# leakless21/VietVoice-TTS

Hardware: AMD Instinct MI355X
Metric: audio-seconds/sec (24 kHz) at batch 32, 256-token utterances; RTF (higher is better)
Workload: dtype bf16

## Files before the change

vietvoice-tts_amd/csrc/vv_api.hip:

```cpp
#include <hip/hip_runtime.h>
#include <algorithm>
#include <cmath>
#include <cstdarg>
#include <cstdio>
#include <cstring>
#include <map>
#include <string>
#include <utility>
#include <vector>
#include "vv_kernels.h"

#define VV_VERSION_STR "vvtts-hip 0.14 (gfx950)"

namespace {
std::string g_create_error;

struct Bound { const void* p; uint64_t bytes; };

struct ProfRec { hipEvent_t a, b; int cls, sub; };

inline size_t align_up(size_t v, size_t a) { return (v + a - 1) / a * a; }
inline int pad_to(int v, int a) { return (v + a - 1) / a * a; }
}

struct vv_ctx {
    int device = 0;
    vv_model_cfg cfg{};
    int dt = VV_DTYPE_BF16;
    std::string err;
    std::map<std::string, Bound> w;
    bool finalized = false;
    bool ever_finalized = false;
    bool vocos = false;
    vv_vocos_cfg vcfg{};
    float post_bias = 0.f;
    int n_steps = 0;
    std::vector<float> dt_host;
    float* modtab = nullptr;
    float* fintab = nullptr;
    int ode_s = 1;
    double ode_a[16] = {}, ode_b[4] = {1.0, 0, 0, 0};
    int ode_kslot[4] = {-1, -1, -1, -1};
    int ode_nk = 0;
    int ms_q = 0;
    std::vector<double> ms_beta;
    double* ode_report = nullptr;
    int report_steps = 0, report_B = 0;
    char* ws = nullptr;
    size_t ws_cap = 0;
    uint64_t ws_generation = 0;
    int* d_mult = nullptr;
    int rope_rows = 0;
    int split_k_tail = 0;
    int chip_share = 1;
    int ring_tiles_max = 256;
    int ring_tiles = 1;
    int pp_min_tiles = -1;
    int lanes = 0;
    hipStream_t side_stream[1] = {};
    hipEvent_t ev_fork = nullptr, ev_join[1] = {};
    float rope_theta = 0.f;
    int rope_q_attn = 1;
    int voc_x3 = -1;
    int voc_x3_rows = 0;
    char* x3_buf = nullptr;
    std::map<std::string, const void*> x3_w;
    int fuse_mrf = 2;
    bool prof = false;
    std::vector<ProfRec> recs;
    std::vector<hipEvent_t> pool;
    int64_t p_launch[VV_PROF_NCLASS]{};
    double p_flops[VV_PROF_NCLASS]{}, p_bytes[VV_PROF_NCLASS]{}, p_ms[VV_PROF_NCLASS]{};

    int fail(int code, const char* fmt, ...) {
        char buf[1024];
        va_list ap;
        va_start(ap, fmt);
        vsnprintf(buf, sizeof buf, fmt, ap);
        va_end(ap);
        err = buf;
        return code;
    }
    const void* W(const std::string& n) const {
        auto it = w.find(n);
        return it == w.end() ? nullptr : it->second.p;
    }
    const float* Wf(const std::string& n) const { return (const float*)W(n); }
    int esz() const { return dt == VV_DTYPE_BF16 ? 2 : 4; }
    int bk() const { return dt == VV_DTYPE_BF16 ? 64 : 32; }
};

namespace {

#define HIPCHK(ctx, call)                                                                   \
    do {                                                                                    \
        hipError_t e__ = (call);                                                            \
        if (e__ != hipSuccess) return (ctx)->fail(-5, "%s: %s", #call, hipGetErrorString(e__)); \
    } while (0)

#define KCHK(ctx, call)                                              \
    do {                                                             \
        const char* m__ = "";                                        \
        int r__ = (call);                                            \
        if (r__ != 0) return (ctx)->fail(r__, "%s", m__);            \
    } while (0)

struct Prof {
    vv_ctx* c; int idx = -1; hipStream_t st;
    Prof(vv_ctx* c_, int cls, double flops, double bytes, hipStream_t st_, int sub = -1) : c(c_), st(st_) {
        if (!c->prof) return;
        ProfRec r; r.cls = cls; r.sub = sub;
        if (sub >= 0) { c->p_launch[sub]++; c->p_flops[sub] += flops; c->p_bytes[sub] += bytes; }
        auto get = [&]() { hipEvent_t e; if (!c->pool.empty()) { e = c->pool.back(); c->pool.pop_back(); } else hipEventCreate(&e); return e; };
        r.a = get(); r.b = get();
        hipEventRecord(r.a, st);
        c->recs.push_back(r); idx = (int)c->recs.size() - 1;
        c->p_launch[cls]++; c->p_flops[cls] += flops; c->p_bytes[cls] += bytes;
    }
    ~Prof() { if (idx >= 0) hipEventRecord(c->recs[idx].b, st); }
};

struct Arena {
    char* base = nullptr; size_t cap = 0, off = 0;
    template <typename T> T* take(size_t n) { off = align_up(off, 256); T* p = base ? (T*)(base + off) : nullptr; off += n * sizeof(T); return p; }
};
template <typename F> size_t plan_bytes(F&& plan) { Arena dry; plan(dry); return dry.off; }
int ensure_ws(vv_ctx* c, size_t bytes, Arena* a) {
    if (bytes > c->ws_cap) {
        if (c->ws) { hipDeviceSynchronize(); hipFree(c->ws); c->ws = nullptr; c->ws_cap = 0; }
        const size_t want = align_up(bytes + bytes / 16, 1 << 20);
        hipError_t e = hipMalloc((void**)&c->ws, want);
        if (e != hipSuccess) return c->fail(-12, "workspace hipMalloc(%zu MiB): %s", want >> 20, hipGetErrorString(e));
        c->ws_cap = want; ++c->ws_generation;
    }
    *a = Arena{c->ws, c->ws_cap, 0};
    return 0;
}
int use_ws(vv_ctx* c, void* block, size_t have, size_t need, Arena* a) {
    if ((uintptr_t)block % 256) return c->fail(-22, "workspace block must be 256-byte aligned");
    if (have < need) return c->fail(-22, "workspace block too small: %zu < %zu bytes", have, need);
    *a = Arena{(char*)block, have, 0};
    return 0;
}
template <typename F> int plan_ws(vv_ctx* c, void* block, size_t have, F&& plan) {
    const size_t need = plan_bytes(plan);
    Arena a;
    if (int r = block ? use_ws(c, block, have, need, &a) : ensure_ws(c, need, &a)) return r;
    plan(a);
    if (a.off > a.cap) return c->fail(-14, "workspace plan took %zu bytes of a %zu-byte block", a.off, a.cap);
    return 0;
}

struct Gemm : vv_gemm_args { const char* wname; };
Gemm gemm_args(const vv_ctx* c, int dtype, int out_dtype, int mode, int act, const void* A, int lda, const char* wname, int ldw,
               const char* bname, void* C, int ldc, int M, int N, int K) {
    Gemm g{};
    g.dtype = dtype; g.out_dtype = out_dtype; g.mode = mode; g.act = act;
    g.A = A; g.lda = lda; g.W = c->W(wname); g.ldw = ldw; g.C = C; g.ldc = ldc; g.M = M; g.N = N; g.K = K;
    g.bias = bname ? c->Wf(bname) : nullptr; g.wname = wname;
    if (bname && !g.bias) g.W = nullptr;
    return g;
}
int launch_gemm(vv_ctx* c, Gemm g, int cls, hipStream_t st, double alg_flops = -1) {
    if (!g.W) return c->fail(-2, "weight '%s' is not bound", g.wname);
    const int M = g.M, N = g.N, K = g.K, bf16 = g.dtype == VV_DTYPE_BF16;
    if (!g.chip_share) g.chip_share = c->chip_share;
    if (g.tile == 0 && c->pp_min_tiles >= 0 && bf16 && N % 256 == 0)
        g.tile = (M >= 4096 && (long long)((M + 255) / 256) * (N / 256) >= c->pp_min_tiles) ? 256 : 128;
    if (c->ring_tiles && g.tile == 0 && bf16 && N <= 1024 && N % 64 == 0 && (long long)((M + 63) / 64) * (N / 128) <= c->ring_tiles_max)
        g.tile = 6464;
    const int esz = bf16 ? 2 : 4, osz = g.out_dtype == VV_DTYPE_BF16 ? 2 : 4;
    const double fl = alg_flops >= 0 ? alg_flops : 2.0 * M * (double)N * K;
    Prof p(c, cls, fl, (double)M * K * esz + (double)N * K * esz + (double)M * N * osz * (g.mode == VV_EPI_GATE_RES ? 2 : 1), st);
    const char* m = "";
    if (int r = vvk_gemm(&g, st, &m)) return c->fail(r, "%s (weight %s, M=%d N=%d K=%d)", m, g.wname, M, N, K);
    return 0;
}

std::string blk(int i, const char* s) { return "blocks." + std::to_string(i) + s; }

inline hipStream_t enter(vv_ctx* c, void* stream) {
    hipSetDevice(c->device);
    return (hipStream_t)stream;
}

inline bool fits(int64_t off, int64_t n, int64_t total) { return off >= 0 && n >= 0 && n <= total && off <= total - n; }

inline bool spans_overlap(const void* a, uint64_t na, const void* b, uint64_t nb) {
    return (uintptr_t)a < (uintptr_t)b + nb && (uintptr_t)b < (uintptr_t)a + na;
}

struct PtrArg { const char* name; const void* p; unsigned align = 1; bool may_be_null = false; };

int check_ptrs(vv_ctx* c, const char* entry, std::initializer_list<PtrArg> args) {
    for (const PtrArg& a : args) {
        if (!a.p && !a.may_be_null) return c->fail(-22, "%s: null pointer (%s)", entry, a.name);
        if ((uintptr_t)a.p % a.align) return c->fail(-22, "%s: misaligned pointer (%s: %u bytes)", entry, a.name, a.align);
    }
    return 0;
}

int check_ws(vv_ctx* c, const char* entry, uint64_t have, uint64_t need, const char* what = "ws") {
    return have < need ? c->fail(-22, "%s: %s of %llu bytes, %llu are needed", entry, what, (unsigned long long)have, (unsigned long long)need) : 0;
}

int flac_rows(vv_ctx* c, const char* name, const int64_t* rows, const int64_t* rows_host, int R, int64_t n_bytes, int* max_channels) {
    if (R < 1 || R > 65535 || n_bytes < 8 || n_bytes > ((int64_t)1 << 31) - 64)
        return c->fail(-22, "%s: bad sizes (1 <= R <= 65535, 8 <= n_bytes <= 2^31 - 64)", name);
    if (int e = check_ptrs(c, name, {{"rows", rows, 8}, {"rows_host", rows_host, 8}})) return e;
    int64_t at = 0;
    *max_channels = 1;
    for (int r = 0; r < R; ++r) {
        const int64_t* q = rows_host + 8 * (size_t)r;
        if (q[0] < at || q[0] % 4 || !fits(q[0], q[1], n_bytes - 8))
            return c->fail(-22, "%s: row %d: the clips lie in ascending order, 4-byte aligned, inside data less 8 bytes of padding", name, r);
        if (q[2] < 1 || q[2] > 8 || (q[3] != 8 && q[3] != 16 && q[3] != 24) || q[5] < 16 || q[5] > 65535 || q[4] < 0 || q[4] > q[5] || q[6] < 1 ||
            q[6] > 1048575 || q[7] < 0 || q[7] > VV_FLAC_MAX_CLIP)
            return c->fail(-22, "%s: row %d: channels 1 ... 8, bits 8 / 16 / 24, 16 <= max block <= 65535, min <= max, rate 1 ... 1048575, total <= 2^26", name, r);
        at = q[0] + q[1];
        if (q[2] > *max_channels) *max_channels = (int)q[2];
    }
    return 0;
}

}

extern "C" {

const char* vv_version(void) { return VV_VERSION_STR; }

const char* vv_last_error(const vv_ctx* ctx) { return ctx ? ctx->err.c_str() : g_create_error.c_str(); }

int vv_create(vv_ctx** out, int device, const vv_model_cfg* cfg, int acoustic_dtype) {
    if (!out || !cfg) { g_create_error = "vv_create: null argument"; return -22; }
    *out = nullptr;
    int n = 0;
    hipError_t e = hipGetDeviceCount(&n);
    if (e != hipSuccess || n <= 0) { g_create_error = "vv_create: no HIP device visible (the HIP path has no CPU fallback)"; return -19; }
    if (device < 0 || device >= n) { g_create_error = "vv_create: device index out of range"; return -22; }
    if (acoustic_dtype != VV_DTYPE_F32 && acoustic_dtype != VV_DTYPE_BF16) { g_create_error = "vv_create: dtype must be f32 or bf16"; return -22; }
    if (cfg->head_dim != 64 || cfg->heads * 64 != cfg->dim) { g_create_error = "vv_create: head_dim must be 64"; return -22; }
    if (cfg->dim % 128 || cfg->text_dim % 128 || cfg->dim / cfg->pos_conv_groups != 64 || cfg->n_mel % 4 || cfg->dim > 1024 ||
        cfg->text_dim > 1024) {
        g_create_error = "vv_create: dim/text_dim must be multiples of 128 (<=1024), 64 channels per pos-conv group"; return -22;
    }
    if (cfg->voc_n_up < 1 || cfg->voc_n_up > VV_MAX_UP || cfg->voc_n_res > VV_MAX_RES || cfg->voc_n_dil > VV_MAX_RES) {
        g_create_error = "vv_create: vocoder topology out of range"; return -22;
    }
    e = hipSetDevice(device);
    if (e != hipSuccess) { g_create_error = hipGetErrorString(e); return -5; }
    vv_ctx* c = new vv_ctx();
    c->device = device; c->cfg = *cfg; c->dt = acoustic_dtype;
    *out = c;
    return 0;
}

void vv_destroy(vv_ctx* c) {
    if (!c) return;
    hipSetDevice(c->device);
    hipDeviceSynchronize();
    if (c->ws) hipFree(c->ws);
    if (c->modtab) hipFree(c->modtab);
    if (c->fintab) hipFree(c->fintab);
    if (c->d_mult) hipFree(c->d_mult);
    if (c->x3_buf) hipFree(c->x3_buf);
    for (auto q : c->side_stream) if (q) hipStreamDestroy(q);
    if (c->ev_fork) hipEventDestroy(c->ev_fork);
    for (auto e : c->ev_join) if (e) hipEventDestroy(e);
    for (auto& r : c->recs) { hipEventDestroy(r.a); hipEventDestroy(r.b); }
    for (auto e : c->pool) hipEventDestroy(e);
    delete c;
}

int vv_bind_weight(vv_ctx* c, const char* name, const void* p, uint64_t bytes) {
    if (!c || !name || !p) return c ? c->fail(-22, "vv_bind_weight: null argument") : -22;
    if ((uintptr_t)p % 16) return c->fail(-22, "vv_bind_weight(%s): pointer must be 16-byte aligned", name);
    c->w[name] = Bound{p, bytes};
    c->finalized = false;
    return 0;
}

int vv_finalize_weights(vv_ctx* c) {
    if (!c) return -22;
    const vv_model_cfg& g = c->cfg;
    const int D = g.dim, Dt = g.text_dim, FF = g.dim * g.ff_mult, es = c->esz();
    const int KP = pad_to(2 * g.n_mel + Dt, 64), MP = pad_to(g.n_mel, 128);
    std::string missing;
    auto need = [&](const std::string& n, uint64_t bytes) {
        auto it = c->w.find(n);
        if (it == c->w.end()) { missing += n + " "; return; }
        if (it->second.bytes < bytes) missing += n + "(short:" + std::to_string(it->second.bytes) + "<" + std::to_string(bytes) + ") ";
    };
    need("const.window", 4ull * g.n_fft); need("const.tw_cos", 4ull * g.n_fft); need("const.tw_sin", 4ull * g.n_fft);
    need("const.mel_fb", 4ull * (g.n_fft / 2 + 1) * g.n_mel);
    need("const.text_pos", 4ull * g.max_pos * Dt);
    need("text.embed.weight", 4ull * g.vocab_rows * Dt);
    for (int i = 0; i < g.text_layers; ++i) {
        const std::string p = "text.blocks." + std::to_string(i);
        need(p + ".dwconv.weight", 4ull * Dt * g.text_conv_k); need(p + ".dwconv.bias", 4ull * Dt);
        need(p + ".norm.weight", 4ull * Dt); need(p + ".norm.bias", 4ull * Dt);
        need(p + ".pwconv1.weight", (uint64_t)es * Dt * g.text_ff_mult * Dt); need(p + ".pwconv1.bias", 4ull * Dt * g.text_ff_mult);
        need(p + ".grn.gamma", 4ull * Dt * g.text_ff_mult); need(p + ".grn.beta", 4ull * Dt * g.text_ff_mult);
        need(p + ".pwconv2.weight", (uint64_t)es * Dt * g.text_ff_mult * Dt); need(p + ".pwconv2.bias", 4ull * Dt);
    }
    need("input.proj.weight", (uint64_t)es * D * KP); need("input.proj.bias", 4ull * D);
    for (int j = 1; j <= 2; ++j) {
        need("input.pos_conv" + std::to_string(j) + ".weight", (uint64_t)es * D * 64 * g.pos_conv_k);
        need("input.pos_conv" + std::to_string(j) + ".bias", 4ull * D);
    }
    need("time.mlp1.weight", 4ull * D * g.time_freq_dim); need("time.mlp1.bias", 4ull * D);
    need("time.mlp2.weight", 4ull * D * D); need("time.mlp2.bias", 4ull * D);
    for (int i = 0; i < g.depth; ++i) {
        need(blk(i, ".adaln.weight"), 4ull * 6 * D * D); need(blk(i, ".adaln.bias"), 4ull * 6 * D);
        need(blk(i, ".attn.qkv.weight"), (uint64_t)es * 3 * D * D); need(blk(i, ".attn.qkv.bias"), 4ull * 3 * D);
        need(blk(i, ".attn.out.weight"), (uint64_t)es * D * D); need(blk(i, ".attn.out.bias"), 4ull * D);
        need(blk(i, ".ff1.weight"), (uint64_t)es * FF * D); need(blk(i, ".ff1.bias"), 4ull * FF);
        need(blk(i, ".ff2.weight"), (uint64_t)es * D * FF); need(blk(i, ".ff2.bias"), 4ull * D);
    }
    need("final.adaln.weight", 4ull * 2 * D * D); need("final.adaln.bias", 4ull * 2 * D);
    need("final.proj.weight", (uint64_t)es * MP * D); need("final.proj.bias", 4ull * MP);
    if (c->vocos) {
        const vv_vocos_cfg& v = c->vcfg;
        const uint64_t V = v.dim, I = v.intermediate, KE = pad_to(v.embed_k * g.n_mel, 32), HP = pad_to(v.n_fft + 2, 128);
        need("const.istft_basis", 4ull * v.n_fft * v.n_fft);
        need("voc.embed.weight", 4 * V * KE); need("voc.embed.bias", 4 * V);
        for (const char* n : {"voc.norm", "voc.final_norm"}) { need(std::string(n) + ".weight", 4 * V); need(std::string(n) + ".bias", 4 * V); }
        for (int i = 0; i < v.layers; ++i) {
            const std::string p = "voc.blocks." + std::to_string(i);
            need(p + ".dwconv.weight", 4 * V * v.dw_k); need(p + ".dwconv.bias", 4 * V);
            need(p + ".norm.weight", 4 * V); need(p + ".norm.bias", 4 * V);
            need(p + ".pwconv1.weight", 4 * I * V); need(p + ".pwconv1.bias", 4 * I);
            need(p + ".pwconv2.weight", 4 * V * I); need(p + ".pwconv2.bias", 4 * V);
            need(p + ".gamma", 4 * V);
        }
        need("voc.head.weight", 4 * HP * V); need("voc.head.bias", 4 * HP);
        if (!missing.empty()) return c->fail(-2, "missing or short weights: %s", missing.c_str());
        c->finalized = c->ever_finalized = true;
        return 0;
    }
    int ch = g.voc_pre_ch;
    struct ConvW { std::string name; int cin_pad, kw, rows_pad; };
    std::vector<ConvW> convs;
    convs.push_back({"voc.pre.weight", pad_to(g.n_mel, 8), g.voc_pre_k, pad_to(ch, 64)});
    need("voc.pre.weight", 4ull * pad_to(g.n_mel, 8) * g.voc_pre_k * pad_to(ch, 64)); need("voc.pre.bias", 4ull * ch);
    for (int s = 0; s < g.voc_n_up; ++s) {
        const int cin = ch, cout = ch / 2, u = g.voc_up_rates[s];
        const std::string p = "voc.up." + std::to_string(s);
        need(p + ".weight", 4ull * pad_to(cin, 8) * 2 * pad_to(cout * u, 64)); need(p + ".bias", 4ull * cout);
        convs.push_back({p + ".weight", pad_to(cin, 8), 2, pad_to(cout * u, 64)});
        for (int a = 0; a < g.voc_n_res; ++a)
            for (int b = 0; b < g.voc_n_dil; ++b)
                for (int k = 1; k <= 2; ++k) {
                    const std::string q = "voc.res." + std::to_string(s) + "." + std::to_string(a) + "." + std::to_string(b) + ".conv" + std::to_string(k);
                    need(q + ".weight", 4ull * pad_to(cout, 8) * g.voc_res_kernels[a] * pad_to(cout, 64)); need(q + ".bias", 4ull * cout);
                    convs.push_back({q + ".weight", pad_to(cout, 8), g.voc_res_kernels[a], pad_to(cout, 64)});
                }
        ch = cout;
    }
    need("voc.post.weight", 4ull * ch * g.voc_post_k); need("voc.post.bias", 4);
    if (!missing.empty()) return c->fail(-2, "missing or short weights: %s", missing.c_str());
    hipSetDevice(c->device);
    HIPCHK(c, hipMemcpy(&c->post_bias, c->W("voc.post.bias"), 4, hipMemcpyDeviceToHost));
    {
        size_t total = 0;
        for (const ConvW& w : convs) total = align_up(total, 256) + vvk_conv_split_bytes(w.cin_pad, w.kw, w.rows_pad);
        if (c->x3_buf) { HIPCHK(c, hipFree(c->x3_buf)); c->x3_buf = nullptr; }
        c->x3_w.clear();
        HIPCHK(c, hipMalloc((void**)&c->x3_buf, total));
        size_t off = 0;
        for (const ConvW& w : convs) {
            off = align_up(off, 256);
            const char* m__ = "";
            if (int r = vvk_conv_split_weights(c->Wf(w.name), w.cin_pad, w.kw, w.rows_pad, c->x3_buf + off, nullptr, &m__))
                return c->fail(r, "%s (%s)", m__, w.name.c_str());
            c->x3_w[w.name] = c->x3_buf + off;
            off += vvk_conv_split_bytes(w.cin_pad, w.kw, w.rows_pad);
        }
        HIPCHK(c, hipStreamSynchronize(nullptr));
    }
    std::vector<int> mult(g.voc_n_up + 1, 1);
    for (int s = 0; s < g.voc_n_up; ++s) mult[s + 1] = mult[s] * g.voc_up_rates[s];
    if (!c->d_mult) HIPCHK(c, hipMalloc((void**)&c->d_mult, sizeof(int) * (VV_MAX_UP + 1)));
    HIPCHK(c, hipMemcpy(c->d_mult, mult.data(), sizeof(int) * mult.size(), hipMemcpyHostToDevice));
    c->finalized = c->ever_finalized = true;
    return 0;
}

int vv_set_vocos(vv_ctx* c, const vv_vocos_cfg* v) {
    if (!c) return -22;
    if (!v) return c->fail(-22, "vv_set_vocos: null cfg");
    if (c->ever_finalized) return c->fail(-22, "vv_set_vocos: only between vv_create and vv_finalize_weights");
    const vv_model_cfg& g = c->cfg;
    if (v->dim < 128 || v->dim > 1024 || v->dim % 128 || v->intermediate < 128 || v->intermediate > 16384 || v->intermediate % 128)
        return c->fail(-22, "vv_set_vocos: dim must be a multiple of 128 in [128, 1024], intermediate a multiple of 128 (fp32 GEMM tiles)");
    if (v->layers < 1 || v->layers > 64 || v->embed_k < 1 || v->embed_k > 31 || v->embed_k % 2 == 0 || v->dw_k < 1 || v->dw_k > 31 || v->dw_k % 2 == 0 ||
        !(v->ln_eps > 0.f))
        return c->fail(-22, "vv_set_vocos: 1..64 layers, odd kernel sizes up to 31, ln_eps > 0");
    if (v->n_fft != v->win_length || v->n_fft != g.n_fft || g.win_length != g.n_fft || v->hop_length != g.hop_length || v->n_fft % 128 ||
        v->hop_length < 1 || v->n_fft % v->hop_length || v->n_fft / v->hop_length > 16)
        return c->fail(-22, "vv_set_vocos: the ISTFT needs n_fft == win_length == the model's n_fft (a multiple of 128) and the model's hop "
                            "(dividing n_fft, at most 16 frames per sample)");
    c->vcfg = *v;
    c->vocos = true;
    return 0;
}

static int set_plan_impl(vv_ctx* c, const char* who, const float* sinus_host, const float* dt_host, int n_steps, int s, const double* a,
                         const double* b, void* stream) {
    if (!c) return -22;
    if (!c->finalized) return c->fail(-1, "%s: weights not finalized", who);
    if (n_steps < 1 || n_steps > 512 || !sinus_host || !dt_host) return c->fail(-22, "%s: bad arguments", who);
    if (s < 1 || s > 4 || !a || !b) return c->fail(-22, "%s: 1 to 4 stages with their tableau", who);
    if ((long long)n_steps * s > 512) return c->fail(-22, "%s: %d steps x %d stages exceed 512 evaluations", who, n_steps, s);
    double sum_b = 0;
    for (int i = 0; i < s; ++i) {
        if (!std::isfinite(b[i])) return c->fail(-22, "%s: the tableau must be finite", who);
        sum_b += b[i];
        for (int j = 0; j < s; ++j) {
            if (!std::isfinite(a[i * s + j])) return c->fail(-22, "%s: the tableau must be finite", who);
            if (j >= i && a[i * s + j] != 0.0) return c->fail(-22, "%s: the tableau must be strictly lower triangular (explicit method)", who);
        }
    }
    if (!(std::fabs(sum_b - 1.0) < 1e-6)) return c->fail(-22, "%s: the weights b must sum to 1", who);
    for (int n = 0; n < n_steps; ++n)
        if (!std::isfinite(dt_host[n])) return c->fail(-22, "%s: the step sizes must be finite", who);
    hipSetDevice(c->device);
    hipStream_t st = (hipStream_t)stream;
    const int D = c->cfg.dim, S = n_steps * s, TF = c->cfg.time_freq_dim, L = c->cfg.depth;
    if (TF % 32) return c->fail(-22, "time_freq_dim must be a multiple of 32");
    if (c->modtab) { hipDeviceSynchronize(); hipFree(c->modtab); hipFree(c->fintab); c->modtab = c->fintab = nullptr; }
    HIPCHK(c, hipMalloc((void**)&c->modtab, sizeof(float) * (size_t)L * S * 6 * D));
    HIPCHK(c, hipMalloc((void**)&c->fintab, sizeof(float) * (size_t)S * 2 * D));
    float *sin_d, *t1, *t2;
    auto bufs = [&](Arena& a) { sin_d = a.take<float>((size_t)S * TF); t1 = a.take<float>((size_t)S * D); t2 = a.take<float>((size_t)S * D); };
    if (int r = plan_ws(c, nullptr, 0, bufs)) return r;
    HIPCHK(c, hipMemcpyAsync(sin_d, sinus_host, 4ull * S * TF, hipMemcpyHostToDevice, st));
    HIPCHK(c, hipStreamSynchronize(st));
    const int f32 = VV_DTYPE_F32, store = VV_EPI_STORE;
    if (int r = launch_gemm(c, gemm_args(c, f32, f32, store, VV_ACT_SILU_, sin_d, TF, "time.mlp1.weight", TF, "time.mlp1.bias", t1, D, S, D, TF), VV_PROF_GEMM, st)) return r;
    if (int r = launch_gemm(c, gemm_args(c, f32, f32, store, VV_ACT_SILU_, t1, D, "time.mlp2.weight", D, "time.mlp2.bias", t2, D, S, D, D), VV_PROF_GEMM, st)) return r;
    for (int l = 0; l < L; ++l) {
        const std::string wn = blk(l, ".adaln.weight"), bn = blk(l, ".adaln.bias");
        if (int r = launch_gemm(c, gemm_args(c, f32, f32, store, VV_ACT_NONE_, t2, D, wn.c_str(), D, bn.c_str(), c->modtab + (size_t)l * S * 6 * D, 6 * D, S, 6 * D, D), VV_PROF_GEMM, st)) return r;
    }
    if (int r = launch_gemm(c, gemm_args(c, f32, f32, store, VV_ACT_NONE_, t2, D, "final.adaln.weight", D, "final.adaln.bias", c->fintab, 2 * D, S, 2 * D, D), VV_PROF_GEMM, st)) return r;
    HIPCHK(c, hipStreamSynchronize(st));
    c->n_steps = n_steps;
    c->dt_host.assign(dt_host, dt_host + n_steps);
    c->ode_s = s;
    std::fill(c->ode_a, c->ode_a + 16, 0.0);
    std::fill(c->ode_b, c->ode_b + 4, 0.0);
    for (int i = 0; i < s; ++i) {
        c->ode_b[i] = b[i];
        for (int j = 0; j < i; ++j) c->ode_a[i * 4 + j] = a[i * s + j];
    }
    c->ode_nk = 0;
    for (int j = 0; j < 4; ++j) {
        bool later = j < s - 1 && c->ode_b[j] != 0.0;
        for (int m = j + 2; m < s; ++m) later = later || c->ode_a[m * 4 + j] != 0.0;
        c->ode_kslot[j] = later ? c->ode_nk++ : -1;
    }
    c->ms_q = 0; c->ms_beta.clear();
    c->ode_report = nullptr; c->report_steps = c->report_B = 0;
    return 0;
}

int vv_set_time_grid(vv_ctx* c, const float* sinus_host, const float* dt_host, int n_steps, void* stream) {
    const double a = 0.0, b = 1.0;
    return set_plan_impl(c, "vv_set_time_grid", sinus_host, dt_host, n_steps, 1, &a, &b, stream);
}

int vv_set_ode_plan(vv_ctx* c, const float* sinus_host, const float* dt_host, int n_steps, int s, const double* a, const double* b, void* stream) {
    return set_plan_impl(c, "vv_set_ode_plan", sinus_host, dt_host, n_steps, s, a, b, stream);
}

int vv_set_ode_multistep(vv_ctx* c, const float* sinus_host, const float* dt_host, int n_steps, int q, const double* beta, void* stream) {
    if (!c) return -22;
    if (n_steps < 1 || n_steps > 512) return c->fail(-22, "vv_set_ode_multistep: bad arguments");
    if (q < 1 || q > 3 || !beta) return c->fail(-22, "vv_set_ode_multistep: 1 to 3 slopes per step with their weights");
    for (int n = 0; n < n_steps; ++n) {
        double sum = 0;
        for (int j = 0; j < q; ++j) {
            const double v = beta[(size_t)n * q + j];
            if (!std::isfinite(v)) return c->fail(-22, "vv_set_ode_multistep: the weights must be finite");
            if (j > n && v != 0.0) return c->fail(-22, "vv_set_ode_multistep: step %d has a weight on a slope from before step 0", n);
            sum += v;
        }
        if (!(std::fabs(sum - 1.0) < 1e-6)) return c->fail(-22, "vv_set_ode_multistep: the weights of step %d must sum to 1", n);
    }
    const double a = 0.0, b = 1.0;
    if (int r = set_plan_impl(c, "vv_set_ode_multistep", sinus_host, dt_host, n_steps, 1, &a, &b, stream)) return r;
    c->ms_q = q;
    c->ms_beta.assign(beta, beta + (size_t)n_steps * q);
    return 0;
}

int vv_set_ode_report(vv_ctx* c, double* report, int n_steps, int B) {
    if (!c) return -22;
    if (!report) { c->ode_report = nullptr; c->report_steps = c->report_B = 0; return 0; }
    if (c->ms_q < 1) return c->fail(-22, "vv_set_ode_report: the report needs a multistep plan (vv_set_ode_multistep)");
    if (n_steps != c->n_steps || B < 1 || B > VVK_GUIDE_MAX_ITEMS) return c->fail(-22, "vv_set_ode_report: [%d steps of the plan][1..%d items][2]", c->n_steps, VVK_GUIDE_MAX_ITEMS);
    if ((uintptr_t)report % 8) return c->fail(-22, "vv_set_ode_report: report must be a float64 array");
    c->ode_report = report; c->report_steps = n_steps; c->report_B = B;
    return 0;
}

static int preprocess_impl(vv_ctx* c, int B, int N, const int16_t* audio, int ld_audio, int max_audio_len, const int32_t* audio_len,
                           const int32_t* audio_len_host, const int32_t* text_ids, int ld_text, const int32_t* text_len, const int32_t* seq_len,
                           float* cat, float* cat_drop, int32_t* ref_len, void* stream, const uint8_t* keep = nullptr, int ld_keep = 0) {
    if (!c) return -22;
    if (!c->finalized) return c->fail(-1, "vv_preprocess: weights not finalized");
    if (B < 1 || N < 1 || !audio || !audio_len || !text_ids || !text_len || !seq_len || !cat || !cat_drop || !ref_len)
        return c->fail(-22, "vv_preprocess: bad arguments");
    const vv_model_cfg& g = c->cfg;
    if (N > g.max_pos) return c->fail(-22, "vv_preprocess: N=%d exceeds the position tables (%d)", N, g.max_pos);
    if (max_audio_len < g.n_fft || max_audio_len > ld_audio) return c->fail(-22, "vv_preprocess: reference clips must hold >= n_fft samples and fit ld_audio");
    if (audio_len_host)
        for (int b = 0; b < B; ++b)
            if (audio_len_host[b] < g.n_fft / 2 + 1 || audio_len_host[b] > max_audio_len)
                return c->fail(-22, "vv_preprocess: reference clip %d has %d samples; a clip needs between n_fft/2 + 1 = %d and max_audio_len = %d",
                               b, audio_len_host[b], g.n_fft / 2 + 1, max_audio_len);
    hipSetDevice(c->device);
    hipStream_t st = (hipStream_t)stream;
    const int Dt = g.text_dim, C2 = Dt * g.text_ff_mult, M = g.n_mel, es = c->esz();
    const int F_max = max_audio_len / g.hop_length + 1;
    const size_t R2 = (size_t)2 * B * N;
    float *mel, *tx, *ty, *sumsq;
    char *th, *tm;
    auto bufs = [&](Arena& a) {
        mel = a.take<float>((size_t)B * F_max * M);
        tx = a.take<float>(R2 * Dt); ty = a.take<float>(R2 * Dt);
        th = a.take<char>((size_t)es * R2 * Dt); tm = a.take<char>((size_t)es * R2 * C2);
        sumsq = a.take<float>((size_t)2 * B * C2);
    };
    if (int r = plan_ws(c, nullptr, 0, bufs)) return r;

    KCHK(c, vvk_ref_len(audio_len, ref_len, B, g.hop_length, st, &m__));
    {
        Prof p(c, VV_PROF_MEL, 4.0 * B * F_max * (double)g.n_fft * (g.n_fft / 2 + 1), 2.0 * B * max_audio_len + 4.0 * B * F_max * M, st);
        KCHK(c, vvk_mel(audio, ld_audio, audio_len, c->Wf("const.window"), c->Wf("const.tw_cos"), c->Wf("const.tw_sin"),
                        c->Wf("const.mel_fb"), mel, B, F_max, g.n_fft, g.hop_length, M, st, &m__));
    }
    {
        Prof p(c, VV_PROF_TEXT, 0, 8.0 * R2 * Dt, st);
        KCHK(c, vvk_text_embed(text_ids, ld_text, text_len, c->Wf("text.embed.weight"), c->Wf("const.text_pos"), tx, B, N, Dt, g.vocab_rows, st, &m__));
    }
    for (int i = 0; i < g.text_layers; ++i) {
        const std::string p = "text.blocks." + std::to_string(i);
        {
            Prof pr(c, VV_PROF_TEXT, 2.0 * R2 * Dt * g.text_conv_k, 8.0 * R2 * Dt, st);
            KCHK(c, vvk_dwconv(tx, ty, c->Wf(p + ".dwconv.weight"), c->Wf(p + ".dwconv.bias"), seq_len, B, 2 * B, N, Dt, g.text_conv_k, st, &m__));
        }
        {
            vv_ln_args a{}; a.out_dtype = c->dt; a.x = ty; a.ldx = Dt; a.y = th; a.ldy = Dt; a.R = (int)R2; a.D = Dt;
            a.w = c->Wf(p + ".norm.weight"); a.b = c->Wf(p + ".norm.bias"); a.add_one = 0; a.eps = 1e-6f;
            Prof pr(c, VV_PROF_NORM, 0, (4.0 + es) * R2 * Dt, st);
            KCHK(c, vvk_ln_mod(&a, st, &m__));
        }
        const std::string w1 = p + ".pwconv1.weight", b1 = p + ".pwconv1.bias", w2 = p + ".pwconv2.weight", b2 = p + ".pwconv2.bias";
        if (int r = launch_gemm(c, gemm_args(c, c->dt, c->dt, VV_EPI_STORE, VV_ACT_GELU_ERF_, th, Dt, w1.c_str(), Dt, b1.c_str(), tm, C2, (int)R2, C2, Dt), VV_PROF_GEMM, st)) return r;
        {
            Prof pr(c, VV_PROF_TEXT, 0, 3.0 * es * R2 * C2, st);
            KCHK(c, vvk_grn(c->dt, tm, sumsq, c->Wf(p + ".grn.gamma"), c->Wf(p + ".grn.beta"), seq_len, B, 2 * B, N, C2, st, &m__));
        }
        if (int r = launch_gemm(c, gemm_args(c, c->dt, VV_DTYPE_F32, VV_EPI_GATE_RES, VV_ACT_NONE_, tm, C2, w2.c_str(), C2, b2.c_str(), tx, Dt, (int)R2, Dt, C2), VV_PROF_GEMM, st)) return r;
    }
    {
        Prof p(c, VV_PROF_ELEMWISE, 0, 12.0 * B * N * (M + Dt) + (keep ? (double)B * N : 0.0), st);
        KCHK(c, vvk_build_cat(mel, F_max, ref_len, tx, cat, cat_drop, B, N, M, Dt, st, &m__, keep, ld_keep));
    }
    if (keep) HIPCHK(c, hipMemsetAsync(ref_len, 0, sizeof(int32_t) * B, st));
    return 0;
}

int vv_preprocess(vv_ctx* c, int B, int N, const int16_t* audio, int ld_audio, int max_audio_len, const int32_t* audio_len,
                  const int32_t* text_ids, int ld_text, const int32_t* text_len, const int32_t* seq_len, float* cat,
                  float* cat_drop, int32_t* ref_len, void* stream) {
    return preprocess_impl(c, B, N, audio, ld_audio, max_audio_len, audio_len, nullptr, text_ids, ld_text, text_len, seq_len, cat, cat_drop, ref_len, stream);
}

int vv_preprocess_h(vv_ctx* c, int B, int N, const int16_t* audio, int ld_audio, int max_audio_len, const int32_t* audio_len,
                    const int32_t* audio_len_host, const int32_t* text_ids, int ld_text, const int32_t* text_len, const int32_t* seq_len,
                    float* cat, float* cat_drop, int32_t* ref_len, void* stream) {
    if (c && !audio_len_host) return c->fail(-22, "vv_preprocess_h: host lengths missing");
    return preprocess_impl(c, B, N, audio, ld_audio, max_audio_len, audio_len, audio_len_host, text_ids, ld_text, text_len, seq_len, cat, cat_drop, ref_len, stream);
}

int vv_preprocess_edit(vv_ctx* c, int B, int N, const int16_t* audio, int ld_audio, int max_audio_len, const int32_t* audio_len,
                       const int32_t* audio_len_host, const int32_t* text_ids, int ld_text, const int32_t* text_len, const int32_t* seq_len,
                       float* cat, float* cat_drop, int32_t* ref_len, const uint8_t* keep, int ld_keep, void* stream) {
    if (!c) return -22;
    if (!audio_len_host) return c->fail(-22, "vv_preprocess_edit: host lengths missing");
    if (!keep || ld_keep < N) return c->fail(-22, "vv_preprocess_edit: keep must be a device array [B][ld_keep] with ld_keep >= N");
    return preprocess_impl(c, B, N, audio, ld_audio, max_audio_len, audio_len, audio_len_host, text_ids, ld_text, text_len, seq_len, cat, cat_drop,
                           ref_len, stream, keep, ld_keep);
}

int vv_edit_splice(vv_ctx* c, const int16_t* src, int64_t n_src, const int64_t* desc, int n_rows, int B, int16_t* out, int ld_out, void* stream) {
    if (!c) return -22;
    if (B < 1 || n_rows < 0 || n_src < 0 || !out || ld_out < 4 || ld_out % 4 || (uintptr_t)out % 8 || (n_rows > 0 && (!src || !desc)))
        return c->fail(-22, "vv_edit_splice: bad arguments (out [B][ld_out] 8-byte aligned with ld_out %% 4 == 0; src and desc for n_rows > 0)");
    hipSetDevice(c->device);
    hipStream_t st = (hipStream_t)stream;
    Prof p(c, VV_PROF_ELEMWISE, 0, 4.0 * B * ld_out + 32.0 * n_rows, st);
    KCHK(c, vvk_edit_splice(src, (long long)n_src, (const long long*)desc, n_rows, B, out, ld_out, st, &m__));
    return 0;
}

int vv_edit_restore(vv_ctx* c, int B, int N, float* x, const float* cat, const uint8_t* keep, int ld_keep, const int32_t* seq_len, void* stream) {
    if (!c) return -22;
    const int M = c->cfg.n_mel, cd = c->cfg.n_mel + c->cfg.text_dim;
    if (B < 1 || N < 1 || !x || !cat || !keep || !seq_len || ld_keep < N || (uintptr_t)x % 16 || (uintptr_t)cat % 16)
        return c->fail(-22, "vv_edit_restore: bad arguments (x, cat 16-byte aligned; keep [B][ld_keep] with ld_keep >= N)");
    hipSetDevice(c->device);
    hipStream_t st = (hipStream_t)stream;
    Prof p(c, VV_PROF_ELEMWISE, 0, (double)B * N * (1 + 8.0 * M), st);
    KCHK(c, vvk_edit_restore(x, cat, keep, ld_keep, seq_len, B, N, M, cd, st, &m__));
    return 0;
}

int vv_noise_fill(vv_ctx* c, int B, int N, int n_mel, float* x, const int32_t* seq_len, const uint64_t* keys, int kind, void* stream) {
    if (!c) return -22;
    if (B < 1 || N < 1 || n_mel < 4 || n_mel % 4 || (kind != 0 && kind != 1) || !x || !seq_len || !keys || (uintptr_t)x % 16 || (uintptr_t)keys % 8)
        return c->fail(-22, "vv_noise_fill: bad arguments (B, N >= 1; n_mel %% 4 == 0; x 16-byte aligned; keys [B][2] uint64; kind 0 or 1)");
    hipSetDevice(c->device);
    hipStream_t st = (hipStream_t)stream;
    Prof p(c, VV_PROF_ELEMWISE, 0, (double)B * (12.0 + 4.0 * N * n_mel), st);
    KCHK(c, vvk_noise_fill(x, seq_len, (const unsigned long long*)keys, B, N, n_mel, kind, st, &m__));
    return 0;
}

int vv_join_chunks(vv_ctx* c, const int16_t* pcm, int64_t n_pcm, const int64_t* chunk_rows, const int64_t* chunk_rows_host, int n_chunks,
                   const int64_t* req_rows, const int64_t* req_rows_host, int R, const double* fade, int64_t n_fade, int max_n, int64_t max_len,
                   int16_t* out, int64_t n_out, void* ws, void* stream) {
    if (!c) return -22;
    hipStream_t st = enter(c, stream);
    if (R < 1 || n_chunks < R || max_n < 0 || max_n > vvk_join_max_n())
        return c->fail(-22, "vv_join_chunks: bad arguments (1 <= R <= n_chunks; max_n <= %d)", vvk_join_max_n());
    if (int e = check_ptrs(c, "vv_join_chunks", {{"pcm", pcm}, {"chunk_rows", chunk_rows}, {"req_rows", req_rows}, {"out", out, 16}, {"ws", ws}})) return e;
    if ((chunk_rows_host == nullptr) != (req_rows_host == nullptr)) return c->fail(-22, "vv_join_chunks: host rows come as a pair or not at all");
    if (chunk_rows_host) {
        for (int r = 0; r < R; ++r) {
            const int64_t* q = req_rows_host + 4 * (size_t)r;
            if (q[1] < 1 || !fits(q[0], q[1], n_chunks) || !fits(q[2], q[3], n_out))
                return c->fail(-22, "vv_join_chunks: request row %d does not fit the chunk rows or the output", r);
            for (int64_t k = q[0]; k < q[0] + q[1]; ++k) {
                const int64_t* w = chunk_rows_host + 8 * (size_t)k;
                if (!fits(w[0], w[1], n_pcm) || w[2] < 0 || w[3] < 0 || w[3] > max_n || w[1] > max_len || w[7] != r ||
                    (w[3] > 0 && !fits(w[5], 2 * w[3], n_fade)))
                    return c->fail(-22, "vv_join_chunks: chunk row %lld does not fit the buffers", (long long)k);
                if (q[1] >= 2 && w[1] <= 0)
                    return c->fail(-22, "vv_join_chunks: chunk %lld is empty inside a request of %lld chunks", (long long)k, (long long)q[1]);
            }
        }
    }
    Prof p(c, VV_PROF_ELEMWISE, 0, 4.0 * (double)n_out + 96.0 * n_chunks, st);
    KCHK(c, vvk_join_chunks(pcm, (long long)n_pcm, (const long long*)chunk_rows, n_chunks, (const long long*)req_rows, R, fade, (long long)n_fade,
                            max_n, (long long)max_len, out, (long long)n_out, ws, st, &m__));
    return 0;
}

int vv_pcm_resample(vv_ctx* c, const int16_t* x, int64_t n_x, const int64_t* rows, int n_rows, int64_t max_out, const double* taps, int n_taps,
                    int up, int down, int skip, int16_t* y, int64_t n_y, void* stream) {
    if (!c) return -22;
    hipStream_t st = enter(c, stream);
    if (n_rows < 1 || n_taps < 1 || up < 1 || down < 1 || skip < 0 || max_out < 0)
        return c->fail(-22, "vv_pcm_resample: bad arguments (n_rows, n_taps, up, down >= 1; skip, max_out >= 0)");
    if (int e = check_ptrs(c, "vv_pcm_resample", {{"x", x}, {"rows", rows}, {"taps", taps}, {"y", y}})) return e;
    Prof p(c, VV_PROF_ELEMWISE, 2.0 * (double)n_y * (n_taps / up + 1), 2.0 * (double)(n_x + n_y), st);
    KCHK(c, vvk_pcm_resample(x, (long long)n_x, (const long long*)rows, n_rows, (long long)max_out, taps, n_taps, up, down, skip, y, (long long)n_y,
                             st, &m__));
    return 0;
}

int vv_pcm_encode(vv_ctx* c, const int16_t* x, int64_t n_x, const int64_t* rows, int n_rows, int64_t max_n, int kind, uint8_t* y, int64_t n_y,
                  void* stream) {
    if (!c) return -22;
    hipStream_t st = enter(c, stream);
    if (n_rows < 1 || (kind != 1 && kind != 2) || max_n < 0)
        return c->fail(-22, "vv_pcm_encode: bad arguments (n_rows >= 1; kind 1 = mu-law, 2 = A-law)");
    if (int e = check_ptrs(c, "vv_pcm_encode", {{"x", x}, {"rows", rows}, {"y", y, 8}})) return e;
    Prof p(c, VV_PROF_ELEMWISE, 0, 2.0 * (double)n_x + (double)n_y, st);
    KCHK(c, vvk_pcm_encode(x, (long long)n_x, (const long long*)rows, n_rows, (long long)max_n, kind, y, (long long)n_y, st, &m__));
    return 0;
}

uint64_t vv_pcm_loudness_ws_bytes(int64_t total_runs, int R) { return vvk_pcm_loudness_ws_bytes((long long)total_runs, R); }

int vv_pcm_loudness(vv_ctx* c, const int16_t* x, int64_t n_x, const int64_t* rows, const int64_t* rows_host, int R, int64_t sub,
                    const double* tables, const double* params, int16_t* y, int64_t n_y, double* stats, void* ws, uint64_t ws_bytes,
                    void* stream) {
    if (!c) return -22;
    hipStream_t st = enter(c, stream);
    if (R < 1 || R > 65535 || sub < VV_LOUD_RUN || sub > (1 << 24) || n_x < 0 || n_y < 0)
        return c->fail(-22, "vv_pcm_loudness: bad sizes (1 <= R <= 65535; sub >= %d)", VV_LOUD_RUN);
    if (int e = check_ptrs(c, "vv_pcm_loudness", {{"x", x, 2}, {"y", y, 2, true}, {"rows", rows, 8}, {"rows_host", rows_host}, {"tables", tables, 8},
                                                  {"params", params, 8}, {"stats", stats, 8}, {"ws", ws, 8}})) return e;
    const int64_t rps = (sub + VV_LOUD_RUN - 1) / VV_LOUD_RUN;
    int64_t total_runs = 0, max_n = 0;
    for (int r = 0; r < R; ++r) {
        const int64_t* q = rows_host + 4 * (size_t)r;
        if (!fits(q[0], q[1], n_x) || q[1] >= ((int64_t)1 << 40))
            return c->fail(-22, "vv_pcm_loudness: row %d does not fit the %lld samples of x", r, (long long)n_x);
        if (y && !fits(q[2], q[1], n_y)) return c->fail(-22, "vv_pcm_loudness: row %d does not fit the %lld samples of y", r, (long long)n_y);
        if (y == x && q[2] != q[0]) return c->fail(-22, "vv_pcm_loudness: in place (y == x) needs dst_off == src_off, row %d", r);
        if (q[3] != total_runs) return c->fail(-22, "vv_pcm_loudness: row %d: run_off is the sum of the runs of the rows before it", r);
        const int64_t J = q[1] / sub;
        total_runs += J * rps + (q[1] - J * sub + VV_LOUD_RUN - 1) / VV_LOUD_RUN;
        if (q[1] > max_n) max_n = q[1];
    }
    if (int e = check_ws(c, "vv_pcm_loudness", ws_bytes, vvk_pcm_loudness_ws_bytes((long long)total_runs, R))) return e;
    Prof p(c, VV_PROF_ELEMWISE, 60.0 * (double)n_x, 6.0 * (double)n_x + 128.0 * (double)total_runs, st);
    KCHK(c, vvk_pcm_loudness(x, (long long)n_x, (const long long*)rows, R, (long long)sub, (long long)total_runs, (long long)max_n, tables,
                             params, y, (long long)n_y, stats, ws, st, &m__));
    return 0;
}

int vv_pcm_limit_tile(int L) { return L < 1 || L > VV_LIMIT_MAX_L ? -22 : vvk_pcm_limit_tile(L); }

uint64_t vv_pcm_limit_ws_bytes(int64_t total_samples, int64_t total_tiles, int R) {
    return vvk_pcm_limit_ws_bytes((long long)total_samples, (long long)total_tiles, R);
}

int vv_pcm_limit(vv_ctx* c, const int16_t* x, int64_t n_x, const int64_t* rows, const int64_t* rows_host, int R, int L, int mode,
                 const double* window, const double* taps, const double* params, const double* meas, int16_t* y, int64_t n_y, double* stats,
                 void* ws, uint64_t ws_bytes, void* stream) {
    if (!c) return -22;
    hipStream_t st = enter(c, stream);
    if (R < 1 || R > 65535 || L < 1 || L > VV_LIMIT_MAX_L || (mode != 0 && mode != 1) || n_x < 0 || n_y < 0)
        return c->fail(-22, "vv_pcm_limit: bad sizes (1 <= R <= 65535; 1 <= L <= %d; mode 0 or 1)", VV_LIMIT_MAX_L);
    if (int e = check_ptrs(c, "vv_pcm_limit", {{"x", x, 2}, {"y", y, 2, true}, {"rows", rows, 8}, {"rows_host", rows_host}, {"window", window, 8},
                                               {"taps", taps, 8}, {"params", params, 8}, {"meas", meas, 8, true}, {"stats", stats, 8}, {"ws", ws, 8}})) return e;
    const int64_t tile = vvk_pcm_limit_tile(L);
    int64_t total_samples = 0, total_tiles = 0, max_tiles = 0, max_out = 0;
    for (int r = 0; r < R; ++r) {
        const int64_t* q = rows_host + 5 * (size_t)r;
        if (q[0] < 0 || q[1] < 0 || q[2] < 0 || q[3] < 0 || q[4] < 0) return c->fail(-22, "vv_pcm_limit: row %d has a negative field", r);
        if (!fits(q[0], q[1], n_x) || q[1] >= ((int64_t)1 << 40))
            return c->fail(-22, "vv_pcm_limit: row %d does not fit the %lld samples of x", r, (long long)n_x);
        if (!fits(q[3], q[4], q[1])) return c->fail(-22, "vv_pcm_limit: row %d: out_lo + out_n exceeds n", r);
        if (y && !fits(q[2], q[4], n_y)) return c->fail(-22, "vv_pcm_limit: row %d does not fit the %lld samples of y", r, (long long)n_y);
        if (y == x && q[4] > 0 && q[2] != q[0] + q[3])
            return c->fail(-22, "vv_pcm_limit: in place (y == x) needs dst_off == src_off + out_lo, row %d", r);
        const int64_t nt = (q[1] + tile - 1) / tile;
        total_samples += q[1];
        total_tiles += nt;
        if (nt > max_tiles) max_tiles = nt;
        if (q[4] > max_out) max_out = q[4];
    }
    if (int e = check_ws(c, "vv_pcm_limit", ws_bytes, vvk_pcm_limit_ws_bytes((long long)total_samples, (long long)total_tiles, R))) return e;
    Prof p(c, VV_PROF_ELEMWISE, (mode ? 640.0 : 500.0) * (double)total_samples * (double)(2 * L + 1) / 241.0,
           20.0 * (double)total_samples + 2.0 * (double)max_out * R, st);
    KCHK(c, vvk_pcm_limit(x, (long long)n_x, (const long long*)rows, R, L, mode, (long long)total_samples, (long long)total_tiles,
                          (long long)max_tiles, (long long)max_out, window, taps, params, meas, y, (long long)n_y, stats, ws, st, &m__));
    return 0;
}

uint64_t vv_pcm_stretch_ws_bytes(int R) { return vvk_pcm_stretch_ws_bytes(R); }

int vv_pcm_stretch(vv_ctx* c, const int16_t* x, int64_t n_x, const int64_t* rows, const int64_t* rows_host, int R, const double* window,
                   int16_t* y, int64_t n_y, int32_t* pos, int64_t n_pos, void* ws, uint64_t ws_bytes, void* stream) {
    if (!c) return -22;
    hipStream_t st = enter(c, stream);
    if (R < 1 || R > 65535 || n_x < 0 || n_y < 0 || n_pos < 0) return c->fail(-22, "vv_pcm_stretch: bad sizes (1 <= R <= 65535)");
    if (int e = check_ptrs(c, "vv_pcm_stretch", {{"x", x, 2}, {"y", y, 2, true}, {"rows", rows, 8}, {"rows_host", rows_host}, {"window", window, 8},
                                                 {"pos", pos, 4}, {"ws", ws, 8}})) return e;
    if (y && spans_overlap(x, 2ull * n_x, y, 2ull * n_y))
        return c->fail(-22, "vv_pcm_stretch: y overlaps x (an output sample reads two frames of the input: not in place)");
    if (int e = check_ws(c, "vv_pcm_stretch", ws_bytes, vvk_pcm_stretch_ws_bytes(R))) return e;
    std::vector<std::pair<int64_t, int64_t>> on_y, on_pos;
    int64_t total_out = 0, total_frames = 0, max_out = 0;
    for (int r = 0; r < R; ++r) {
        const int64_t* q = rows_host + 6 * (size_t)r;
        if (q[0] < 0 || q[1] < 0 || q[2] < 0 || q[5] < 0) return c->fail(-22, "vv_pcm_stretch: row %d has a negative field", r);
        if (q[3] < 1 || q[3] > VV_WSOLA_MAX_PQ || q[4] < 1 || q[4] > VV_WSOLA_MAX_PQ || q[3] == q[4] || 4 * q[3] < q[4] || q[3] > 4 * q[4])
            return c->fail(-22, "vv_pcm_stretch: row %d: p and q in 1 ... %d, p != q, 1/4 <= p / q <= 4", r, VV_WSOLA_MAX_PQ);
        if (!fits(q[0], q[1], n_x) || q[1] > ((int64_t)1 << 30))
            return c->fail(-22, "vv_pcm_stretch: row %d does not fit the %lld samples of x", r, (long long)n_x);
        const int64_t n_s = (q[1] * q[3] + q[4] - 1) / q[4], M = (n_s + VV_WSOLA_HS - 1) / VV_WSOLA_HS;
        if (y && !fits(q[2], n_s, n_y)) return c->fail(-22, "vv_pcm_stretch: row %d does not fit the %lld samples of y", r, (long long)n_y);
        if (!fits(q[5], M + 1, n_pos)) return c->fail(-22, "vv_pcm_stretch: row %d does not fit the %lld entries of pos", r, (long long)n_pos);
        if (y && n_s > 0) on_y.emplace_back(q[2], q[2] + n_s);
        on_pos.emplace_back(q[5], q[5] + M + 1);
        total_out += n_s;
        total_frames += M;
        if (n_s > max_out) max_out = n_s;
    }
    for (auto* spans : {&on_y, &on_pos}) {
        std::sort(spans->begin(), spans->end());
        for (size_t i = 1; i < spans->size(); ++i)
            if ((*spans)[i].first < (*spans)[i - 1].second)
                return c->fail(-22, "vv_pcm_stretch: rows overlap on %s", spans == &on_y ? "y" : "pos");
    }
    Prof p(c, VV_PROF_ELEMWISE, 2.0 * (double)total_frames * VV_WSOLA_N * 2 * VV_WSOLA_D + 3.0 * (double)total_out,
           2.0 * (double)total_frames * (2 * VV_WSOLA_N + 2 * VV_WSOLA_D) + 6.0 * (double)total_out, st);
    KCHK(c, vvk_pcm_stretch(x, (long long)n_x, (const long long*)rows, R, (long long)max_out, window, y, (long long)n_y, (int*)pos,
                            (long long)n_pos, ws, st, &m__));
    return 0;
}

uint64_t vv_pcm_formant_ws_bytes(int64_t total_frames, int R) { return vvk_pcm_formant_ws_bytes((long long)total_frames, R); }

int vv_pcm_formant(vv_ctx* c, const int16_t* x, int64_t n_x, const int16_t* y, int64_t n_y, const int64_t* rows, const int64_t* rows_host, int R,
                   const double* wa, const double* g, const double* window, int16_t* z, int64_t n_z, double* h_out, int64_t n_h, void* ws,
                   uint64_t ws_bytes, void* stream) {
    if (!c) return -22;
    hipStream_t st = enter(c, stream);
    if (R < 1 || R > 65535 || n_x < 0 || n_y < 0 || n_z < 0 || n_h < 0) return c->fail(-22, "vv_pcm_formant: bad sizes (1 <= R <= 65535)");
    if (int e = check_ptrs(c, "vv_pcm_formant", {{"x", x, 2}, {"y", y, 2}, {"rows", rows, 8}, {"rows_host", rows_host}, {"wa", wa, 8}, {"g", g, 8},
                                                 {"window", window, 8}, {"z", z, 2}, {"h_out", h_out, 8, true}, {"ws", ws, 8}})) return e;
    if (spans_overlap(x, 2ull * n_x, z, 2ull * n_z) || spans_overlap(y, 2ull * n_y, z, 2ull * n_z))
        return c->fail(-22, "vv_pcm_formant: z overlaps x or y (an output sample reads L samples of y: not in place)");
    std::vector<std::pair<int64_t, int64_t>> on_z;
    int64_t total_frames = 0, max_frames = 0, total_out = 0;
    for (int r = 0; r < R; ++r) {
        const int64_t* q = rows_host + 7 * (size_t)r;
        if (q[0] < 0 || q[1] < 0 || q[2] < 0 || q[3] < 0 || q[4] < 0) return c->fail(-22, "vv_pcm_formant: row %d has a negative field", r);
        if (q[5] < 1 || q[5] > VV_WSOLA_MAX_PQ || q[6] < 1 || q[6] > VV_WSOLA_MAX_PQ)
            return c->fail(-22, "vv_pcm_formant: row %d: tn and td in 1 ... %d", r, VV_WSOLA_MAX_PQ);
        if (!fits(q[0], q[1], n_x) || q[1] > ((int64_t)1 << 30))
            return c->fail(-22, "vv_pcm_formant: row %d does not fit the %lld samples of x", r, (long long)n_x);
        if (q[3] != (q[1] * q[6] + q[5] - 1) / q[5]) return c->fail(-22, "vv_pcm_formant: row %d: n_f is not ceil(n td / tn)", r);
        if (!fits(q[2], q[3], n_y)) return c->fail(-22, "vv_pcm_formant: row %d does not fit the %lld samples of y", r, (long long)n_y);
        if (!fits(q[4], q[3], n_z)) return c->fail(-22, "vv_pcm_formant: row %d does not fit the %lld samples of z", r, (long long)n_z);
        const int64_t frames = (q[3] + VV_FORMANT_H - 1) / VV_FORMANT_H + 1;
        if (q[3] > 0) on_z.emplace_back(q[4], q[4] + q[3]);
        total_frames += frames;
        total_out += q[3];
        if (frames > max_frames) max_frames = frames;
    }
    std::sort(on_z.begin(), on_z.end());
    for (size_t i = 1; i < on_z.size(); ++i)
        if (on_z[i].first < on_z[i - 1].second) return c->fail(-22, "vv_pcm_formant: rows overlap on z");
    if (h_out && n_h / VV_FORMANT_L < total_frames)
        return c->fail(-22, "vv_pcm_formant: h_out of %lld doubles, %lld are needed", (long long)n_h, (long long)total_frames * VV_FORMANT_L);
    if (int e = check_ws(c, "vv_pcm_formant", ws_bytes, vvk_pcm_formant_ws_bytes((long long)total_frames, R))) return e;
    Prof p(c, VV_PROF_ELEMWISE, 4.0 * (double)total_out * VV_FORMANT_L + 2.0 * (double)total_frames * VV_FORMANT_L * VV_FORMANT_P,
           24.0 * (double)total_frames * VV_FORMANT_L + 4.0 * (double)total_out, st);
    KCHK(c, vvk_pcm_formant(x, (long long)n_x, y, (long long)n_y, (const long long*)rows, R, (long long)total_frames, (long long)max_frames, wa, g,
                            window, z, (long long)n_z, h_out, ws, st, &m__));
    return 0;
}

uint64_t vv_pcm_denoise_ws_bytes(int R) { return vvk_pcm_denoise_ws_bytes(R); }

int vv_pcm_denoise(vv_ctx* c, const int16_t* x, int64_t n_x, const int64_t* rows, const int64_t* rows_host, int R, const double* strengths,
                   const double* strengths_host, const double* bias, int64_t n_bias, const double* window, const double* twiddles, int16_t* y,
                   int64_t n_y, double* mag_out, int64_t n_mag, void* ws, uint64_t ws_bytes, void* stream) {
    if (!c) return -22;
    hipStream_t st = enter(c, stream);
    if (R < 1 || R > 65535 || n_x < 0 || n_y < 0 || n_bias < 1 || n_mag < 0) return c->fail(-22, "vv_pcm_denoise: bad sizes (1 <= R <= 65535, n_bias >= 1)");
    if (int e = check_ptrs(c, "vv_pcm_denoise", {{"x", x, 2}, {"rows", rows, 8}, {"rows_host", rows_host}, {"strengths", strengths, 8},
                                                 {"strengths_host", strengths_host}, {"bias", bias, 8}, {"window", window, 8},
                                                 {"twiddles", twiddles, 8}, {"y", y, 2}, {"mag_out", mag_out, 8, true}, {"ws", ws, 8}})) return e;
    if (spans_overlap(x, 2ull * n_x, y, 2ull * n_y))
        return c->fail(-22, "vv_pcm_denoise: y overlaps x (a hop reads the input under its neighbours: not in place)");
    std::vector<std::pair<int64_t, int64_t>> on_y;
    int64_t total_frames = 0, max_hops = 1, total_hops = 0;
    for (int r = 0; r < R; ++r) {
        const int64_t* q = rows_host + 4 * (size_t)r;
        if (q[0] < 0 || q[1] < 0 || q[2] < 0 || q[3] < 0) return c->fail(-22, "vv_pcm_denoise: row %d has a negative field", r);
        if (q[3] >= n_bias) return c->fail(-22, "vv_pcm_denoise: row %d: bias_row %lld of %lld", r, (long long)q[3], (long long)n_bias);
        if (!(strengths_host[r] >= 0.0 && strengths_host[r] <= 16.0)) return c->fail(-22, "vv_pcm_denoise: row %d: a strength in 0 ... 16 is needed", r);
        if (!fits(q[0], q[1], n_x) || q[1] > ((int64_t)1 << 30))
            return c->fail(-22, "vv_pcm_denoise: row %d does not fit the %lld samples of x", r, (long long)n_x);
        if (!fits(q[2], q[1], n_y)) return c->fail(-22, "vv_pcm_denoise: row %d does not fit the %lld samples of y", r, (long long)n_y);
// ... 581 lines not shown
            }
        }
        return n_views;
    }
};

int steps_schedule(const StepsRun& r, Lane* lanes, hipStream_t st) {
    vv_ctx* c = r.c;
    const int n_lanes = r.P.n_lanes, step0 = r.q.a.step0, n_steps = r.q.a.n_steps;
    const bool branch_lanes = r.P.branch_lanes, guide = r.q.guide != nullptr;
    if ((n_lanes > 1 || branch_lanes) && !c->side_stream[0]) {
        HIPCHK(c, hipStreamCreateWithFlags(&c->side_stream[0], hipStreamNonBlocking));
        HIPCHK(c, hipEventCreateWithFlags(&c->ev_join[0], hipEventDisableTiming));
    }
    if ((n_lanes > 1 || branch_lanes) && !c->ev_fork) HIPCHK(c, hipEventCreateWithFlags(&c->ev_fork, hipEventDisableTiming));
    const hipStream_t streams[2] = {st, c->side_stream[0]};
    auto fork = [&]() -> int {
        HIPCHK(c, hipEventRecord(c->ev_fork, st)); HIPCHK(c, hipStreamWaitEvent(c->side_stream[0], c->ev_fork, 0));
        return 0;
    };
    auto join = [&]() { hipEventRecord(c->ev_join[0], c->side_stream[0]); hipStreamWaitEvent(st, c->ev_join[0], 0); };
    Lane views[2]; GuideState gstate[2];
    auto make_views = [&](const GuideState* gs) {
        const int n = r.lane_views(gs, views);
        for (int v = 0; v < n; ++v) views[v].st = streams[v];
        return c->chip_share = n;
    };
    for (int li = 0; li < n_lanes; ++li) lanes[li].st = streams[li];
    int n_views = make_views(nullptr), rc = 0;
    if (n_lanes > 1) rc = fork();
    for (int li = 0; li < n_lanes && !rc; ++li) rc = r.setup(lanes[li]);
    for (int s = step0; s < step0 + n_steps && !rc; ++s)
        for (int i = 0; i < r.ns && !rc; ++i) {
            const int e = s * r.ns + i;
            for (int li = 0; li < n_lanes && !rc; ++li) rc = r.pack(lanes[li], gstate[li], s, i);
            if (guide) n_views = make_views(gstate);
            const bool want_fork = branch_lanes && n_views == 2;
            if (want_fork && !rc) rc = fork();
            const bool forked = want_fork && !rc;
            for (int v = 0; v < n_views && !rc; ++v) rc = r.step_head(views[v]);
            for (int l = 0; l < r.g.depth && !rc; ++l)
                for (int v = 0; v < n_views && !rc; ++v) rc = r.block(views[v], e, l);
            for (int v = 0; v < n_views && !rc; ++v) rc = r.step_tail(views[v], e);
            if (forked) join();
            for (int li = 0; li < n_lanes && !rc; ++li) rc = r.combine(lanes[li], s, i);
        }
    if (n_lanes > 1) join();
    c->chip_share = 1;
    return rc;
}
}

static int transformer_steps(vv_ctx* c, StepsCall q, void* stream) {
    if (!c) return -22;
    const vv_steps_args& a = q.a;
    q.with_apg = q.apg != nullptr || q.ws_form == WS_APG; q.guided = q.guide != nullptr || q.ws_form != WS_PLAIN || q.with_apg;
    q.rk = c->ode_s > 1 || c->ms_q > 0 || a.cfg_item != nullptr || q.guide != nullptr || q.apg != nullptr;
    const int B = a.B, N = a.N;
    if (!c->finalized || !c->modtab) return c->fail(-1, "vv_transformer_steps: weights/time grid not ready");
    if (B < 1 || N < 1 || (!q.ws_only && (!a.seq_len || !a.x || !a.cat_mel_text || !a.cat_mel_text_drop || !a.rope_cos_q || !a.rope_sin_q || !a.rope_cos_k || !a.rope_sin_k)))
        return c->fail(-22, "vv_transformer_steps: bad arguments");
    if (a.step0 < 0 || a.n_steps < 0 || a.step0 + a.n_steps > c->n_steps) return c->fail(-22, "vv_transformer_steps: steps [%d,%d) outside the time grid (%d)", a.step0, a.step0 + a.n_steps, c->n_steps);
    if (c->ms_q && !q.ws_only && a.step0 != 0) return c->fail(-22, "vv_transformer_steps: under a multistep plan a call starts at step 0 (the kept slopes live for one call), got step0 = %d", a.step0);
    if (c->ms_q && c->ode_report && !q.ws_only && (c->report_B != B || c->report_steps != c->n_steps))
        return c->fail(-22, "vv_transformer_steps: the step report was set for %d steps of %d items, the call has %d of %d", c->report_steps, c->report_B, c->n_steps, B);
    if (q.guide && q.ld_guide < B) return c->fail(-22, "vv_transformer_steps_guided: ld_guide = %d < B = %d", q.ld_guide, B);
    if (q.guide && c->split_k_tail) return c->fail(-22, "vv_transformer_steps_guided: a guidance mask cannot be combined with option split_k_tail (its tail plan depends on the row count)");
    if (q.guided && B > VVK_GUIDE_MAX_ITEMS) return c->fail(-22, "vv_transformer_steps_guided: at most %d items per call", VVK_GUIDE_MAX_ITEMS);
    q.with_drift = q.ws_form == WS_REUSE_REPORT || (q.reuse && q.reuse->report); q.with_reuse = q.with_drift || q.ws_form == WS_REUSE;
    if (q.reuse_entry && !q.ws_only) {
        const int E = c->n_steps * c->ode_s, ns = c->ode_s, e0 = a.step0 * ns, e1 = (a.step0 + a.n_steps) * ns;
        if (q.with_drift && !q.guide) return c->fail(-22, "vv_transformer_steps_reuse: the drift report needs a mask");
        if (q.with_drift && ((uintptr_t)q.reuse->report % 8 || q.reuse->report_B != B || q.reuse->report_evals != E))
            return c->fail(-22, "vv_transformer_steps_reuse: the report is float64 [%d evaluations of the plan][%d items][2], got [%d][%d][2]", E, B, q.reuse->report_evals, q.reuse->report_B);
        bool has2 = false;
        for (int e = 0; e < E && q.guide; ++e)
            for (int b = 0; b < B; ++b) {
                const uint8_t v = q.guide[(size_t)e * q.ld_guide + b];
                if (v > 2) return c->fail(-22, "vv_transformer_steps_reuse: mask value %d at evaluation %d, item %d (0 = not guided, 1 = computed, 2 = reused)", (int)v, e, b);
                has2 = has2 || v == 2;
            }
        if (has2 && a.step0 != 0) return c->fail(-22, "vv_transformer_steps_reuse: a call that reuses starts at step 0 (the stored differences live for one call), got step0 = %d", a.step0);
        q.with_reuse = q.with_reuse || has2;
        if (q.with_reuse) {
            q.ru_mode.assign((size_t)(e1 - e0) * B, 0); q.ru_old.assign((size_t)(e1 - e0) * B, 0);
            for (int b = 0; b < B; ++b) {
                bool seen = false, need = false;
                for (int e = e0; e < e1; ++e) {
                    const uint8_t v = q.guide[(size_t)e * q.ld_guide + b];
                    if (v == 2 && !seen) return c->fail(-22, "vv_transformer_steps_reuse: item %d reuses at evaluation %d with no computed evaluation before it in the call", b, e);
                    q.ru_old[(size_t)(e - e0) * B + b] = seen;
                    if (v == 2) q.ru_mode[(size_t)(e - e0) * B + b] = VV_REUSE_LOAD;
                    seen = seen || v == 1;
                }
                for (int e = e1 - 1; e >= e0; --e) {
                    const uint8_t v = q.guide[(size_t)e * q.ld_guide + b];
                    if (v == 2) need = true;
                    if (v == 1) { if (need || q.with_drift) q.ru_mode[(size_t)(e - e0) * B + b] = VV_REUSE_STORE; need = false; }
                }
            }
        }
    }
    hipStream_t st = enter(c, stream);
    const vv_model_cfg& g = c->cfg;
    const StepDims d{g.dim, g.dim * g.ff_mult, g.n_mel, g.n_mel + g.text_dim, c->esz(), pad_to(2 * g.n_mel + g.text_dim, 64), pad_to(g.n_mel, 128)};
    if ((size_t)2 * B * N > (size_t)1 << 30) return c->fail(-22, "batch too large");
    std::vector<int> hlen(B);
    if (a.seq_len_host) std::copy(a.seq_len_host, a.seq_len_host + B, hlen.begin());
    else {
        HIPCHK(c, hipMemcpyAsync(hlen.data(), a.seq_len, sizeof(int) * B, hipMemcpyDeviceToHost, st));
        HIPCHK(c, hipStreamSynchronize(st));
    }
    size_t Rc_all = 0;
    for (int b = 0; b < B; ++b) {
        if (hlen[b] < 1 || hlen[b] > N) return c->fail(-22, "vv_transformer_steps: seq_len[%d] = %d outside [1, %d]", b, hlen[b], N);
        Rc_all += hlen[b];
    }
    if (2 * Rc_all * 3 * (size_t)d.D * d.es >= ((size_t)1 << 31))
        return c->fail(-22, "vv_transformer_steps: %zu packed rows make a %zu-byte qkv buffer; kernels address it with 32-bit byte offsets "
                            "(< 2 GiB) -- synthesise fewer units per call", 2 * Rc_all, 2 * Rc_all * 3 * (size_t)d.D * d.es);
    LanePlan P = lane_plan(c, d, hlen, N);
    auto bufs = [&](Arena& ar) { for (int li = 0; li < P.n_lanes; ++li) lane_bufs(ar, P.lanes[li], c, d, N, q.guided, q.with_apg, q.with_reuse, q.with_drift); };
    if (q.ws_only) { *q.ws_only = (uint64_t)align_up(plan_bytes(bufs), 256); return 0; }
    if (int r = plan_ws(c, a.ws, (size_t)a.ws_bytes, bufs)) return r;
    for (int li = 0; li < P.n_lanes; ++li) {
        Lane& L = P.lanes[li];
        L.seq_len = a.seq_len + L.b0; L.x = a.x + (size_t)L.b0 * N * d.M;
        L.cat = a.cat_mel_text + (size_t)L.b0 * N * d.CD; L.cat_drop = a.cat_mel_text_drop + (size_t)L.b0 * N * d.CD;
    }
    return steps_schedule(StepsRun(c, d, q, hlen, P), P.lanes, st);
}

static StepsCall steps_call(int B, int N, const int32_t* seq_len, const int32_t* seq_len_host, float* x, const float* cat, const float* cat_drop,
                            const float* rope_cos_q, const float* rope_sin_q, const float* rope_cos_k, const float* rope_sin_k, int step0, int n_steps) {
    StepsCall q; vv_steps_args& a = q.a;
    a.B = B; a.N = N; a.seq_len = seq_len; a.seq_len_host = seq_len_host; a.x = x; a.cat_mel_text = cat; a.cat_mel_text_drop = cat_drop;
    a.rope_cos_q = rope_cos_q; a.rope_sin_q = rope_sin_q; a.rope_cos_k = rope_cos_k; a.rope_sin_k = rope_sin_k; a.step0 = step0; a.n_steps = n_steps;
    return q;
}
static int steps_struct_call(vv_ctx* c, const char* entry, const vv_steps_args* a, const uint8_t* guide, int ld_guide, const vv_apg_args* apg, void* stream) {
    if (!c) return -22;
    if (!a) return c->fail(-22, "%s: null arguments", entry);
    if (a->ws && !a->seq_len_host) return c->fail(-22, "%s: a workspace block needs the host lengths", entry);
    if (a->cfg_item && (uintptr_t)a->cfg_item % 4) return c->fail(-22, "%s: cfg_item must be a float array", entry);
    if (apg && !apg->t_host) return c->fail(-22, "%s: the evaluation times t_host are required", entry);
    if (apg && ((uintptr_t)apg->eta | (uintptr_t)apg->norm_rms) % 4) return c->fail(-22, "%s: eta and norm_rms must be float arrays", entry);
    StepsCall q; q.a = *a; q.guide = guide; q.ld_guide = ld_guide; q.apg = apg;
    return transformer_steps(c, q, stream);
}
static int steps_ws_query(vv_ctx* c, const char* entry, WsForm form, int B, int N, const int32_t* seq_len_host, uint64_t* bytes) {
    if (c && (!seq_len_host || !bytes)) return c->fail(-22, "%s: bad arguments", entry);
    StepsCall q; q.a.B = B; q.a.N = N; q.a.seq_len_host = seq_len_host; q.ws_form = form; q.ws_only = bytes;
    return transformer_steps(c, q, nullptr);
}

int vv_transformer_steps(vv_ctx* c, int B, int N, const int32_t* seq_len, float* x, const float* cat, const float* cat_drop,
                         const float* rope_cos_q, const float* rope_sin_q, const float* rope_cos_k, const float* rope_sin_k,
                         int step0, int n_steps, void* stream) {
    return transformer_steps(c, steps_call(B, N, seq_len, nullptr, x, cat, cat_drop, rope_cos_q, rope_sin_q, rope_cos_k, rope_sin_k, step0, n_steps), stream);
}

int vv_transformer_steps_h(vv_ctx* c, int B, int N, const int32_t* seq_len, const int32_t* seq_len_host, float* x, const float* cat,
                           const float* cat_drop, const float* rope_cos_q, const float* rope_sin_q, const float* rope_cos_k,
                           const float* rope_sin_k, int step0, int n_steps, void* stream) {
    if (c && !seq_len_host) return c->fail(-22, "vv_transformer_steps_h: host lengths missing");
    return transformer_steps(c, steps_call(B, N, seq_len, seq_len_host, x, cat, cat_drop, rope_cos_q, rope_sin_q, rope_cos_k, rope_sin_k, step0, n_steps), stream);
}

int vv_transformer_ws_bytes(vv_ctx* c, int B, int N, const int32_t* seq_len_host, uint64_t* bytes) {
    return steps_ws_query(c, "vv_transformer_ws_bytes", WS_PLAIN, B, N, seq_len_host, bytes);
}

int vv_transformer_steps_into(vv_ctx* c, int B, int N, const int32_t* seq_len, const int32_t* seq_len_host, float* x, const float* cat,
                              const float* cat_drop, const float* rope_cos_q, const float* rope_sin_q, const float* rope_cos_k,
                              const float* rope_sin_k, int step0, int n_steps, void* ws, uint64_t ws_bytes, void* stream) {
    if (c && (!seq_len_host || !ws)) return c->fail(-22, "vv_transformer_steps_into: host lengths and a workspace block are required");
    StepsCall q = steps_call(B, N, seq_len, seq_len_host, x, cat, cat_drop, rope_cos_q, rope_sin_q, rope_cos_k, rope_sin_k, step0, n_steps);
    q.a.ws = ws; q.a.ws_bytes = ws_bytes;
    return transformer_steps(c, q, stream);
}

int vv_transformer_steps_ex(vv_ctx* c, const vv_steps_args* a, void* stream) {
    return steps_struct_call(c, "vv_transformer_steps_ex", a, nullptr, 0, nullptr, stream);
}

int vv_transformer_steps_guided(vv_ctx* c, const vv_steps_args* a, const uint8_t* guide_host, int ld_guide, void* stream) {
    if (!guide_host) return vv_transformer_steps_ex(c, a, stream);
    return steps_struct_call(c, "vv_transformer_steps_guided", a, guide_host, ld_guide, nullptr, stream);
}

int vv_transformer_guided_ws_bytes(vv_ctx* c, int B, int N, const int32_t* seq_len_host, uint64_t* bytes) {
    return steps_ws_query(c, "vv_transformer_guided_ws_bytes", WS_GUIDED, B, N, seq_len_host, bytes);
}

int vv_transformer_steps_apg(vv_ctx* c, const vv_steps_args* a, const uint8_t* guide_host, int ld_guide, const vv_apg_args* apg, void* stream) {
    if (!apg) return vv_transformer_steps_guided(c, a, guide_host, ld_guide, stream);
    return steps_struct_call(c, "vv_transformer_steps_apg", a, guide_host, ld_guide, apg, stream);
}

int vv_transformer_apg_ws_bytes(vv_ctx* c, int B, int N, const int32_t* seq_len_host, uint64_t* bytes) {
    return steps_ws_query(c, "vv_transformer_apg_ws_bytes", WS_APG, B, N, seq_len_host, bytes);
}

int vv_transformer_steps_reuse(vv_ctx* c, const vv_steps_args* a, const uint8_t* guide_host, int ld_guide, const vv_reuse_args* reuse, void* stream) {
    if (!c) return -22;
    if (!a) return c->fail(-22, "vv_transformer_steps_reuse: null arguments");
    if (!guide_host && !(reuse && reuse->report)) return vv_transformer_steps_ex(c, a, stream);
    if (a->ws && !a->seq_len_host) return c->fail(-22, "vv_transformer_steps_reuse: a workspace block needs the host lengths");
    if (a->cfg_item && (uintptr_t)a->cfg_item % 4) return c->fail(-22, "vv_transformer_steps_reuse: cfg_item must be a float array");
    StepsCall q; q.a = *a; q.guide = guide_host; q.ld_guide = ld_guide; q.reuse_entry = true; q.reuse = reuse;
    return transformer_steps(c, q, stream);
}

int vv_transformer_reuse_ws_bytes(vv_ctx* c, int B, int N, const int32_t* seq_len_host, int with_report, uint64_t* bytes) {
    return steps_ws_query(c, "vv_transformer_reuse_ws_bytes", with_report ? WS_REUSE_REPORT : WS_REUSE, B, N, seq_len_host, bytes);
}

static int vocos_wide(const vv_ctx* c) {
    const vv_vocos_cfg& v = c->vcfg;
    return std::max(std::max(pad_to(v.embed_k * c->cfg.n_mel, 32), v.intermediate), pad_to(v.n_fft + 2, 128));
}
struct VocosBufs { int* lens; float *res, *t, *hn, *big, *spec; };
static VocosBufs vocos_bufs(Arena& a, const vv_ctx* c, int B, int T_max) {
    const size_t R = (size_t)B * T_max, V = c->vcfg.dim;
    VocosBufs w;
    w.lens = a.take<int>(B);
    w.res = a.take<float>(R * V); w.t = a.take<float>(R * V); w.hn = a.take<float>(R * V);
    w.big = a.take<float>(R * vocos_wide(c)); w.spec = a.take<float>(R * c->vcfg.n_fft);
    return w;
}
struct HifiPlan { int Ts[VV_MAX_UP + 1], Cs[VV_MAX_UP + 1]; size_t big; };
static HifiPlan hifi_plan(const vv_model_cfg& g, int t_gen_max) {
    HifiPlan p;
    p.Ts[0] = t_gen_max; p.Cs[0] = g.voc_pre_ch; p.big = (size_t)p.Cs[0] * p.Ts[0];
    for (int s = 0; s < g.voc_n_up; ++s) { p.Ts[s + 1] = p.Ts[s] * g.voc_up_rates[s]; p.Cs[s + 1] = p.Cs[s] / 2; p.big = std::max(p.big, (size_t)p.Cs[s + 1] * p.Ts[s + 1]); }
    return p;
}
struct HifiBufs { float *v0, *buf[5]; int* lens; };
static HifiBufs hifi_bufs(Arena& a, const vv_model_cfg& g, const HifiPlan& p, int B) {
    HifiBufs w{a.take<float>((size_t)B * g.n_mel * p.Ts[0])};
    for (float*& b : w.buf) b = a.take<float>((size_t)B * p.big);
    w.lens = a.take<int>((size_t)(g.voc_n_up + 1) * B);
    return w;
}

int vv_decode_ws_bytes(vv_ctx* c, int B, int t_gen_max, uint64_t* bytes) {
    if (!c || !bytes || B < 1 || t_gen_max < 1) return c ? c->fail(-22, "vv_decode_ws_bytes: bad arguments") : -22;
    Arena dry;
    if (c->vocos) vocos_bufs(dry, c, B, t_gen_max); else hifi_bufs(dry, c->cfg, hifi_plan(c->cfg, t_gen_max), B);
    *bytes = (uint64_t)align_up(dry.off, 256);
    return 0;
}

uint64_t vv_ws_generation(const vv_ctx* c) { return c ? c->ws_generation : 0; }

static Gemm vocos_gemm(const vv_ctx* c, int mode, int act, const float* A, int lda, const char* wn, const char* bn, float* C, int ldc, int M, int N, int K) {
    Gemm g = gemm_args(c, VV_DTYPE_F32, VV_DTYPE_F32, mode, act, A, lda, wn, K, bn, C, ldc, M, N, K);
    g.tile = 128; g.chip_share = 1;
    return g;
}

static int vocos_ln(vv_ctx* c, const float* x, float* y, int R, const std::string& n, hipStream_t st) {
    vv_ln_args a{};
    a.out_dtype = VV_DTYPE_F32; a.x = x; a.ldx = c->vcfg.dim; a.y = y; a.ldy = c->vcfg.dim; a.R = R; a.D = c->vcfg.dim;
    a.w = c->Wf(n + ".weight"); a.b = c->Wf(n + ".bias"); a.add_one = 0; a.eps = c->vcfg.ln_eps;
    Prof p(c, VV_PROF_VOC_CONV, 0, 8.0 * R * c->vcfg.dim, st);
    KCHK(c, vvk_ln_mod(&a, st, &m__));
    return 0;
}

static int vocos_istft(vv_ctx* c, int B, int T_max, const float* head, int ld_head, const int* lens, int16_t* pcm, int ld_pcm, int32_t* pcm_len,
                       float* wave, float* spec, float* frames, hipStream_t st) {
    const int n = c->vcfg.n_fft, hop = c->vcfg.hop_length, R = B * T_max;
    {
        Prof p(c, VV_PROF_VOC_POST, 0, 4.0 * R * ((double)n + 2 + n), st);
        KCHK(c, vvk_vocos_spectrum(head, ld_head, R, n, spec, st, &m__));
    }
    if (int r = launch_gemm(c, vocos_gemm(c, VV_EPI_STORE, VV_ACT_NONE_, spec, n, "const.istft_basis", nullptr, frames, n, R, n, n), VV_PROF_VOC_POST, st)) return r;
    Prof p(c, VV_PROF_VOC_POST, 0, 4.0 * R * (double)n + 6.0 * B * (double)T_max * hop, st);
    KCHK(c, vvk_vocos_ola(frames, n, B, T_max, lens, c->Wf("const.window"), n, hop, pcm, ld_pcm, pcm_len, wave, T_max * hop, st, &m__));
    return 0;
}

static int decode_vocos(vv_ctx* c, int B, int N, const float* x, const int32_t* ref_len, const int32_t* seq_len, int T_max, int16_t* pcm,
                        int ld_pcm, int32_t* pcm_len, float* wave_f32, void* ext_ws, uint64_t ext_bytes, hipStream_t st) {
    const vv_vocos_cfg& v = c->vcfg;
    const int M = c->cfg.n_mel, V = v.dim, I = v.intermediate, KE = pad_to(v.embed_k * M, 32), HP = pad_to(v.n_fft + 2, 128);
    if ((size_t)B * T_max * vocos_wide(c) * 4 >= ((size_t)1 << 31)) return c->fail(-22, "vv_decode: a Vocos plane of 2 GiB or more (split the batch)");
    const int R = B * T_max;
    VocosBufs w;
    if (int r = plan_ws(c, ext_ws, (size_t)ext_bytes, [&](Arena& a) { w = vocos_bufs(a, c, B, T_max); })) return r;
    auto [lens, res, t, hn, big, spec] = w;
    KCHK(c, vvk_vocos_lens(seq_len, ref_len, lens, B, N, T_max, st, &m__));
    {
        Prof p(c, VV_PROF_VOC_CONV, 0, 4.0 * R * ((double)M + KE), st);
        KCHK(c, vvk_vocos_im2col(x, B, N, M, ref_len, seq_len, T_max, v.embed_k, big, KE, st, &m__));
    }
    if (int r = launch_gemm(c, vocos_gemm(c, VV_EPI_STORE, VV_ACT_NONE_, big, KE, "voc.embed.weight", "voc.embed.bias", t, V, R, V, KE), VV_PROF_VOC_CONV, st)) return r;
    if (int r = vocos_ln(c, t, res, R, "voc.norm", st)) return r;
    for (int i = 0; i < v.layers; ++i) {
        const std::string p = "voc.blocks." + std::to_string(i);
        {
            Prof pr(c, VV_PROF_VOC_CONV, 2.0 * R * (double)V * v.dw_k, 8.0 * R * V, st);
            KCHK(c, vvk_dwconv(res, t, c->Wf(p + ".dwconv.weight"), c->Wf(p + ".dwconv.bias"), lens, B, B, T_max, V, v.dw_k, st, &m__));
        }
        if (int r = vocos_ln(c, t, hn, R, p + ".norm", st)) return r;
        const std::string w1 = p + ".pwconv1.weight", b1 = p + ".pwconv1.bias", w2 = p + ".pwconv2.weight", b2 = p + ".pwconv2.bias";
        if (int r = launch_gemm(c, vocos_gemm(c, VV_EPI_STORE, VV_ACT_GELU_ERF_, hn, V, w1.c_str(), b1.c_str(), big, I, R, I, V), VV_PROF_VOC_CONV, st)) return r;
        Gemm g2 = vocos_gemm(c, VV_EPI_GATE_RES, VV_ACT_NONE_, big, I, w2.c_str(), b2.c_str(), res, V, R, V, I);
        g2.gate = c->Wf(p + ".gamma");
        if (int r = launch_gemm(c, g2, VV_PROF_VOC_CONV, st)) return r;
    }
    if (int r = vocos_ln(c, res, hn, R, "voc.final_norm", st)) return r;
    Gemm head = vocos_gemm(c, VV_EPI_STORE, VV_ACT_NONE_, hn, V, "voc.head.weight", "voc.head.bias", big, HP, R, HP, V);
    head.n_store = v.n_fft + 2;
    if (int r = launch_gemm(c, head, VV_PROF_VOC_POST, st)) return r;
    return vocos_istft(c, B, T_max, big, HP, lens, pcm, ld_pcm, pcm_len, wave_f32, spec, big, st);
}

static int decode_impl(vv_ctx* c, int B, int N, const float* x, const int32_t* ref_len, const int32_t* seq_len, int t_gen_max, int16_t* pcm,
                       int ld_pcm, int32_t* pcm_len, float* wave_f32, void* ext_ws, uint64_t ext_bytes, void* stream) {
    if (!c) return -22;
    if (!c->finalized) return c->fail(-1, "vv_decode: weights not finalized");
    if (B < 1 || N < 1 || !x || !ref_len || !seq_len || !pcm || !pcm_len || t_gen_max < 1 || t_gen_max > N)
        return c->fail(-22, "vv_decode: bad arguments");
    const vv_model_cfg& g = c->cfg;
    if (ld_pcm < t_gen_max * g.hop_length) return c->fail(-22, "vv_decode: ld_pcm too small");
    hipSetDevice(c->device);
    hipStream_t st = (hipStream_t)stream;
    if (c->vocos) return decode_vocos(c, B, N, x, ref_len, seq_len, t_gen_max, pcm, ld_pcm, pcm_len, wave_f32, ext_ws, ext_bytes, st);
    const int M = g.n_mel, nu = g.voc_n_up;
    const HifiPlan plan = hifi_plan(g, t_gen_max);
    const int *Ts = plan.Ts, *Cs = plan.Cs;
    HifiBufs w;
    if (int r = plan_ws(c, ext_ws, (size_t)ext_bytes, [&](Arena& a) { w = hifi_bufs(a, g, plan, B); })) return r;
    auto [v0, buf, lens] = w;

    KCHK(c, vvk_decode_len(seq_len, ref_len, lens, B, nu + 1, c->d_mult, N, Ts[0], st, &m__));
    HIPCHK(c, hipMemcpyAsync(pcm_len, lens + (size_t)nu * B, sizeof(int) * B, hipMemcpyDeviceToDevice, st));
    {
        Prof p(c, VV_PROF_ELEMWISE, 0, 8.0 * B * M * Ts[0], st);
        KCHK(c, vvk_mel_slice(x, B, N, M, ref_len, seq_len, v0, Ts[0], st, &m__));
    }
    const bool x3 = c->voc_x3 == 1 || (c->voc_x3 < 0 && c->dt == VV_DTYPE_BF16);
    auto conv = [&](const float* in, const std::string& name, float* out, const float* resid, int Cin, int Cout, int T_in, int T_out, int KW,
                    int dil, int up, float pre_slope, float scale, int accumulate, const int* len_in, int stage_cls) -> int {
        vv_conv_args a{};
        a.in = in; a.W = c->Wf(name + ".weight"); a.bias = c->Wf(name + ".bias"); a.out = out; a.resid = resid;
        if (x3) {
            auto it = c->x3_w.find(name + ".weight");
            if (it == c->x3_w.end()) return c->fail(-2, "split weights of %s missing", name.c_str());
            a.W_x3 = it->second; a.wg_rows = c->voc_x3_rows;
        }
        a.B = B; a.Cin = Cin; a.Cout = Cout; a.T_in = T_in; a.T_out = T_out; a.KW = KW; a.dil = dil; a.transposed = up > 0; a.up = up;
        a.rows_total = up > 0 ? Cout * up : Cout; a.rows_pad = pad_to(a.rows_total, 64); a.accumulate = accumulate;
        a.pre_slope = pre_slope; a.out_scale = scale; a.len_in = len_in;
        const double taps = up > 0 ? 2.0 : (double)KW;
        Prof p(c, VV_PROF_VOC_CONV, 2.0 * B * (double)T_out * Cout * Cin * taps,
               4.0 * B * ((double)Cin * T_in + (double)Cout * T_out * (1 + (resid ? 1 : 0) + (accumulate ? 1 : 0))), st, stage_cls);
        const char* m = "";
        int r = vvk_conv(&a, st, &m);
        if (r) return c->fail(r, "%s (%s)", m, name.c_str());
        return 0;
    };
    if (int r = conv(v0, "voc.pre", buf[0], nullptr, M, Cs[0], Ts[0], Ts[0], g.voc_pre_k, 1, 0, 1.0f, 1.0f, 0, lens, VV_PROF_VOC_PRE)) return r;
    float* cur = buf[0];
    float* up_out = buf[1];
    for (int s = 0; s < nu; ++s) {
        const int C = Cs[s + 1], T = Ts[s + 1];
        const int* len_s = lens + (size_t)(s + 1) * B;
        if (int r = conv(cur, "voc.up." + std::to_string(s), up_out, nullptr, Cs[s], C, Ts[s], T, 2, 1, g.voc_up_rates[s], g.voc_lrelu, 1.0f, 0, lens + (size_t)s * B,
                         s < 4 ? VV_PROF_VOC_UP0 + s : -1)) return r;
        float* acc = cur;
        float* t1 = (up_out == buf[1]) ? buf[2] : buf[1];
        float* ya = buf[3];
        float* yb = buf[4];
        const float inv = 1.0f / (float)g.voc_n_res;
        const int mrf_cls = s < 4 ? VV_PROF_VOC_MRF0 + s : -1;
        for (int a = 0; a < g.voc_n_res; ++a) {
            const float* y = up_out;
            for (int b = 0; b < g.voc_n_dil; ++b) {
                const std::string q = "voc.res." + std::to_string(s) + "." + std::to_string(a) + "." + std::to_string(b);
                const bool last = b == g.voc_n_dil - 1;
                float* dst = last ? acc : ((y == ya) ? yb : ya);
                const int kw = g.voc_res_kernels[a], dil = g.voc_res_dilations[b];
                if ((c->fuse_mrf == 1 || (c->fuse_mrf == 2 && B <= 8 && !x3)) && (C == 32 || C == 64) && (kw == 3 || kw == 7 || kw == 11)) {
                    vv_mrf_args m{};
                    m.y = y; m.W1 = c->Wf(q + ".conv1.weight"); m.b1 = c->Wf(q + ".conv1.bias"); m.W2 = c->Wf(q + ".conv2.weight"); m.b2 = c->Wf(q + ".conv2.bias");
                    m.out = dst; m.B = B; m.C = C; m.T = T; m.KW = kw; m.dil = dil; m.rows_pad = 64; m.accumulate = last && a > 0;
                    m.slope = g.voc_lrelu; m.out_scale = last ? inv : 1.0f; m.len_in = len_s;
                    Prof p(c, VV_PROF_VOC_CONV, 2.0 * 2.0 * B * (double)T * C * C * kw, 4.0 * B * (double)C * T * (2 + (m.accumulate ? 1 : 0)), st, mrf_cls);
                    const char* em = "";
                    if (int r = vvk_mrf_pair(&m, st, &em)) return c->fail(r, "%s (%s)", em, q.c_str());
                } else {
                    if (int r = conv(y, q + ".conv1", t1, nullptr, C, C, T, T, kw, dil, 0, g.voc_lrelu, 1.0f, 0, len_s, mrf_cls)) return r;
                    if (int r = conv(t1, q + ".conv2", dst, y, C, C, T, T, kw, 1, 0, g.voc_lrelu, last ? inv : 1.0f, last && a > 0, len_s, mrf_cls)) return r;
                }
                y = dst;
            }
        }
    }
    {
        const int C = Cs[nu], T = Ts[nu];
        Prof p(c, VV_PROF_VOC_POST, 2.0 * B * (double)T * C * g.voc_post_k, 4.0 * B * (double)C * T + 2.0 * B * T, st);
        KCHK(c, vvk_conv_post(cur, c->Wf("voc.post.weight"), c->post_bias, pcm, ld_pcm, wave_f32, B, C, T, g.voc_post_k, 0.01f,
                              lens + (size_t)nu * B, st, &m__));
    }
    return 0;
}

int vv_set_rope_theta(vv_ctx* c, float theta) {
    if (!c) return -22;
    if (theta != 0.f && !(theta > 1.f)) return c->fail(-22, "vv_set_rope_theta: the base must be > 1 (0 = read the tables)");
    c->rope_theta = theta;
    return 0;
}

int vv_set_option(vv_ctx* c, const char* name, int value) {
    if (!c || !name) return -22;
    if (!strcmp(name, "rope_rows")) { c->rope_rows = value != 0; return 0; }
    if (!strcmp(name, "rope_q_attn")) { c->rope_q_attn = value != 0; return 0; }
    if (!strcmp(name, "voc_x3_rows")) {
        if (value != 0 && value != 128) return c->fail(-22, "vv_set_option: voc_x3_rows takes 0 (64-row workgroups) or 128");
        c->voc_x3_rows = value; return 0;
    }
    if (!strcmp(name, "voc_x3")) {
        if (value < -1 || value > 1) return c->fail(-22, "vv_set_option: voc_x3 takes -1 (by acoustic dtype), 0 (f32 MFMA) or 1 (3-way bf16 split)");
        c->voc_x3 = value; return 0;
    }
    if (!strcmp(name, "split_k_tail")) {
        if (value < 0 || value > 2) return c->fail(-22, "vv_set_option: split_k_tail takes 0 (off), 1 (out-projection and FF2) or 2 (FF2 only)");
        c->split_k_tail = value; return 0;
    }
    if (!strcmp(name, "ring_tiles")) { c->ring_tiles = value != 0; if (value > 1) c->ring_tiles_max = value; return 0; }
    if (!strcmp(name, "pp_min_tiles")) {
        if (value < -1) return c->fail(-22, "vv_set_option: pp_min_tiles takes -1 (the launcher's rule) or a 256-tile count >= 0");
        c->pp_min_tiles = value; return 0;
    }
    if (!strcmp(name, "lanes")) {
        if (value < 0 || value > 2) return c->fail(-22, "vv_set_option: lanes takes 0 (auto), 1 (one lane) or 2 (two lanes whenever the batch has two items)");
        c->lanes = value; return 0;
    }
    if (!strcmp(name, "fuse_mrf")) {
        if (value < 0 || value > 2) return c->fail(-22, "vv_set_option: fuse_mrf takes 0 (off), 1 (on) or 2 (auto)");
        c->fuse_mrf = value; return 0;
    }
    return c->fail(-22, "vv_set_option: unknown option '%s'", name);
}

int vv_decode(vv_ctx* c, int B, int N, const float* x, const int32_t* ref_len, const int32_t* seq_len, int t_gen_max, int16_t* pcm,
              int ld_pcm, int32_t* pcm_len, float* wave_f32, void* stream) {
    return decode_impl(c, B, N, x, ref_len, seq_len, t_gen_max, pcm, ld_pcm, pcm_len, wave_f32, nullptr, 0, stream);
}

int vv_decode_into(vv_ctx* c, int B, int N, const float* x, const int32_t* ref_len, const int32_t* seq_len, int t_gen_max, int16_t* pcm,
                   int ld_pcm, int32_t* pcm_len, float* wave_f32, void* ws, uint64_t ws_bytes, void* stream) {
    if (!c) return -22;
    if (!ws) return c->fail(-22, "vv_decode_into: null workspace block");
    return decode_impl(c, B, N, x, ref_len, seq_len, t_gen_max, pcm, ld_pcm, pcm_len, wave_f32, ws, ws_bytes, stream);
}

int vv_prof_enable(vv_ctx* c, int on) {
    if (!c) return -22;
    c->prof = on != 0;
    return 0;
}
int vv_prof_collect(vv_ctx* c, int64_t* launches, double* ms, double* flops, double* bytes) {
    if (!c) return -22;
    hipSetDevice(c->device);
    HIPCHK(c, hipDeviceSynchronize());
    for (auto& r : c->recs) {
        float t = 0.f;
        if (hipEventElapsedTime(&t, r.a, r.b) == hipSuccess) { c->p_ms[r.cls] += t; if (r.sub >= 0) c->p_ms[r.sub] += t; }
        c->pool.push_back(r.a); c->pool.push_back(r.b);
    }
    c->recs.clear();
    for (int i = 0; i < VV_PROF_NCLASS; ++i) {
        if (launches) launches[i] = c->p_launch[i];
        if (ms) ms[i] = c->p_ms[i];
        if (flops) flops[i] = c->p_flops[i];
        if (bytes) bytes[i] = c->p_bytes[i];
        c->p_launch[i] = 0; c->p_ms[i] = 0; c->p_flops[i] = 0; c->p_bytes[i] = 0;
    }
    return 0;
}

#define SINGLE(ctx, call)                                     \
    do {                                                      \
        if (!(ctx)) return -22;                               \
        hipSetDevice((ctx)->device);                          \
        const char* m__ = "";                                 \
        int r__ = (call);                                     \
        if (r__) return (ctx)->fail(r__, "%s", m__);          \
        return 0;                                             \
    } while (0)

int vv_gemm(vv_ctx* c, const vv_gemm_args* a, void* st) { SINGLE(c, vvk_gemm(a, (hipStream_t)st, &m__)); }
int vv_gemm_tail_plan(vv_ctx* c, int32_t M, int32_t N, int32_t K, int32_t* row0, int32_t* parts) {
    if (!row0 || !parts || M < 1 || N < 1 || K < 1) return c ? c->fail(-22, "vv_gemm_tail_plan: bad arguments") : -22;
    if (c) HIPCHK(c, hipSetDevice(c->device));
    vvk_gemm_tail_plan(M, N, K, K, K, N, row0, parts);
    return 0;
}
int vv_attention(vv_ctx* c, const vv_attn_args* a, void* st) { SINGLE(c, vvk_attention(a, (hipStream_t)st, &m__)); }
int vv_layernorm(vv_ctx* c, const vv_ln_args* a, void* st) { SINGLE(c, vvk_ln_mod(a, (hipStream_t)st, &m__)); }
int vv_posconv(vv_ctx* c, const vv_posconv_args* a, void* st) { SINGLE(c, vvk_posconv(a, (hipStream_t)st, &m__)); }
int vv_conv1d(vv_ctx* c, const vv_conv_args* a, void* st) { SINGLE(c, vvk_conv(a, (hipStream_t)st, &m__)); }
uint64_t vv_conv_split_bytes(int32_t Cin_pad, int32_t KW, int32_t rows_pad) {
    return (Cin_pad < 1 || KW < 1 || rows_pad < 1) ? 0 : (uint64_t)vvk_conv_split_bytes(Cin_pad, KW, rows_pad);
}
int vv_conv_split_weights(vv_ctx* c, const float* W, int32_t Cin_pad, int32_t KW, int32_t rows_pad, void* out, void* st) {
    SINGLE(c, vvk_conv_split_weights(W, Cin_pad, KW, rows_pad, out, (hipStream_t)st, &m__));
}
int vv_mrf_resblock(vv_ctx* c, const vv_mrf_args* a, void* st) { SINGLE(c, vvk_mrf_pair(a, (hipStream_t)st, &m__)); }
int vv_conv_post(vv_ctx* c, const float* in, const float* w, float bias, int16_t* pcm, int ld_pcm, float* wave_f32, int B, int C, int T,
                 int KW, float pre_slope, const int32_t* len_in, void* st) {
    SINGLE(c, vvk_conv_post(in, w, bias, pcm, ld_pcm, wave_f32, B, C, T, KW, pre_slope, len_in, (hipStream_t)st, &m__));
}
int vv_mel(vv_ctx* c, const int16_t* audio, int ld_audio, const int32_t* audio_len, float* mel, int B, int F_max, void* st) {
    if (!c) return -22;
    if (!c->W("const.window") || !c->W("const.tw_cos") || !c->W("const.tw_sin") || !c->W("const.mel_fb"))
        return c->fail(-2, "vv_mel: constant tables not bound");
    SINGLE(c, vvk_mel(audio, ld_audio, audio_len, c->Wf("const.window"), c->Wf("const.tw_cos"), c->Wf("const.tw_sin"), c->Wf("const.mel_fb"),
                      mel, B, F_max, c->cfg.n_fft, c->cfg.hop_length, c->cfg.n_mel, (hipStream_t)st, &m__));
}
int vv_groupnorm(vv_ctx* c, const float* x, float* y, const float* gamma, const float* beta, int B, int C, int T, int G, float eps, int act, void* st) {
    SINGLE(c, vvk_groupnorm(x, y, gamma, beta, B, C, T, G, eps, act, (hipStream_t)st, &m__));
}
int vv_rope_rows(vv_ctx* c, const float* compact, const int32_t* pos, float* out, int rows, void* st) {
    SINGLE(c, vvk_rope_rows(compact, pos, out, rows, (hipStream_t)st, &m__));
}
int vv_rope_compact(vv_ctx* c, const float* cos_t, const float* sin_t, float* out, int n, void* st) {
    SINGLE(c, vvk_rope_compact(cos_t, sin_t, out, n, (hipStream_t)st, &m__));
}
int vv_resample_poly(vv_ctx* c, const float* x, int n_in, const double* taps, int n_taps, int up, int down, int skip, float* y, int n_out, void* st) {
    SINGLE(c, vvk_resample_poly(x, n_in, taps, n_taps, up, down, skip, y, n_out, (hipStream_t)st, &m__));
}
int vv_ingest_pcm(vv_ctx* c, const void* pcm, const int64_t* desc, int n_clips, int64_t max_out, float* out, void* st) {
    SINGLE(c, vvk_ingest_pcm(pcm, (const long long*)desc, n_clips, (long long)max_out, out, (hipStream_t)st, &m__));
}
size_t vv_normalize_scratch_bytes(int n_clips, int64_t total_len) { return vvk_normalize_scratch_bytes(n_clips, (long long)total_len); }
int vv_normalize_clips(vv_ctx* c, const float* x, const int64_t* offsets, int n_clips, int64_t max_len, void* scratch, int16_t* out, void* st) {
    SINGLE(c, vvk_normalize_clips(x, (const long long*)offsets, n_clips, (long long)max_len, scratch, out, (hipStream_t)st, &m__));
}
int vv_vocos_im2col(vv_ctx* c, const float* x, int B, int N, const int32_t* ref_len, const int32_t* seq_len, int T_max, float* out, int ld_out,
                    void* st) {
    if (c && !c->vocos) return c->fail(-22, "vv_vocos_im2col: not a Vocos context (vv_set_vocos)");
    SINGLE(c, vvk_vocos_im2col(x, B, N, c->cfg.n_mel, ref_len, seq_len, T_max, c->vcfg.embed_k, out, ld_out, (hipStream_t)st, &m__));
}
int vv_istft_head(vv_ctx* c, int B, int T_max, const float* head, int ld_head, const int32_t* n_frames, int16_t* pcm, int ld_pcm, int32_t* pcm_len,
                  float* wave_f32, void* stream) {
    if (!c) return -22;
    if (!c->vocos || !c->finalized) return c->fail(-22, "vv_istft_head: needs a finalized Vocos context");
    if (B < 1 || T_max < 1 || !head || !n_frames || !pcm || ld_head < c->vcfg.n_fft + 2 || ld_pcm < T_max * c->vcfg.hop_length)
        return c->fail(-22, "vv_istft_head: bad arguments (ld_head >= n_fft + 2, ld_pcm >= T_max * hop)");
    if ((size_t)B * T_max * c->vcfg.n_fft * 4 >= ((size_t)1 << 31)) return c->fail(-22, "vv_istft_head: a plane of 2 GiB or more");
    hipSetDevice(c->device);
    const size_t R = (size_t)B * T_max;
    float *spec, *frames;
    if (int r = plan_ws(c, nullptr, 0, [&](Arena& a) { spec = a.take<float>(R * c->vcfg.n_fft); frames = a.take<float>(R * c->vcfg.n_fft); })) return r;
    return vocos_istft(c, B, T_max, head, ld_head, n_frames, pcm, ld_pcm, pcm_len, wave_f32, spec, frames, (hipStream_t)stream);
}
int vv_ode_stage(vv_ctx* c, const vv_ode_stage_args* a, void* st) {
    if (!c || !a) return c ? c->fail(-22, "vv_ode_stage: null arguments") : -22;
    SINGLE(c, vvk_ode_stage(a, nullptr, nullptr, (hipStream_t)st, &m__));
}
int vv_ode_stage_guided(vv_ctx* c, const vv_ode_stage_args* a, const int32_t* u_row, void* st) {
    if (!c || !a) return c ? c->fail(-22, "vv_ode_stage_guided: null arguments") : -22;
    if ((uintptr_t)u_row % 4) return c->fail(-22, "vv_ode_stage_guided: u_row must be an int32 array");
    SINGLE(c, vvk_ode_stage(a, u_row, nullptr, (hipStream_t)st, &m__));
}
int vv_ode_stage_apg(vv_ctx* c, const vv_ode_stage_args* a, const int32_t* u_row, const vv_apg_stage_args* apg, void* st) {
    if (!apg) return vv_ode_stage_guided(c, a, u_row, st);
    if (!c || !a) return c ? c->fail(-22, "vv_ode_stage_apg: null arguments") : -22;
    if ((uintptr_t)u_row % 4) return c->fail(-22, "vv_ode_stage_apg: u_row must be an int32 array");
    SINGLE(c, vvk_ode_stage(a, u_row, apg, (hipStream_t)st, &m__));
}
int vv_ode_stage_reuse(vv_ctx* c, const vv_ode_stage_args* a, const int32_t* u_row, const vv_reuse_stage_args* reuse, void* st) {
    if (!reuse) return vv_ode_stage_guided(c, a, u_row, st);
    if (!c || !a) return c ? c->fail(-22, "vv_ode_stage_reuse: null arguments") : -22;
    if ((uintptr_t)u_row % 4) return c->fail(-22, "vv_ode_stage_reuse: u_row must be an int32 array");
    SINGLE(c, vvk_ode_stage(a, u_row, nullptr, (hipStream_t)st, &m__, 0, reuse));
}
int vv_cfg_drift_reduce(vv_ctx* c, const vv_cfg_drift_args* a, void* st) {
    if (!c || !a) return c ? c->fail(-22, "vv_cfg_drift_reduce: null arguments") : -22;
    if (((uintptr_t)a->u_row | (uintptr_t)a->row_start | (uintptr_t)a->len) % 4) return c->fail(-22, "vv_cfg_drift_reduce: the index arrays must be 4-byte aligned");
    SINGLE(c, vvk_cfg_drift_reduce(a, 3, (hipStream_t)st, &m__));
}
int vv_ode_diff_reduce(vv_ctx* c, const vv_ode_diff_args* a, void* st) {
    if (!c || !a) return c ? c->fail(-22, "vv_ode_diff_reduce: null arguments") : -22;
    if (((uintptr_t)a->row_start | (uintptr_t)a->len) % 4) return c->fail(-22, "vv_ode_diff_reduce: the index arrays must be 4-byte aligned");
    SINGLE(c, vvk_ode_diff_reduce(a, 3, (hipStream_t)st, &m__));
}
int vv_apg_coef(vv_ctx* c, const vv_apg_coef_args* a, void* st) {
    if (!c || !a) return c ? c->fail(-22, "vv_apg_coef: null arguments") : -22;
    if (((uintptr_t)a->u_row | (uintptr_t)a->row_src | (uintptr_t)a->row_start | (uintptr_t)a->len | (uintptr_t)a->g_item | (uintptr_t)a->eta |
         (uintptr_t)a->norm_rms) % 4)
        return c->fail(-22, "vv_apg_coef: the index and item arrays must be 4-byte aligned");
    SINGLE(c, vvk_apg_coef(a, 3, (hipStream_t)st, &m__));
}
int vv_text_embed(vv_ctx* c, const int32_t* ids, int ld_ids, const int32_t* text_len, const float* emb, const float* pos, int vocab_rows,
                  float* out, int B, int N, int Dt, void* st) {
    if (!c) return -22;
    if (!ids || !text_len || !emb || !pos || !out || B < 1 || N < 1 || ld_ids < 1 || vocab_rows < 1 || Dt < 4 || Dt % 4)
        return c->fail(-22, "vv_text_embed: bad arguments (B, N, ld_ids, vocab_rows >= 1, Dt a multiple of 4)");
    if (((uintptr_t)emb | (uintptr_t)pos | (uintptr_t)out) % 16 || ((uintptr_t)ids | (uintptr_t)text_len) % 4)
        return c->fail(-22, "vv_text_embed: emb, pos and out must be 16-byte aligned, ids and text_len 4-byte");
    SINGLE(c, vvk_text_embed(ids, ld_ids, text_len, emb, pos, out, B, N, Dt, vocab_rows, (hipStream_t)st, &m__));
}
int vv_dwconv(vv_ctx* c, const float* in, float* out, const float* w, const float* bias, const int32_t* seq_len, int B, int n_seq, int N, int C,
              int KW, void* st) {
    if (!c) return -22;
    if (!in || !out || !w || !bias || in == out || n_seq < 1 || N < 1 || C < 4 || C % 4 || KW < 1 || !(KW & 1) || (seq_len && B < 1))
        return c->fail(-22, "vv_dwconv: bad arguments (out a buffer of its own, C a multiple of 4, KW odd, B >= 1 with seq_len)");
    if (((uintptr_t)in | (uintptr_t)out | (uintptr_t)bias) % 16 || ((uintptr_t)w | (uintptr_t)seq_len) % 4)
        return c->fail(-22, "vv_dwconv: in, out and bias must be 16-byte aligned, w and seq_len 4-byte");
    SINGLE(c, vvk_dwconv(in, out, w, bias, seq_len, seq_len ? B : 1, n_seq, N, C, KW, (hipStream_t)st, &m__));
}
int vv_grn(vv_ctx* c, int dtype, void* x, float* sumsq, const float* gamma, const float* beta, const int32_t* seq_len, int B, int n_seq, int N,
           int C, void* st) {
    if (!c) return -22;
    if ((dtype != VV_DTYPE_F32 && dtype != VV_DTYPE_BF16) || !x || !sumsq || !gamma || !beta || n_seq < 1 || N < 1 || C < 64 || C % 64 || C > 8192 ||
        (seq_len && B < 1))
        return c->fail(-22, "vv_grn: bad arguments (dtype f32 / bf16, C a multiple of 64 up to 8192, B >= 1 with seq_len)");
    if ((uintptr_t)x % (dtype == VV_DTYPE_BF16 ? 8 : 16) || (uintptr_t)beta % 16 || ((uintptr_t)sumsq | (uintptr_t)gamma | (uintptr_t)seq_len) % 4)
        return c->fail(-22, "vv_grn: x must be aligned to 4 elements, beta to 16 bytes, sumsq, gamma and seq_len to 4");
    SINGLE(c, vvk_grn(dtype, x, sumsq, gamma, beta, seq_len, seq_len ? B : 1, n_seq, N, C, (hipStream_t)st, &m__));
}
int vv_cfg_euler(vv_ctx* c, float* x, const float* pred, int ldp, int BN, int n_mel, float cfg, float dt, void* st) {
    SINGLE(c, vvk_cfg_euler(x, pred, ldp, BN, n_mel, cfg, dt, nullptr, (hipStream_t)st, &m__));
}
#define ALIGN4(ctx, name, ptrs)                                                                                   \
    do {                                                                                                              \
        if (!(ctx)) return -22;                                                                                       \
        if ((ptrs) % 4) return (ctx)->fail(-22, name ": every array must be 4-byte aligned");                    \
    } while (0)
int vv_cfg_euler_rows(vv_ctx* c, float* x, const float* pred, int ldp, int BN, int n_mel, float cfg, float dt, const int32_t* row_src, void* st) {
    ALIGN4(c, "vv_cfg_euler_rows", (uintptr_t)row_src);
    SINGLE(c, vvk_cfg_euler(x, pred, ldp, BN, n_mel, cfg, dt, row_src, (hipStream_t)st, &m__));
}
int vv_pack_cat(vv_ctx* c, int dtype, const float* x, const float* cat, const float* cat_drop, void* out, int ldo, int BN, int n_mel, int cond_dim,
                int only_x, const int32_t* row_src, void* st) {
    ALIGN4(c, "vv_pack_cat", (uintptr_t)row_src);
    if (dtype != VV_DTYPE_F32 && dtype != VV_DTYPE_BF16) return c->fail(-22, "vv_pack_cat: dtype must be VV_DTYPE_F32 or VV_DTYPE_BF16");
    SINGLE(c, vvk_pack_cat(dtype, x, cat, cat_drop, out, ldo, BN, n_mel, cond_dim, only_x, row_src, (hipStream_t)st, &m__));
}
int vv_pack_cat_guided(vv_ctx* c, int dtype, const float* x, const float* cat, const float* cat_drop, void* out, int ldo, int Rc, int row0,
                       int n_rows, int n_mel, int cond_dim, int only_x, int x_packed, const int32_t* row_src, const int32_t* u_src,
                       const int32_t* u_crow, void* st) {
    ALIGN4(c, "vv_pack_cat_guided", (uintptr_t)row_src | (uintptr_t)u_src | (uintptr_t)u_crow);
    if (dtype != VV_DTYPE_F32 && dtype != VV_DTYPE_BF16) return c->fail(-22, "vv_pack_cat_guided: dtype must be VV_DTYPE_F32 or VV_DTYPE_BF16");
    SINGLE(c, vvk_pack_cat_guided(dtype, x, cat, cat_drop, out, ldo, Rc, row0, n_rows, n_mel, cond_dim, only_x, x_packed, row_src, u_src, u_crow,
                                  (hipStream_t)st, &m__));
}
int vv_row_tables(vv_ctx* c, const int32_t* seq_len, int B, int N, int Rc, int32_t* row_start, int32_t* row_src, int32_t* row_pos, int32_t* kv_len,
                  void* st) {
    ALIGN4(c, "vv_row_tables", (uintptr_t)seq_len | (uintptr_t)row_start | (uintptr_t)row_src | (uintptr_t)row_pos | (uintptr_t)kv_len);
    if (!seq_len || !row_start || !row_src || !row_pos || !kv_len) return c->fail(-22, "vv_row_tables: seq_len and the four tables are required");
    if ((long long)B * N >= (1ll << 31)) return c->fail(-22, "vv_row_tables: B * N must stay below 2^31 (row_src holds b * N + t)");
    SINGLE(c, vvk_row_tables(seq_len, B, N, Rc, row_start, row_src, row_pos, kv_len, (hipStream_t)st, &m__));
}
int vv_guided_tables(vv_ctx* c, const int32_t* seq_len, const uint8_t* guided, int B, int N, int Rc, int Ru, int32_t* row_start, int32_t* rs_rel,
                     int32_t* kv_len, int32_t* row_pos, int32_t* u_src, int32_t* u_crow, int32_t* u_row, void* st) {
    ALIGN4(c, "vv_guided_tables", (uintptr_t)seq_len | (uintptr_t)row_start | (uintptr_t)rs_rel | (uintptr_t)kv_len | (uintptr_t)row_pos |
                                          (uintptr_t)u_src | (uintptr_t)u_crow | (uintptr_t)u_row);
    if (!seq_len || !row_start || !rs_rel || !kv_len || !row_pos || !u_src || !u_crow || !u_row)
        return c->fail(-22, "vv_guided_tables: seq_len and the seven tables are required");
    if ((long long)B * N >= (1ll << 31)) return c->fail(-22, "vv_guided_tables: B * N must stay below 2^31 (u_src holds b * N + t)");
    SINGLE(c, vvk_guided_tables(seq_len, guided, B, N, Rc, Ru, row_start, rs_rel, kv_len, row_pos, u_src, u_crow, u_row, (hipStream_t)st, &m__));
}
int vv_ref_len(vv_ctx* c, const int32_t* audio_len, int32_t* ref_len, int B, int hop, void* st) {
    ALIGN4(c, "vv_ref_len", (uintptr_t)audio_len | (uintptr_t)ref_len);
    SINGLE(c, vvk_ref_len(audio_len, ref_len, B, hop, (hipStream_t)st, &m__));
}
int vv_decode_len(vv_ctx* c, const int32_t* seq_len, const int32_t* ref_len, int32_t* lens, int B, int n_levels, const int32_t* mult, int N, int T_max,
                  void* st) {
    ALIGN4(c, "vv_decode_len", (uintptr_t)seq_len | (uintptr_t)ref_len | (uintptr_t)lens | (uintptr_t)mult);
    SINGLE(c, vvk_decode_len(seq_len, ref_len, lens, B, n_levels, mult, N, T_max, (hipStream_t)st, &m__));
}
int vv_vocos_lens(vv_ctx* c, const int32_t* seq_len, const int32_t* ref_len, int32_t* lens, int B, int N, int T_max, void* st) {
    ALIGN4(c, "vv_vocos_lens", (uintptr_t)seq_len | (uintptr_t)ref_len | (uintptr_t)lens);
    SINGLE(c, vvk_vocos_lens(seq_len, ref_len, lens, B, N, T_max, (hipStream_t)st, &m__));
}
int vv_mel_slice(vv_ctx* c, const float* x, int B, int N, int n_mel, const int32_t* ref_len, const int32_t* seq_len, float* out, int T, void* st) {
    ALIGN4(c, "vv_mel_slice", (uintptr_t)ref_len | (uintptr_t)seq_len | (uintptr_t)x | (uintptr_t)out);
    SINGLE(c, vvk_mel_slice(x, B, N, n_mel, ref_len, seq_len, out, T, (hipStream_t)st, &m__));
}
int vv_vocos_im2col_ex(vv_ctx* c, const float* x, int B, int N, int n_mel, const int32_t* ref_len, const int32_t* seq_len, int T_max, int k, float* out,
                       int ld_out, void* st) {
    ALIGN4(c, "vv_vocos_im2col_ex", (uintptr_t)ref_len | (uintptr_t)seq_len);
    SINGLE(c, vvk_vocos_im2col(x, B, N, n_mel, ref_len, seq_len, T_max, k, out, ld_out, (hipStream_t)st, &m__));
}
int vv_vocos_spectrum(vv_ctx* c, const float* head, int ld_head, int R, int n_fft, float* out, void* st) {
    if (!c) return -22;
    if (((uintptr_t)head | (uintptr_t)out) % 4) return c->fail(-22, "vv_vocos_spectrum: head and out must be 4-byte aligned");
    SINGLE(c, vvk_vocos_spectrum(head, ld_head, R, n_fft, out, (hipStream_t)st, &m__));
}
int vv_vocos_ola(vv_ctx* c, const float* frames, int ld_f, int B, int T_max, const int32_t* lens, const float* window, int n_fft, int hop,
                 int16_t* pcm, int ld_pcm, int32_t* pcm_len, float* wave, int ld_wave, void* st) {
    ALIGN4(c, "vv_vocos_ola", (uintptr_t)lens | (uintptr_t)pcm_len | (uintptr_t)frames | (uintptr_t)window | (uintptr_t)wave);
    if ((uintptr_t)pcm % 2) return c->fail(-22, "vv_vocos_ola: pcm must be 2-byte aligned");
    if (n_fft < 2 || n_fft % 2) return c->fail(-22, "vv_vocos_ola: n_fft must be even and at least 2");
    SINGLE(c, vvk_vocos_ola(frames, ld_f, B, T_max, lens, window, n_fft, hop, pcm, ld_pcm, pcm_len, wave, ld_wave, (hipStream_t)st, &m__));
}
#undef ALIGN4

}
```

vietvoice-tts_amd/csrc/vv_elementwise.hip:

```cpp
#ifndef VV_ELEMENTWISE_HOST_CHECK
#include "vv_common.h"
#include "vv_kernels.h"
#endif
#include <type_traits>

namespace {

template <typename T> __device__ __forceinline__ float4 round4_as(float4 a) {
    if constexpr (sizeof(T) == 2) {
        typedef __attribute__((ext_vector_type(4))) float f4v;
        const f4v r = __builtin_convertvector(__builtin_convertvector((f4v){a.x, a.y, a.z, a.w}, bf16x4), f4v);
        return make_float4(r[0], r[1], r[2], r[3]);
    } else {
        return a;
    }
}

template <typename To, typename Td>
__global__ __launch_bounds__(256) void ln_mod_kernel(float* __restrict__ x, int ldx, To* __restrict__ y, int ldy,
                                                     int R, int D, const float* __restrict__ w,
                                                     const float* __restrict__ b, int add_one, float eps,
                                                     const Td* __restrict__ delta, int ldd, const Td* __restrict__ delta2,
                                                     int keep_x, int tail_row0, int tp1, const float* __restrict__ dt1, int tp2,
                                                     const float* __restrict__ dt2) {
// ... 391 lines not shown
            dv[0] = p.x; dv[1] = p.y; dv[2] = p.z; dv[3] = p.w;
        }
#pragma unroll
        for (int j = 0; j < 4; ++j) {
            const double v = (double)dn[j];
            if (old) {
                const double d = v - (double)dv[j];
                const double dd = d * d;
                s1 = s1 + dd;
            }
            const double vv = v * v;
            s2 = s2 + vv;
        }
    }
    red[0][threadIdx.x] = s1; red[1][threadIdx.x] = s2;
    __syncthreads();
    for (int w = 128; w > 0; w >>= 1) {
        if ((int)threadIdx.x < w) {
            red[0][threadIdx.x] += red[0][threadIdx.x + w];
            red[1][threadIdx.x] += red[1][threadIdx.x + w];
        }
        __syncthreads();
    }
    if (threadIdx.x < 2) partials[((size_t)b * n_tiles + tile) * 2 + threadIdx.x] = red[threadIdx.x][0];
}

__global__ __launch_bounds__(256) void text_embed_kernel(const int* __restrict__ ids, int ld_ids,
                                                         const int* __restrict__ text_len, const float* __restrict__ emb,
                                                         const float* __restrict__ pos, float* __restrict__ out, int B,
                                                         int N, int Dt, int vocab_rows) {
    const int c4 = Dt >> 2;
    const size_t total = (size_t)2 * B * N * c4;
    for (size_t i = (size_t)blockIdx.x * 256 + threadIdx.x; i < total; i += (size_t)gridDim.x * 256) {
        const int c = (int)(i % c4) * 4;
        const size_t row = i / c4;
        const int t = (int)(row % N);
        const int s = (int)(row / N);
        const int b = s % B;
        int id = 0;
        if (s < B && t < text_len[b] && t < ld_ids) id = ids[(size_t)b * ld_ids + t] + 1;
        id = min(max(id, 0), vocab_rows - 1);
        const float4 e = *(const float4*)(emb + (size_t)id * Dt + c);
        const float4 p = *(const float4*)(pos + (size_t)t * Dt + c);
        *(float4*)(out + row * Dt + c) = make_float4(e.x + p.x, e.y + p.y, e.z + p.z, e.w + p.w);
    }
}

__global__ __launch_bounds__(256) void dwconv_kernel(const float* __restrict__ in, float* __restrict__ out,
                                                     const float* __restrict__ w , const float* __restrict__ bias,
                                                     const int* __restrict__ seq_len, int B, int n_seq, int N, int C, int KW) {
    const int c4 = C >> 2;
    const size_t total = (size_t)n_seq * N * c4;
    const int pad = KW / 2;
    for (size_t i = (size_t)blockIdx.x * 256 + threadIdx.x; i < total; i += (size_t)gridDim.x * 256) {
        const int c = (int)(i % c4) * 4;
        const size_t row = i / c4;
        const int t = (int)(row % N);
        const int s = (int)(row / N);
        const int len = seq_len ? min(seq_len[s % B], N) : N;
        float4 acc = *(const float4*)(bias + c);
        for (int k = 0; k < KW; ++k) {
            const int tt = t + k - pad;
            if (tt < 0 || tt >= len) continue;
            const float4 v = *(const float4*)(in + ((size_t)s * N + tt) * C + c);
            acc.x += w[(c + 0) * KW + k] * v.x;
            acc.y += w[(c + 1) * KW + k] * v.y;
            acc.z += w[(c + 2) * KW + k] * v.z;
            acc.w += w[(c + 3) * KW + k] * v.w;
        }
        *(float4*)(out + row * C + c) = acc;
    }
}

template <typename T>
__global__ __launch_bounds__(256) void grn_stats_kernel(const T* __restrict__ x, float* __restrict__ sumsq,
                                                        const int* __restrict__ seq_len, int B, int N, int C) {
    __shared__ float red[256];
    const int s = blockIdx.y;
    const int c = blockIdx.x * 64 + (threadIdx.x & 63);
    const int ph = threadIdx.x >> 6;
    const int len = seq_len ? min(seq_len[s % B], N) : N;
    float acc = 0.f;
    for (int t = ph; t < len; t += 4) {
        const float v = to_f32<T>(x[((size_t)s * N + t) * C + c]);
        acc += v * v;
    }
    red[threadIdx.x] = acc;
    __syncthreads();
    if (ph == 0) sumsq[(size_t)s * C + c] = (red[threadIdx.x] + red[threadIdx.x + 64]) + (red[threadIdx.x + 128] + red[threadIdx.x + 192]);
}

template <typename T>
__global__ __launch_bounds__(256) void grn_apply_kernel(T* __restrict__ x, const float* __restrict__ sumsq,
                                                        const float* __restrict__ gamma, const float* __restrict__ beta,
                                                        int N, int C, int rows_per_block) {
#ifndef VV_ELEMENTWISE_HOST_CHECK
    extern __shared__ float sc[];
#else
    float* sc = (float*)vv_host::dynamic_lds();
#endif
    __shared__ float red[4];
    const int s = blockIdx.y;
    float part = 0.f;
    for (int c = threadIdx.x; c < C; c += 256) part += sqrtf(sumsq[(size_t)s * C + c]);
    part = wave_sum(part);
    if ((threadIdx.x & 63) == 0) red[threadIdx.x >> 6] = part;
    __syncthreads();
    const float mean = ((red[0] + red[1]) + (red[2] + red[3])) / (float)C;
    for (int c = threadIdx.x; c < C; c += 256) sc[c] = gamma[c] * (sqrtf(sumsq[(size_t)s * C + c]) / (mean + 1e-6f)) + 1.0f;
    __syncthreads();
    const int t0 = blockIdx.x * rows_per_block;
    const int c4 = C >> 2;
    for (int i = threadIdx.x; i < rows_per_block * c4; i += 256) {
        const int t = t0 + i / c4;
        if (t >= N) break;
        const int c = (i % c4) * 4;
        T* p = x + ((size_t)s * N + t) * C + c;
        const float4 v = load4<T>(p);
        const float4 bb = *(const float4*)(beta + c);
        store4<T>(p, v.x * sc[c] + bb.x, v.y * sc[c + 1] + bb.y, v.z * sc[c + 2] + bb.z, v.w * sc[c + 3] + bb.w);
    }
}

template <bool MASKED>
__global__ __launch_bounds__(256) void build_cat_kernel(const float* __restrict__ mel, int F_max,
                                                        const int* __restrict__ ref_len, const float* __restrict__ text,
                                                        float* __restrict__ cat, float* __restrict__ cat_drop, int B, int N,
                                                        int n_mel, int Dt, const uint8_t* __restrict__ keep, int ld_keep) {
    const int cd = n_mel + Dt;
    const int c4 = cd >> 2;
    const size_t total = (size_t)B * N * c4;
    for (size_t i = (size_t)blockIdx.x * 256 + threadIdx.x; i < total; i += (size_t)gridDim.x * 256) {
        const int c = (int)(i % c4) * 4;
        const size_t row = i / c4;
        const int t = (int)(row % N);
        const int b = (int)(row / N);
        float4 v, vd;
        if (c < n_mel) {
            v = (t < ref_len[b] && t < F_max && (!MASKED || keep[(size_t)b * ld_keep + t])) ? *(const float4*)(mel + ((size_t)b * F_max + t) * n_mel + c)
                                               : make_float4(0.f, 0.f, 0.f, 0.f);
            vd = make_float4(0.f, 0.f, 0.f, 0.f);
        } else {
            v = *(const float4*)(text + row * Dt + (c - n_mel));
            vd = *(const float4*)(text + ((size_t)B * N + row) * Dt + (c - n_mel));
        }
        *(float4*)(cat + row * cd + c) = v;
        *(float4*)(cat_drop + row * cd + c) = vd;
    }
}

__global__ void ref_len_kernel(const int* __restrict__ audio_len, int* __restrict__ ref_len, int B, int hop) {
    const int b = blockIdx.x * 64 + threadIdx.x;
    if (b < B) ref_len[b] = audio_len[b] / hop + 1;
}
__global__ void decode_len_kernel(const int* __restrict__ seq_len, const int* __restrict__ ref_len, int* __restrict__ lens,
                                  int B, int n_levels, const int* __restrict__ mult, int N, int T_max) {
    const int b = blockIdx.x * 64 + threadIdx.x;
    if (b >= B) return;
    const int sl = max(min(seq_len[b], N), 0);
    const int tg = min(sl - min(max(ref_len[b], 0), sl), T_max);
    for (int l = 0; l < n_levels; ++l) lens[l * B + b] = tg * mult[l];
}

__global__ __launch_bounds__(256) void row_tables_kernel(const int* __restrict__ seq_len, int B, int N, int Rc, int* __restrict__ row_start,
                                                         int* __restrict__ row_src, int* __restrict__ row_pos, int* __restrict__ kv_len) {
    const int b = blockIdx.x;
    int r0 = 0;
    for (int i = 0; i < b; ++i) r0 += min(max(seq_len[i], 0), N);
    r0 = min(r0, Rc);
    const int len = min(min(max(seq_len[b], 0), N), Rc - r0);
    if (threadIdx.x == 0) { row_start[b] = r0; row_start[B + b] = Rc + r0; kv_len[b] = len; kv_len[B + b] = len; }
    for (int t = threadIdx.x; t < len; t += 256) {
        row_src[r0 + t] = b * N + t;
        row_pos[r0 + t] = t;
        row_pos[Rc + r0 + t] = t;
    }
    if (b == B - 1)
        for (int t = r0 + len + (int)threadIdx.x; t < Rc; t += 256) {
            const int p = min(len + (t - (r0 + len)), N - 1);
            row_src[t] = b * N + p;
            row_pos[t] = p;
            row_pos[Rc + t] = p;
        }
}

__global__ __launch_bounds__(256) void guided_tables_kernel(const int* __restrict__ seq_len, GuideFlags flags, int B, int N, int Rc, int Ru,
                                                            int* __restrict__ row_start, int* __restrict__ rs_rel, int* __restrict__ kv_len,
                                                            int* __restrict__ row_pos, int* __restrict__ u_src, int* __restrict__ u_crow,
                                                            int* __restrict__ u_row) {
    const int b = blockIdx.x;
    int r0 = 0, u0 = 0, j = 0;
    for (int i = 0; i < b; ++i) {
        const int li = min(min(max(seq_len[i], 0), N), Rc - r0);
        r0 += li;
        if ((flags.w[i >> 5] >> (i & 31)) & 1u) { u0 += min(li, Ru - u0); ++j; }
    }
    const int len = min(min(max(seq_len[b], 0), N), Rc - r0);
    const bool guided = (flags.w[b >> 5] >> (b & 31)) & 1u;
    const int ulen = guided ? min(len, Ru - u0) : 0;
    if (threadIdx.x == 0) {
        row_start[b] = r0; kv_len[b] = len;
        if (guided) { row_start[B + j] = Rc + u0; rs_rel[j] = u0; kv_len[B + j] = ulen; }
    }
    for (int t = threadIdx.x; t < len; t += 256) {
        row_pos[r0 + t] = t;
        u_row[r0 + t] = t < ulen ? Rc + u0 + t : -1;
    }
    for (int t = threadIdx.x; t < ulen; t += 256) {
        row_pos[Rc + u0 + t] = t;
        u_src[u0 + t] = b * N + t;
        u_crow[u0 + t] = r0 + t;
    }
    if (b == B - 1) {
        for (int t = r0 + len + (int)threadIdx.x; t < Rc; t += 256) {
            row_pos[t] = min(len + (t - (r0 + len)), N - 1);
            u_row[t] = -1;
        }
        for (int t = u0 + ulen + (int)threadIdx.x; t < Ru; t += 256) {
            const int p = min(len + (t - (u0 + ulen)), N - 1);
            row_pos[Rc + t] = p;
            u_src[t] = b * N + p;
            u_crow[t] = Rc - 1;
        }
    }
}

__global__ __launch_bounds__(256) void groupnorm_kernel(const float* __restrict__ x, float* __restrict__ y,
                                                        const float* __restrict__ gamma, const float* __restrict__ beta,
                                                        int C, int T, int G, float eps, int act) {
    __shared__ float red[3][4];
    const int b = blockIdx.y, g = blockIdx.x;
    const int cpg = C / G;
    const size_t n = (size_t)cpg * T;
    const float* xs = x + ((size_t)b * C + (size_t)g * cpg) * T;
    float* ys = y + ((size_t)b * C + (size_t)g * cpg) * T;
    const bool vec = (T & 3) == 0 && (((uintptr_t)xs | (uintptr_t)ys) & 15) == 0;
    const size_t n4 = n >> 2;
    float s0 = 0.f;
    if (vec) {
        for (size_t i = threadIdx.x; i < n4; i += 256) {
            const float4 v = *(const float4*)(xs + i * 4);
            s0 += (v.x + v.y) + (v.z + v.w);
        }
    } else {
        for (size_t i = threadIdx.x; i < n; i += 256) s0 += xs[i];
    }
    s0 = wave_sum(s0);
    if ((threadIdx.x & 63) == 0) red[0][threadIdx.x >> 6] = s0;
    __syncthreads();
    const float m0 = ((red[0][0] + red[0][1]) + (red[0][2] + red[0][3])) / (float)n;
    float s = 0.f, q = 0.f;
    if (vec) {
        for (size_t i = threadIdx.x; i < n4; i += 256) {
            const float4 v = *(const float4*)(xs + i * 4);
            const float a0 = v.x - m0, a1 = v.y - m0, a2 = v.z - m0, a3 = v.w - m0;
            s += (a0 + a1) + (a2 + a3);
            q += (a0 * a0 + a1 * a1) + (a2 * a2 + a3 * a3);
        }
    } else {
        for (size_t i = threadIdx.x; i < n; i += 256) { const float d = xs[i] - m0; s += d; q += d * d; }
    }
    s = wave_sum(s); q = wave_sum(q);
    if ((threadIdx.x & 63) == 0) { red[1][threadIdx.x >> 6] = s; red[2][threadIdx.x >> 6] = q; }
    __syncthreads();
    const float sd = ((red[1][0] + red[1][1]) + (red[1][2] + red[1][3])) / (float)n;
    const float var = fmaxf(((red[2][0] + red[2][1]) + (red[2][2] + red[2][3])) / (float)n - sd * sd, 0.f);
    const float mean = m0 + sd, rstd = rsqrtf(var + eps);
    if (vec) {
        const int t4 = T >> 2;
        for (size_t i = threadIdx.x; i < n4; i += 256) {
            const int c = g * cpg + (int)(i / t4);
            const float ga = (gamma ? gamma[c] : 1.f) * rstd, be = beta ? beta[c] : 0.f;
            const float4 v = *(const float4*)(xs + i * 4);
            float4 o;
            o.x = act_apply((v.x - mean) * ga + be, act); o.y = act_apply((v.y - mean) * ga + be, act);
            o.z = act_apply((v.z - mean) * ga + be, act); o.w = act_apply((v.w - mean) * ga + be, act);
            *(float4*)(ys + i * 4) = o;
        }
    } else {
        for (size_t i = threadIdx.x; i < n; i += 256) {
            const int c = g * cpg + (int)(i / T);
            ys[i] = act_apply((xs[i] - mean) * ((gamma ? gamma[c] : 1.f) * rstd) + (beta ? beta[c] : 0.f), act);
        }
    }
}

__global__ __launch_bounds__(256) void rope_compact_kernel(const float* __restrict__ c, const float* __restrict__ s, float* __restrict__ out, int n) {
    const int i = blockIdx.x * 256 + threadIdx.x;
    if (i >= n * 32) return;
    const int pos = i >> 5, pr = i & 31;
    out[(size_t)pos * 64 + 2 * pr] = c[(size_t)pos * 64 + 2 * pr];
    out[(size_t)pos * 64 + 2 * pr + 1] = s[(size_t)pos * 64 + 2 * pr];
}

__global__ __launch_bounds__(256) void rope_rows_kernel(const float* __restrict__ cs, const int* __restrict__ pos, float* __restrict__ out, int rows) {
    const size_t i = (size_t)blockIdx.x * 256 + threadIdx.x;
    if (i >= (size_t)rows * 16) return;
    const size_t r = i >> 4;
    const int q = (int)(i & 15);
    *(float4*)(out + r * 64 + q * 4) = *(const float4*)(cs + (size_t)pos[r] * 64 + q * 4);
}

#ifndef VV_ELEMENTWISE_HOST_CHECK
inline int grid_for(size_t total) { return (int)std::min<size_t>((total + 255) / 256, 256 * 8); }
#endif

}

#ifndef VV_ELEMENTWISE_HOST_CHECK
#define VVK_CHECK_LAUNCH()                                               \
    do {                                                                 \
        hipError_t he__ = hipGetLastError();                             \
        if (he__ != hipSuccess) { *err = hipGetErrorString(he__); return -5; } \
    } while (0)

int vvk_ln_mod(const vv_ln_args* a, hipStream_t st, const char** err) {
    if (a->R <= 0) { *err = "ln: empty"; return -22; }
    if (a->D < 4 || a->D % 4 || a->D > 1024 || a->ldx % 4 || a->ldy % 4) { *err = "ln: D must be a multiple of 4 within [4, 1024]"; return -22; }
    if (a->ldx < a->D || a->ldy < a->D) { *err = "ln: ldx and ldy must be at least D"; return -22; }
    if (a->delta && (a->ld_delta % 4 || a->ld_delta < a->D)) { *err = "ln: bad delta leading dimension"; return -22; }
    if (a->delta2 && !a->delta) { *err = "ln: delta2 without delta"; return -22; }
    const int grid = (a->R + 3) / 4;
    float* x = const_cast<float*>(a->x);
    const bool ob = a->out_dtype == VV_BF16, db = a->delta_dtype == VV_BF16;
    const int tp1 = a->delta && a->delta_tail_parts > 1 ? a->delta_tail_parts : 0, tp2 = a->delta2 && a->delta2_tail_parts > 1 ? a->delta2_tail_parts : 0;
    if ((tp1 || tp2) && (((uintptr_t)a->delta_tail | (uintptr_t)a->delta2_tail) % 16)) { *err = "ln: split-K tail buffers must be 16-byte aligned"; return -22; }
    if ((a->delta_tail_parts > 1 && !a->delta) || (a->delta2_tail_parts > 1 && !a->delta2)) { *err = "ln: a delta tail without its delta"; return -22; }
    if ((tp1 || tp2) && (a->tail_row0 < 0 || a->tail_row0 >= a->R || (tp1 && !a->delta_tail) || (tp2 && !a->delta2_tail) || tp1 > 8 || tp2 > 8)) {
        *err = "ln: bad split-K tail (row0 within [0, R), buffers given, at most 8 parts)"; return -22;
    }
    const int tail_row0 = (tp1 || tp2) ? a->tail_row0 : a->R;
#define LN_GO(To, Td) ln_mod_kernel<To, Td><<<grid, 256, 0, st>>>(x, a->ldx, (To*)a->y, a->ldy, a->R, a->D, a->w, a->b, a->add_one, a->eps, (const Td*)a->delta, a->ld_delta, (const Td*)a->delta2, a->keep_x, tail_row0, tp1, (const float*)a->delta_tail, tp2, (const float*)a->delta2_tail)
    if (ob && db) LN_GO(bf16, bf16);
    else if (ob) LN_GO(bf16, float);
    else if (db) LN_GO(float, bf16);
    else LN_GO(float, float);
#undef LN_GO
    VVK_CHECK_LAUNCH();
    return 0;
}

int vvk_pack_cat(int dtype, const float* x, const float* cat, const float* cat_drop, void* out, int ldo, int BN, int n_mel,
                 int cond_dim, int only_x, const int* row_src, hipStream_t st, const char** err) {
    if (n_mel % 4 || cond_dim % 4 || ldo % 4 || ldo < n_mel + cond_dim) { *err = "pack_cat: bad widths"; return -22; }
    if (BN < 1 || n_mel < 4 || cond_dim < 0) { *err = "pack_cat: BN >= 1, n_mel >= 4, cond_dim >= 0"; return -22; }
    if (!x || !out || (!only_x && cond_dim > 0 && (!cat || !cat_drop))) { *err = "pack_cat: x, out and (unless only_x) cat and cat_drop are required"; return -22; }
    if (((uintptr_t)x | (uintptr_t)cat | (uintptr_t)cat_drop) % 16 || (uintptr_t)out % (dtype == VV_BF16 ? 8 : 16)) {
        *err = "pack_cat: x, cat and cat_drop must be 16-byte aligned, out 16-byte (f32) or 8-byte (bf16)"; return -22;
    }
    const size_t total = (size_t)2 * BN * ((only_x ? n_mel : ldo) / 4);
    if (dtype == VV_BF16)
        pack_cat_kernel<bf16><<<grid_for(total), 256, 0, st>>>(x, cat, cat_drop, (bf16*)out, ldo, BN, n_mel, cond_dim, only_x, row_src);
    else
        pack_cat_kernel<float><<<grid_for(total), 256, 0, st>>>(x, cat, cat_drop, (float*)out, ldo, BN, n_mel, cond_dim, only_x, row_src);
    VVK_CHECK_LAUNCH();
    return 0;
}

int vvk_cfg_euler(float* x, const float* pred, int ldp, int BN, int n_mel, float cfg, float dt, const int* row_src, hipStream_t st,
                  const char** err) {
    if (n_mel % 4 || ldp % 4) { *err = "cfg_euler: widths must be multiples of 4"; return -22; }
    if (BN < 1 || n_mel < 4 || ldp < n_mel) { *err = "cfg_euler: BN >= 1, n_mel >= 4, ldp >= n_mel"; return -22; }
    if (!x || !pred) { *err = "cfg_euler: x and pred are required"; return -22; }
    if (((uintptr_t)x | (uintptr_t)pred) % 16) { *err = "cfg_euler: x and pred must be 16-byte aligned"; return -22; }
    cfg_euler_kernel<<<grid_for((size_t)BN * n_mel / 4), 256, 0, st>>>(x, pred, ldp, BN, n_mel, cfg, dt, row_src);
    VVK_CHECK_LAUNCH();
    return 0;
}

int vvk_ode_stage(const vv_ode_stage_args* a, const int* u_row, const vv_apg_stage_args* apg, hipStream_t st, const char** err, int k_out_ring,
                  const vv_reuse_stage_args* reuse) {
    if (a->n_mel < 4 || a->n_mel % 4 || a->ldp % 4 || a->ldp < a->n_mel || a->Rc < 1) { *err = "ode_stage: widths must be multiples of 4, ldp >= n_mel, Rc >= 1"; return -22; }
    if (!a->x || !a->pred || a->n_prev < 0 || a->n_prev > 3) { *err = "ode_stage: x, pred and 0..3 earlier slopes"; return -22; }
    if (a->g_item && a->seq_n < 1) { *err = "ode_stage: g_item needs the padded sequence length seq_n"; return -22; }
    uintptr_t al = (uintptr_t)a->x | (uintptr_t)a->pred | (uintptr_t)a->k_out | (uintptr_t)a->x_out;
    OdeStagePrev pv{};
    for (int j = 0; j < a->n_prev; ++j) {
        if (!(a->coef[j] == a->coef[j]) || !(a->coef[a->n_prev] == a->coef[a->n_prev])) { *err = "ode_stage: NaN coefficient"; return -22; }
        if (a->coef[j] == 0.f) continue;
        if (!a->k_prev[j]) { *err = "ode_stage: a non-zero coefficient without its slope buffer"; return -22; }
        pv.k[j] = a->k_prev[j]; pv.c[j] = a->coef[j];
        al |= (uintptr_t)a->k_prev[j];
        if ((a->k_prev[j] == a->k_out && !k_out_ring) || a->k_prev[j] == a->x_out) { *err = "ode_stage: an output aliases an earlier slope"; return -22; }
    }
    if (al % 16) { *err = "ode_stage: buffers must be 16-byte aligned"; return -22; }
    if (a->x_out && (a->x_out == a->x || a->x_out == a->k_out)) { *err = "ode_stage: x_out must be a buffer of its own"; return -22; }
    if (apg) {
        if (!apg->coef || !apg->x_e || a->seq_n < 1) { *err = "ode_stage: APG needs coef, x_e and the padded sequence length seq_n"; return -22; }
        if (((uintptr_t)apg->coef % 8) || ((uintptr_t)apg->x_e % 16)) { *err = "ode_stage: APG coef must be 8-byte and x_e 16-byte aligned"; return -22; }
        if (apg->x_e == a->x_out || apg->x_e == a->k_out) { *err = "ode_stage: APG x_e aliases an output of the launch"; return -22; }
        if (!(apg->t_e == apg->t_e)) { *err = "ode_stage: NaN evaluation time"; return -22; }
    }
    const int grid = grid_for((size_t)a->Rc * a->n_mel / 4);
    const float omt = apg ? 1.0f - apg->t_e : 0.f;
    if (reuse) {
        if (apg || !u_row) { *err = "ode_stage: the reuse form needs u_row and is not combined with APG"; return -22; }
        if (!reuse->d_buf || (uintptr_t)reuse->d_buf % 16 || !reuse->item_mode_host) { *err = "ode_stage: d_buf (16-byte aligned) and the item modes are required"; return -22; }
        if (a->seq_n < 1 || reuse->n_items < 1 || reuse->n_items > VVK_GUIDE_MAX_ITEMS) { *err = "ode_stage: the reuse form needs seq_n and 1..1024 item modes"; return -22; }
        if (reuse->d_buf == a->k_out || reuse->d_buf == a->x_out || reuse->d_buf == a->x) { *err = "ode_stage: d_buf must be a buffer of its own"; return -22; }
        for (int j = 0; j < 3; ++j)
            if (pv.k[j] == reuse->d_buf) { *err = "ode_stage: d_buf must be a buffer of its own"; return -22; }
        OdeStageReuse ru{};
        ru.d_buf = reuse->d_buf;
        for (int b = 0; b < reuse->n_items; ++b) {
            if (reuse->item_mode_host[b] & ~3u) { *err = "ode_stage: an item mode is VV_REUSE_LOAD | VV_REUSE_STORE at the most"; return -22; }
            if (reuse->item_mode_host[b] & VV_REUSE_LOAD) ru.load.w[b >> 5] |= 1u << (b & 31);
            if (reuse->item_mode_host[b] & VV_REUSE_STORE) ru.store.w[b >> 5] |= 1u << (b & 31);
        }
        ode_stage_kernel<true, false, true><<<grid, 256, 0, st>>>(a->x, a->pred, a->ldp, a->Rc, a->n_mel, a->g, a->g_item, a->seq_n, a->row_src, pv,
                                                                   a->coef[a->n_prev], a->k_out, a->x_out, u_row, nullptr, nullptr, 0, omt, ru);
        VVK_CHECK_LAUNCH();
        return 0;
    }
#define STAGE_GO(G, A) ode_stage_kernel<G, A><<<grid, 256, 0, st>>>(a->x, a->pred, a->ldp, a->Rc, a->n_mel, a->g, a->g_item, a->seq_n, a->row_src, pv, \
        a->coef[a->n_prev], a->k_out, a->x_out, u_row, apg ? apg->coef : nullptr, apg ? apg->x_e : nullptr, apg ? apg->x_e_packed : 0, omt, OdeStageNoReuse{})
    if (apg) { if (u_row) STAGE_GO(true, true); else STAGE_GO(false, true); }
    else if (u_row) STAGE_GO(true, false);
    else STAGE_GO(false, false);
#undef STAGE_GO
    VVK_CHECK_LAUNCH();
    return 0;
}

int vvk_apg_coef(const vv_apg_coef_args* a, int which, hipStream_t st, const char** err) {
    if (a->n_mel < 4 || a->n_mel % 4 || a->ldp % 4 || a->ldp < a->n_mel || a->Rc < 1) { *err = "apg_coef: widths must be multiples of 4, ldp >= n_mel, Rc >= 1"; return -22; }
    if (!a->pred || !a->x_e || !a->row_start || !a->len || !a->partials || !a->coef) { *err = "apg_coef: pred, x_e, row_start, len, partials and coef are required"; return -22; }
    if (a->B < 1 || a->B > VVK_GUIDE_MAX_ITEMS || a->n_tiles < 1) { *err = "apg_coef: 1..1024 items, n_tiles >= 1"; return -22; }
    if (((uintptr_t)a->pred | (uintptr_t)a->x_e) % 16 || (uintptr_t)a->partials % 8 || (uintptr_t)a->coef % 8) { *err = "apg_coef: pred and x_e 16-byte, partials and coef 8-byte aligned"; return -22; }
    if (!(a->t_e == a->t_e)) { *err = "apg_coef: NaN evaluation time"; return -22; }
    const double omt = 1.0 - (double)a->t_e;
    if (which & 1) {
        apg_reduce_kernel<<<dim3(a->n_tiles, a->B), 256, 0, st>>>(a->pred, a->ldp, a->Rc, a->n_mel, a->u_row, a->x_e, a->row_src, a->row_start,
                                                                   a->len, a->n_tiles, omt, a->partials);
        VVK_CHECK_LAUNCH();
    }
    if (which & 2) {
        apg_coef_kernel<<<a->B, 64, 0, st>>>(a->partials, a->n_tiles, a->Rc, a->n_mel, a->u_row, a->row_start, a->len, omt, a->g, a->g_item,
                                             a->eta, a->norm_rms, a->coef);
        VVK_CHECK_LAUNCH();
    }
    return 0;
}

int vvk_ode_diff_reduce(const vv_ode_diff_args* a, int which, hipStream_t st, const char** err) {
    if (a->n_mel < 4 || a->n_mel % 4 || a->Rc < 1) { *err = "ode_diff_reduce: n_mel must be a multiple of 4, Rc >= 1"; return -22; }
    if (!a->f || !a->row_start || !a->len || !a->partials || !a->report) { *err = "ode_diff_reduce: f, row_start, len, partials and report are required"; return -22; }
    if (a->B < 1 || a->B > VVK_GUIDE_MAX_ITEMS || a->n_tiles < 1) { *err = "ode_diff_reduce: 1..1024 items, n_tiles >= 1"; return -22; }
    if (((uintptr_t)a->f | (uintptr_t)a->f_prev) % 16 || ((uintptr_t)a->partials | (uintptr_t)a->report) % 8) { *err = "ode_diff_reduce: f and f_prev 16-byte, partials and report 8-byte aligned"; return -22; }
    if (which & 1) {
        ode_diff_reduce_kernel<<<dim3(a->n_tiles, a->B), 256, 0, st>>>(a->f, a->f_prev, a->Rc, a->n_mel, a->row_start, a->len, a->n_tiles, a->partials);
        VVK_CHECK_LAUNCH();
    }
    if (which & 2) {
        ode_diff_finish_kernel<<<a->B, 64, 0, st>>>(a->partials, a->n_tiles, a->Rc, a->row_start, a->len, a->report);
        VVK_CHECK_LAUNCH();
    }
    return 0;
}

int vvk_cfg_drift_reduce(const vv_cfg_drift_args* a, int which, hipStream_t st, const char** err) {
    if (a->n_mel < 4 || a->n_mel % 4 || a->ldp % 4 || a->ldp < a->n_mel || a->Rc < 1) { *err = "cfg_drift_reduce: widths must be multiples of 4, ldp >= n_mel, Rc >= 1"; return -22; }
    if (!a->pred || !a->u_row || !a->row_start || !a->len || !a->partials || !a->report) { *err = "cfg_drift_reduce: pred, u_row, row_start, len, partials and report are required"; return -22; }
    if (a->B < 1 || a->B > VVK_GUIDE_MAX_ITEMS || a->n_tiles < 1) { *err = "cfg_drift_reduce: 1..1024 items, n_tiles >= 1"; return -22; }
    if (((uintptr_t)a->pred | (uintptr_t)a->d_buf) % 16 || ((uintptr_t)a->partials | (uintptr_t)a->report) % 8) { *err = "cfg_drift_reduce: pred and d_buf 16-byte, partials and report 8-byte aligned"; return -22; }
    GuideFlags old{};
    for (int b = 0; b < a->B && a->has_old_host; ++b)
        if (a->has_old_host[b]) old.w[b >> 5] |= 1u << (b & 31);
    if (a->has_old_host && !a->d_buf)
        for (unsigned w : old.w)
            if (w) { *err = "cfg_drift_reduce: an item with a stored difference needs d_buf"; return -22; }
    if (which & 1) {
        cfg_drift_reduce_kernel<<<dim3(a->n_tiles, a->B), 256, 0, st>>>(a->pred, a->ldp, a->Rc, a->n_mel, a->u_row, a->d_buf, old, a->row_start, a->len,
                                                                         a->n_tiles, a->partials);
        VVK_CHECK_LAUNCH();
    }
    if (which & 2) {
        ode_diff_finish_kernel<<<a->B, 64, 0, st>>>(a->partials, a->n_tiles, a->Rc, a->row_start, a->len, a->report);
        VVK_CHECK_LAUNCH();
    }
    return 0;
}

int vvk_pack_cat_guided(int dtype, const float* x, const float* cat, const float* cat_drop, void* out, int ldo, int Rc, int row0, int n_rows,
                        int n_mel, int cond_dim, int only_x, int x_packed, const int* row_src, const int* u_src, const int* u_crow,
                        hipStream_t st, const char** err) {
    if (n_mel % 4 || cond_dim % 4 || ldo % 4 || ldo < n_mel + cond_dim) { *err = "pack_cat_guided: bad widths"; return -22; }
    if (Rc < 1 || row0 < 0 || n_rows < 1 || !row_src || !u_src || !u_crow) { *err = "pack_cat_guided: rows and their three tables"; return -22; }
    if (n_mel < 4 || cond_dim < 0) { *err = "pack_cat_guided: n_mel >= 4, cond_dim >= 0"; return -22; }
    if (!x || !out || (!only_x && cond_dim > 0 && (!cat || !cat_drop))) { *err = "pack_cat_guided: x, out and (unless only_x) cat and cat_drop are required"; return -22; }
    if (((uintptr_t)x | (uintptr_t)cat | (uintptr_t)cat_drop) % 16 || (uintptr_t)out % (dtype == VV_BF16 ? 8 : 16)) {
        *err = "pack_cat_guided: x, cat and cat_drop must be 16-byte aligned, out 16-byte (f32) or 8-byte (bf16)"; return -22;
    }
    const size_t total = (size_t)n_rows * ((only_x ? n_mel : ldo) / 4);
    if (dtype == VV_BF16)
        pack_cat_guided_kernel<bf16><<<grid_for(total), 256, 0, st>>>(x, cat, cat_drop, (bf16*)out, ldo, Rc, row0, n_rows, n_mel, cond_dim, only_x,
                                                                      x_packed, row_src, u_src, u_crow);
    else
        pack_cat_guided_kernel<float><<<grid_for(total), 256, 0, st>>>(x, cat, cat_drop, (float*)out, ldo, Rc, row0, n_rows, n_mel, cond_dim, only_x,
                                                                       x_packed, row_src, u_src, u_crow);
    VVK_CHECK_LAUNCH();
    return 0;
}

int vvk_guided_tables(const int* seq_len, const unsigned char* flags, int B, int N, int Rc, int Ru, int* row_start, int* rs_rel, int* kv_len,
                      int* row_pos, int* u_src, int* u_crow, int* u_row, hipStream_t st, const char** err) {
    if (B < 1 || B > VVK_GUIDE_MAX_ITEMS || N < 1 || Rc < 1 || Ru < 0 || Ru > Rc || !flags) { *err = "guided_tables: 1..1024 items, 0 <= Ru <= Rc"; return -22; }
    GuideFlags f{};
    for (int b = 0; b < B; ++b)
        if (flags[b]) f.w[b >> 5] |= 1u << (b & 31);
    guided_tables_kernel<<<B, 256, 0, st>>>(seq_len, f, B, N, Rc, Ru, row_start, rs_rel, kv_len, row_pos, u_src, u_crow, u_row);
    VVK_CHECK_LAUNCH();
    return 0;
}

int vvk_text_embed(const int* ids, int ld_ids, const int* text_len, const float* emb, const float* pos, float* out, int B,
                   int N, int Dt, int vocab_rows, hipStream_t st, const char** err) {
    if (Dt % 4) { *err = "text_embed: Dt % 4"; return -22; }
    text_embed_kernel<<<grid_for((size_t)2 * B * N * Dt / 4), 256, 0, st>>>(ids, ld_ids, text_len, emb, pos, out, B, N, Dt, vocab_rows);
    VVK_CHECK_LAUNCH();
    return 0;
}

int vvk_dwconv(const float* in, float* out, const float* w, const float* bias, const int* seq_len, int B, int n_seq, int N,
               int C, int KW, hipStream_t st, const char** err) {
    if (C % 4) { *err = "dwconv: C % 4"; return -22; }
    dwconv_kernel<<<grid_for((size_t)n_seq * N * C / 4), 256, 0, st>>>(in, out, w, bias, seq_len, B, n_seq, N, C, KW);
    VVK_CHECK_LAUNCH();
    return 0;
}

int vvk_grn(int dtype, void* x, float* sumsq, const float* gamma, const float* beta, const int* seq_len, int B, int n_seq,
            int N, int C, hipStream_t st, const char** err) {
    if (C % 64 || C > 8192) { *err = "grn: C must be a multiple of 64"; return -22; }
    dim3 g1(C / 64, n_seq);
    const int rpb = 16;
    dim3 g2((N + rpb - 1) / rpb, n_seq);
    if (dtype == VV_BF16) {
        grn_stats_kernel<bf16><<<g1, 256, 0, st>>>((const bf16*)x, sumsq, seq_len, B, N, C);
        grn_apply_kernel<bf16><<<g2, 256, C * sizeof(float), st>>>((bf16*)x, sumsq, gamma, beta, N, C, rpb);
    } else {
        grn_stats_kernel<float><<<g1, 256, 0, st>>>((const float*)x, sumsq, seq_len, B, N, C);
        grn_apply_kernel<float><<<g2, 256, C * sizeof(float), st>>>((float*)x, sumsq, gamma, beta, N, C, rpb);
    }
    VVK_CHECK_LAUNCH();
    return 0;
}

int vvk_build_cat(const float* mel, int F_max, const int* ref_len, const float* text, float* cat, float* cat_drop, int B, int N,
                  int n_mel, int Dt, hipStream_t st, const char** err, const uint8_t* keep, int ld_keep) {
    if (n_mel % 4 || Dt % 4) { *err = "build_cat: widths % 4"; return -22; }
    if (keep && ld_keep < N) { *err = "build_cat: ld_keep < N"; return -22; }
    const int grid = grid_for((size_t)B * N * (n_mel + Dt) / 4);
    if (keep)
        build_cat_kernel<true><<<grid, 256, 0, st>>>(mel, F_max, ref_len, text, cat, cat_drop, B, N, n_mel, Dt, keep, ld_keep);
    else
        build_cat_kernel<false><<<grid, 256, 0, st>>>(mel, F_max, ref_len, text, cat, cat_drop, B, N, n_mel, Dt, nullptr, 0);
    VVK_CHECK_LAUNCH();
    return 0;
}

int vvk_ref_len(const int* audio_len, int* ref_len, int B, int hop, hipStream_t st, const char** err) {
    if (B < 1 || hop < 1 || !audio_len || !ref_len) { *err = "ref_len: B >= 1, hop >= 1, audio_len and ref_len required"; return -22; }
    ref_len_kernel<<<(B + 63) / 64, 64, 0, st>>>(audio_len, ref_len, B, hop);
    VVK_CHECK_LAUNCH();
    return 0;
}
int vvk_decode_len(const int* seq_len, const int* ref_len, int* lens, int B, int n_levels, const int* mult, int N, int T_max, hipStream_t st,
                   const char** err) {
    if (B < 1 || n_levels < 1 || N < 1 || T_max < 1 || !seq_len || !ref_len || !lens || !mult) {
        *err = "decode_len: B, n_levels, N, T_max >= 1, seq_len, ref_len, lens and mult required"; return -22;
    }
    decode_len_kernel<<<(B + 63) / 64, 64, 0, st>>>(seq_len, ref_len, lens, B, n_levels, mult, N, T_max);
    VVK_CHECK_LAUNCH();
    return 0;
}
int vvk_row_tables(const int* seq_len, int B, int N, int Rc, int* row_start, int* row_src, int* row_pos, int* kv_len, hipStream_t st, const char** err) {
    if (B <= 0 || N <= 0 || Rc <= 0) { *err = "row_tables: empty"; return -22; }
    row_tables_kernel<<<B, 256, 0, st>>>(seq_len, B, N, Rc, row_start, row_src, row_pos, kv_len);
    hipError_t he = hipGetLastError();
    if (he != hipSuccess) { *err = hipGetErrorString(he); return -5; }
    return 0;
}

int vvk_groupnorm(const float* x, float* y, const float* gamma, const float* beta, int B, int C, int T, int G, float eps, int act,
                  hipStream_t st, const char** err) {
    if (B <= 0 || C <= 0 || T <= 0 || G <= 0 || C % G) { *err = "groupnorm: C must be a multiple of G"; return -22; }
    dim3 grid(G, B);
    groupnorm_kernel<<<grid, 256, 0, st>>>(x, y, gamma, beta, C, T, G, eps, act);
    VVK_CHECK_LAUNCH();
    return 0;
}
int vvk_rope_rows(const float* cs, const int* pos, float* out, int rows, hipStream_t st, const char** err) {
    if (rows <= 0 || !cs || !pos || !out) { *err = "rope_rows: bad arguments"; return -22; }
    rope_rows_kernel<<<(unsigned)(((size_t)rows * 16 + 255) / 256), 256, 0, st>>>(cs, pos, out, rows);
    hipError_t he = hipGetLastError();
    if (he != hipSuccess) { *err = hipGetErrorString(he); return -5; }
    return 0;
}

int vvk_rope_compact(const float* c, const float* s, float* out, int n, hipStream_t st, const char** err) {
    if (n <= 0) { *err = "rope_compact: empty"; return -22; }
    rope_compact_kernel<<<(n * 32 + 255) / 256, 256, 0, st>>>(c, s, out, n);
    VVK_CHECK_LAUNCH();
    return 0;
}
#endif
```

vietvoice-tts_amd/csrc/vv_kernels.h:

```cpp
#pragma once
#include <hip/hip_runtime.h>
#include <algorithm>
#include "../../include/vvtts.h"

typedef vv_gemm_args vvk_gemm_args;

int vvk_gemm(const vv_gemm_args* g, hipStream_t st, const char** err);
void vvk_gemm_tail_plan(int M, int N, int K, int lda, int ldw, int ldc, int* row0, int* parts);
int vvk_attention(const vv_attn_args* a, hipStream_t st, const char** err);
int vvk_ln_mod(const vv_ln_args* a, hipStream_t st, const char** err);
int vvk_posconv(const vv_posconv_args* a, hipStream_t st, const char** err);
int vvk_conv(const vv_conv_args* a, hipStream_t st, const char** err);
int vvk_conv_x3(const vv_conv_args* a, hipStream_t st, const char** err);
size_t vvk_conv_split_bytes(int Cin_pad, int KW, int rows_pad);
int vvk_conv_split_weights(const float* Wt, int Cin_pad, int KW, int rows_pad, void* Wb, hipStream_t st, const char** err);
int vvk_mrf_pair(const vv_mrf_args* a, hipStream_t st, const char** err);
int vvk_conv_post(const float* in, const float* w, float bias, int16_t* pcm, int ld_pcm, float* wave_f32, int B, int C, int T,
                  int KW, float pre_slope, const int* len_in, hipStream_t st, const char** err);
int vvk_mel_slice(const float* x, int B, int N, int n_mel, const int* ref_len, const int* seq_len, float* out, int T,
                  hipStream_t st, const char** err);
int vvk_mel(const int16_t* audio, int ld_audio, const int* audio_len, const float* window, const float* tw_cos,
            const float* tw_sin, const float* fb, float* mel, int B, int F_max, int n_fft, int hop, int n_mel, hipStream_t st,
            const char** err);
int vvk_pack_cat(int dtype, const float* x, const float* cat, const float* cat_drop, void* out, int ldo, int BN, int n_mel,
                 int cond_dim, int only_x, const int* row_src, hipStream_t st, const char** err);
int vvk_cfg_euler(float* x, const float* pred, int ldp, int BN, int n_mel, float cfg, float dt, const int* row_src, hipStream_t st,
                  const char** err);
int vvk_ode_stage(const vv_ode_stage_args* a, const int* u_row, const vv_apg_stage_args* apg, hipStream_t st, const char** err, int k_out_ring = 0,
                  const vv_reuse_stage_args* reuse = nullptr);
int vvk_cfg_drift_reduce(const vv_cfg_drift_args* a, int which, hipStream_t st, const char** err);
int vvk_ode_diff_reduce(const vv_ode_diff_args* a, int which, hipStream_t st, const char** err);
int vvk_apg_coef(const vv_apg_coef_args* a, int which, hipStream_t st, const char** err);
#define VVK_GUIDE_MAX_ITEMS 1024
int vvk_guided_tables(const int* seq_len, const unsigned char* flags, int B, int N, int Rc, int Ru, int* row_start, int* rs_rel, int* kv_len,
                      int* row_pos, int* u_src, int* u_crow, int* u_row, hipStream_t st, const char** err);
int vvk_pack_cat_guided(int dtype, const float* x, const float* cat, const float* cat_drop, void* out, int ldo, int Rc, int row0, int n_rows,
                        int n_mel, int cond_dim, int only_x, int x_packed, const int* row_src, const int* u_src, const int* u_crow,
                        hipStream_t st, const char** err);
int vvk_text_embed(const int* ids, int ld_ids, const int* text_len, const float* emb, const float* pos, float* out, int B, int N,
                   int Dt, int vocab_rows, hipStream_t st, const char** err);
int vvk_dwconv(const float* in, float* out, const float* w, const float* bias, const int* seq_len, int B, int n_seq, int N, int C,
               int KW, hipStream_t st, const char** err);
int vvk_grn(int dtype, void* x, float* sumsq, const float* gamma, const float* beta, const int* seq_len, int B, int n_seq, int N,
            int C, hipStream_t st, const char** err);
int vvk_build_cat(const float* mel, int F_max, const int* ref_len, const float* text, float* cat, float* cat_drop, int B, int N,
                  int n_mel, int Dt, hipStream_t st, const char** err, const uint8_t* keep = nullptr, int ld_keep = 0);
int vvk_ref_len(const int* audio_len, int* ref_len, int B, int hop, hipStream_t st, const char** err);
int vvk_decode_len(const int* seq_len, const int* ref_len, int* lens, int B, int n_levels, const int* mult, int N, int T_max, hipStream_t st,
                   const char** err);
int vvk_row_tables(const int* seq_len, int B, int N, int Rc, int* row_start, int* row_src, int* row_pos, int* kv_len, hipStream_t st, const char** err);
int vvk_resample_poly(const float* x, int n_in, const double* h, int n_taps, int up, int down, int skip, float* y, int n_out,
                      hipStream_t st, const char** err);
int vvk_ingest_pcm(const void* pcm, const long long* desc, int n_clips, long long max_out, float* out, hipStream_t st, const char** err);
size_t vvk_normalize_scratch_bytes(int n_clips, long long total_len);
int vvk_normalize_clips(const float* x, const long long* off, int n_clips, long long max_len, void* scratch, int16_t* out,
                        hipStream_t st, const char** err);
int vvk_rope_compact(const float* c, const float* s, float* out, int n, hipStream_t st, const char** err);
int vvk_rope_rows(const float* cs, const int* pos, float* out, int rows, hipStream_t st, const char** err);
int vvk_groupnorm(const float* x, float* y, const float* gamma, const float* beta, int B, int C, int T, int G, float eps, int act,
                  hipStream_t st, const char** err);
int vvk_edit_splice(const int16_t* src, long long n_src, const long long* desc, int n_rows, int B, int16_t* out, int ld_out,
                    hipStream_t st, const char** err);
int vvk_edit_restore(float* x, const float* cat, const uint8_t* keep, int ld_keep, const int* seq_len, int B, int N, int n_mel, int cd,
                     hipStream_t st, const char** err);
int vvk_noise_fill(float* x, const int* seq_len, const unsigned long long* keys, int B, int N, int n_mel, int kind, hipStream_t st,
                   const char** err);
int vvk_join_max_n();
int vvk_join_chunks(const int16_t* pcm, long long n_pcm, const long long* chunk_rows, int n_chunks, const long long* req_rows, int R,
                    const double* fade, long long n_fade, int max_n, long long max_len, int16_t* out, long long n_out, void* ws,
                    hipStream_t st, const char** err);
int vvk_pcm_resample(const int16_t* x, long long n_x, const long long* rows, int n_rows, long long max_out, const double* taps, int n_taps,
                     int up, int down, int skip, int16_t* y, long long n_y, hipStream_t st, const char** err);
int vvk_pcm_encode(const int16_t* x, long long n_x, const long long* rows, int n_rows, long long max_n, int kind, uint8_t* y, long long n_y,
                   hipStream_t st, const char** err);
unsigned long long vvk_pcm_loudness_ws_bytes(long long total_runs, int R);
int vvk_pcm_loudness(const int16_t* x, long long n_x, const long long* rows, int R, long long sub, long long total_runs, long long max_n,
                     const double* tables, const double* params, int16_t* y, long long n_y, double* stats, void* ws, hipStream_t st,
                     const char** err);
int vvk_pcm_limit_tile(int L);
unsigned long long vvk_pcm_limit_ws_bytes(long long total_samples, long long total_tiles, int R);
int vvk_pcm_limit(const int16_t* x, long long n_x, const long long* rows, int R, int L, int mode, long long total_samples,
                  long long total_tiles, long long max_tiles, long long max_out, const double* window, const double* taps,
                  const double* params, const double* meas, int16_t* y, long long n_y, double* stats, void* ws, hipStream_t st,
                  const char** err);
unsigned long long vvk_pcm_stretch_ws_bytes(int R);
int vvk_pcm_stretch(const int16_t* x, long long n_x, const long long* rows, int R, long long max_out, const double* window, int16_t* y,
                    long long n_y, int* pos, long long n_pos, void* ws, hipStream_t st, const char** err);
unsigned long long vvk_pcm_formant_ws_bytes(long long total_frames, int R);
int vvk_pcm_formant(const int16_t* x, long long n_x, const int16_t* y, long long n_y, const long long* rows, int R, long long total_frames,
                    long long max_frames, const double* wa, const double* g, const double* window, int16_t* z, long long n_z, double* h_out,
                    void* ws, hipStream_t st, const char** err);
unsigned long long vvk_pcm_denoise_ws_bytes(int R);
int vvk_pcm_denoise(const int16_t* x, long long n_x, const long long* rows, int R, long long total_frames, long long max_hops, const double* strengths,
                    const double* bias, long long n_bias, const double* window, const double* twiddles, int16_t* y, long long n_y, double* mag_out,
                    void* ws, hipStream_t st, const char** err);
unsigned long long vvk_pcm_denoise_bias_ws_bytes(long long total_frames, int R);
int vvk_pcm_denoise_bias(const int16_t* x, long long n_x, const long long* rows, int R, long long total_frames, long long max_frames,
                         const double* window, const double* twiddles, double* out, void* ws, hipStream_t st, const char** err);
unsigned long long vvk_pcm_watermark_ws_bytes(int R);
int vvk_pcm_watermark(const int16_t* x, long long n_x, const long long* rows, int R, long long total_frames, long long max_hops, const int8_t* chips,
                      double gp, double gm, const double* window, const double* twiddles, int16_t* y, long long n_y, void* ws, hipStream_t st,
                      const char** err);
unsigned long long vvk_pcm_watermark_detect_ws_bytes(long long total_frames, int R);
int vvk_pcm_watermark_detect(const int16_t* x, long long n_x, const long long* rows, int R, long long total_frames, long long max_frames,
                             const int8_t* chips, const double* window, const double* twiddles, long long* stats, int* cells_out, void* ws,
                             hipStream_t st, const char** err);
unsigned long long vvk_flac_frame_bound(long long m);
unsigned long long vvk_pcm_flac_ws_bytes(long long total_frames, int R);
unsigned long long vvk_pcm_flac_lpc_ws_bytes(long long total_frames, int R);
int vvk_pcm_flac(const int16_t* x, long long n_x, const long long* rows, int R, int rate, int lpc_order, long long total_frames, long long max_frames,
                 uint8_t* y, long long n_y, long long* info, void* ws, hipStream_t st, const char** err);
unsigned long long vvk_flac_decode_frame_bound(int block, int channels, int bits);
unsigned long long vvk_flac_index_ws_bytes(long long n_bytes, int R);
unsigned long long vvk_flac_decode_ws_bytes(long long n_plane, long long total_frames);
int vvk_flac_index(const uint8_t* data, long long n_bytes, const long long* rows, int R, long long* info, void* ws, hipStream_t st, const char** err);
int vvk_flac_decode(const uint8_t* data, long long n_bytes, const long long* rows, int R, const long long* lay, long long total_frames,
                    long long total_samples, long long n_plane, int max_channels, void* ws, uint8_t* pcm, long long n_pcm, long long* info2, void* ws2,
                    hipStream_t st, const char** err);
int vvk_vocos_lens(const int* seq_len, const int* ref_len, int* lens, int B, int N, int T_max, hipStream_t st, const char** err);
int vvk_vocos_im2col(const float* x, int B, int N, int M, const int* ref_len, const int* seq_len, int T_max, int k, float* out, int ld_out,
                     hipStream_t st, const char** err);
int vvk_vocos_spectrum(const float* head, int ld_head, int R, int n_fft, float* out, hipStream_t st, const char** err);
int vvk_vocos_ola(const float* frames, int ld_f, int B, int T_max, const int* lens, const float* window, int n_fft, int hop, int16_t* pcm,
                  int ld_pcm, int32_t* pcm_len, float* wave, int ld_wave, hipStream_t st, const char** err);
```

vietvoice-tts_amd/csrc/vv_mel.hip:

```cpp
#ifndef VV_MEL_HOST_CHECK
#include "vv_common.h"
#include "vv_kernels.h"
#endif

namespace {

__global__ __launch_bounds__(256) void mel_kernel(const int16_t* __restrict__ audio, int ld_audio,
                                                  const int* __restrict__ audio_len, const float* __restrict__ window,
                                                  const float* __restrict__ tw_cos, const float* __restrict__ tw_sin,
                                                  const float* __restrict__ fb , float* __restrict__ mel,
                                                  int F_max, int n_fft, int hop, int n_mel) {
#ifndef VV_MEL_HOST_CHECK
    extern __shared__ __attribute__((aligned(16))) char smem[];
#else
    char* const smem = (char*)vv_host::dynamic_lds();
#endif
    float* fr = (float*)smem;
    float* tc = fr + n_fft;
    float* ts = tc + n_fft;
    float* mag = ts + n_fft;
    const int b = blockIdx.y, f = blockIdx.x;
    const int L = min(max(audio_len[b], 0), ld_audio);
    const int S = max(L, 1);
    const int frames = L / hop + 1;
    const int nb = n_fft / 2 + 1;
    if (f >= frames) {
        for (int m = threadIdx.x; m < n_mel; m += 256) mel[((size_t)b * F_max + f) * n_mel + m] = 0.f;
        return;
    }
    const int16_t* a = audio + (size_t)b * ld_audio;
    const int half = n_fft / 2;
    for (int n = threadIdx.x; n < n_fft; n += 256) {
        int pos = f * hop + n - half;
        if (pos < 0) pos = -pos;
        if (pos >= S) pos = 2 * (S - 1) - pos;
        pos = min(max(pos, 0), S - 1);
        fr[n] = (float)a[pos] * (1.0f / 32768.0f) * window[n];
        tc[n] = tw_cos[n];
        ts[n] = tw_sin[n];
    }
    __syncthreads();
    const int mask = n_fft - 1;
    for (int k = threadIdx.x; k < nb; k += 256) {
        float re = 0.f, im = 0.f;
        int idx = 0;
        for (int n = 0; n < n_fft; ++n) {
            const float x = fr[n];
            re = fmaf(x, tc[idx], re);
            im = fmaf(x, ts[idx], im);
            idx = (idx + k) & mask;
        }
        mag[k] = sqrtf(re * re + im * im);
    }
    __syncthreads();
    for (int m = threadIdx.x; m < n_mel; m += 256) {
        float acc = 0.f;
        for (int k = 0; k < nb; ++k) acc = fmaf(fb[(size_t)k * n_mel + m], mag[k], acc);
        mel[((size_t)b * F_max + f) * n_mel + m] = logf(fmaxf(acc, 1e-5f));
    }
}

}

#ifndef VV_MEL_HOST_CHECK
int vvk_mel(const int16_t* audio, int ld_audio, const int* audio_len, const float* window, const float* tw_cos, const float* tw_sin,
            const float* fb, float* mel, int B, int F_max, int n_fft, int hop, int n_mel, hipStream_t st, const char** err) {
    if (B <= 0 || F_max <= 0) { *err = "mel: empty"; return -22; }
    if (!audio || !audio_len || !mel || !window || !tw_cos || !tw_sin || !fb) { *err = "mel: audio, audio_len, mel and the four tables are required"; return -22; }
    if (ld_audio < 1 || hop < 1 || n_mel < 1) { *err = "mel: ld_audio, hop and n_mel must be at least 1"; return -22; }
    if (n_fft < 2 || n_fft & (n_fft - 1) || n_fft > 4096) { *err = "mel: n_fft must be a power of two within [2, 4096]"; return -22; }
    if (B > 65535) { *err = "mel: at most 65535 clips per launch (grid.y)"; return -22; }
    const size_t lds = (size_t)(3 * n_fft + n_fft / 2 + 1) * sizeof(float);
    dim3 grid(F_max, B);
    mel_kernel<<<grid, 256, lds, st>>>(audio, ld_audio, audio_len, window, tw_cos, tw_sin, fb, mel, F_max, n_fft, hop, n_mel);
    hipError_t he = hipGetLastError();
    if (he != hipSuccess) { *err = hipGetErrorString(he); return -5; }
    return 0;
}
#endif
```

Baseline: 184.4.

## Add direct multi-frame mel kernel, GEMM mel path, streaming dwconv/GRN, GELU tile

Adds a multi-frame direct DFT mel kernel, now the default. It also adds an optional fp32 GEMM path that multiplies frames by a precomputed DFT basis. Text and vocos depthwise conv and GRN stats get new streaming kernels that reuse a sliding register window and prefetch rows ahead. Large GELU-erf GEMMs are steered to a 64 tile. These changes target the preprocessing and vocoder stages, at the cost of more code paths and a different numeric order in the GEMM mel option.

```diff
diff --git a/vietvoice-tts_amd/csrc/vv_api.hip b/vietvoice-tts_amd/csrc/vv_api.hip
--- a/vietvoice-tts_amd/csrc/vv_api.hip
+++ b/vietvoice-tts_amd/csrc/vv_api.hip
@@ -66,6 +66,10 @@
     char* x3_buf = nullptr;
     std::map<std::string, const void*> x3_w;
     int fuse_mrf = 2;
+    int mel_form = 1;
+    float* mel_basis = nullptr;
+    int text_stream = 1;
+    int gelu_erf_tile = 1;
     bool prof = false;
     std::vector<ProfRec> recs;
     std::vector<hipEvent_t> pool;
@@ -169,6 +173,7 @@
         g.tile = (M >= 4096 && (long long)((M + 255) / 256) * (N / 256) >= c->pp_min_tiles) ? 256 : 128;
     if (c->ring_tiles && g.tile == 0 && bf16 && N <= 1024 && N % 64 == 0 && (long long)((M + 63) / 64) * (N / 128) <= c->ring_tiles_max)
         g.tile = 6464;
+    if (c->gelu_erf_tile && g.tile == 0 && bf16 && g.act == VV_ACT_GELU_ERF_ && M >= 4096 && N % 256 == 0) g.tile = 64;
     const int esz = bf16 ? 2 : 4, osz = g.out_dtype == VV_DTYPE_BF16 ? 2 : 4;
     const double fl = alg_flops >= 0 ? alg_flops : 2.0 * M * (double)N * K;
     Prof p(c, cls, fl, (double)M * K * esz + (double)N * K * esz + (double)M * N * osz * (g.mode == VV_EPI_GATE_RES ? 2 : 1), st);
@@ -264,12 +269,27 @@
     if (c->fintab) hipFree(c->fintab);
     if (c->d_mult) hipFree(c->d_mult);
     if (c->x3_buf) hipFree(c->x3_buf);
+    if (c->mel_basis) hipFree(c->mel_basis);
     for (auto q : c->side_stream) if (q) hipStreamDestroy(q);
     if (c->ev_fork) hipEventDestroy(c->ev_fork);
     for (auto e : c->ev_join) if (e) hipEventDestroy(e);
     for (auto& r : c->recs) { hipEventDestroy(r.a); hipEventDestroy(r.b); }
     for (auto e : c->pool) hipEventDestroy(e);
     delete c;
+}
+
+static int build_mel_basis(vv_ctx* c) {
+    const int n_fft = c->cfg.n_fft;
+    c->w.erase("const.mel_basis");
+    if (!vvk_mel_matrix_ok(n_fft)) return 0;
+    hipSetDevice(c->device);
+    const int rows = pad_to(n_fft + 2, 128);
+    const uint64_t bytes = 4ull * rows * n_fft;
+    if (!c->mel_basis) HIPCHK(c, hipMalloc((void**)&c->mel_basis, bytes));
+    KCHK(c, vvk_mel_basis(c->Wf("const.tw_cos"), c->Wf("const.tw_sin"), c->mel_basis, n_fft, rows, nullptr, &m__));
+    HIPCHK(c, hipStreamSynchronize(nullptr));
+    c->w["const.mel_basis"] = Bound{c->mel_basis, bytes};
+    return 0;
 }
 
 int vv_bind_weight(vv_ctx* c, const char* name, const void* p, uint64_t bytes) {
@@ -335,6 +355,7 @@
         }
         need("voc.head.weight", 4 * HP * V); need("voc.head.bias", 4 * HP);
         if (!missing.empty()) return c->fail(-2, "missing or short weights: %s", missing.c_str());
+        if (int r = build_mel_basis(c)) return r;
         c->finalized = c->ever_finalized = true;
         return 0;
     }
@@ -359,6 +380,7 @@
     }
     need("voc.post.weight", 4ull * ch * g.voc_post_k); need("voc.post.bias", 4);
     if (!missing.empty()) return c->fail(-2, "missing or short weights: %s", missing.c_str());
+    if (int r = build_mel_basis(c)) return r;
     hipSetDevice(c->device);
     HIPCHK(c, hipMemcpy(&c->post_bias, c->W("voc.post.bias"), 4, hipMemcpyDeviceToHost));
     {
@@ -505,6 +527,40 @@
     return 0;
 }
 
+constexpr size_t MEL_CHUNK_ROWS = 32768;
+struct MelScratch { float* frames = nullptr; float* spec = nullptr; size_t rows = 0; int ld_spec = 0; };
+static bool mel_as_gemm(const vv_ctx* c) { return c->mel_form == 2 && vvk_mel_matrix_ok(c->cfg.n_fft) && c->W("const.mel_basis"); }
+static void mel_scratch(const vv_ctx* c, Arena& a, int B, int F_max, MelScratch* s) {
+    if (!mel_as_gemm(c) || B < 1 || F_max < 1) { *s = MelScratch{}; return; }
+    s->rows = std::min((size_t)B * F_max, MEL_CHUNK_ROWS);
+    s->ld_spec = pad_to(c->cfg.n_fft + 2, 128);
+    s->frames = a.take<float>(s->rows * c->cfg.n_fft);
+    s->spec = a.take<float>(s->rows * s->ld_spec);
+}
+static int mel_stage(vv_ctx* c, const int16_t* audio, int ld_audio, const int32_t* audio_len, float* mel, int B, int F_max, const MelScratch& s,
+                     hipStream_t st) {
+    const vv_model_cfg& g = c->cfg;
+    const int n_fft = g.n_fft, M = g.n_mel;
+    if (!s.frames) {
+        KCHK(c, vvk_mel(audio, ld_audio, audio_len, c->Wf("const.window"), c->Wf("const.tw_cos"), c->Wf("const.tw_sin"), c->Wf("const.mel_fb"), mel, B,
+                        F_max, n_fft, g.hop_length, M, st, &m__, c->mel_form != 0));
+        return 0;
+    }
+    KCHK(c, vvk_mel_args(audio, ld_audio, audio_len, c->Wf("const.window"), c->Wf("const.tw_cos"), c->Wf("const.tw_sin"), c->Wf("const.mel_fb"), mel, B,
+                         F_max, n_fft, g.hop_length, M, &m__));
+    const size_t R = (size_t)B * F_max;
+    for (size_t r0 = 0; r0 < R; r0 += s.rows) {
+        const size_t rows = std::min(s.rows, R - r0);
+        KCHK(c, vvk_mel_frames(audio, ld_audio, audio_len, c->Wf("const.window"), s.frames, r0, rows, F_max, n_fft, g.hop_length, st, &m__));
+        const Gemm gm = gemm_args(c, VV_DTYPE_F32, VV_DTYPE_F32, VV_EPI_STORE, VV_ACT_NONE_, s.frames, n_fft, "const.mel_basis", n_fft, nullptr, s.spec,
+                                  s.ld_spec, (int)rows, s.ld_spec, n_fft);
+        if (!gm.W) return c->fail(-2, "weight '%s' is not bound", gm.wname);
+        KCHK(c, vvk_gemm(&gm, st, &m__));
+        KCHK(c, vvk_mel_fb(s.spec, s.ld_spec, rows, audio_len, ld_audio, c->Wf("const.mel_fb"), mel, r0, F_max, n_fft, g.hop_length, M, st, &m__));
+    }
+    return 0;
+}
+
 static int preprocess_impl(vv_ctx* c, int B, int N, const int16_t* audio, int ld_audio, int max_audio_len, const int32_t* audio_len,
                            const int32_t* audio_len_host, const int32_t* text_ids, int ld_text, const int32_t* text_len, const int32_t* seq_len,
                            float* cat, float* cat_drop, int32_t* ref_len, void* stream, const uint8_t* keep = nullptr, int ld_keep = 0) {
@@ -527,8 +583,10 @@
     const size_t R2 = (size_t)2 * B * N;
     float *mel, *tx, *ty, *sumsq;
     char *th, *tm;
+    MelScratch ms;
     auto bufs = [&](Arena& a) {
         mel = a.take<float>((size_t)B * F_max * M);
+        mel_scratch(c, a, B, F_max, &ms);
         tx = a.take<float>(R2 * Dt); ty = a.take<float>(R2 * Dt);
         th = a.take<char>((size_t)es * R2 * Dt); tm = a.take<char>((size_t)es * R2 * C2);
         sumsq = a.take<float>((size_t)2 * B * C2);
@@ -538,8 +596,7 @@
     KCHK(c, vvk_ref_len(audio_len, ref_len, B, g.hop_length, st, &m__));
     {
         Prof p(c, VV_PROF_MEL, 4.0 * B * F_max * (double)g.n_fft * (g.n_fft / 2 + 1), 2.0 * B * max_audio_len + 4.0 * B * F_max * M, st);
-        KCHK(c, vvk_mel(audio, ld_audio, audio_len, c->Wf("const.window"), c->Wf("const.tw_cos"), c->Wf("const.tw_sin"),
-                        c->Wf("const.mel_fb"), mel, B, F_max, g.n_fft, g.hop_length, M, st, &m__));
+        if (int r = mel_stage(c, audio, ld_audio, audio_len, mel, B, F_max, ms, st)) return r;
     }
     {
         Prof p(c, VV_PROF_TEXT, 0, 8.0 * R2 * Dt, st);
@@ -549,7 +606,7 @@
         const std::string p = "text.blocks." + std::to_string(i);
         {
             Prof pr(c, VV_PROF_TEXT, 2.0 * R2 * Dt * g.text_conv_k, 8.0 * R2 * Dt, st);
-            KCHK(c, vvk_dwconv(tx, ty, c->Wf(p + ".dwconv.weight"), c->Wf(p + ".dwconv.bias"), seq_len, B, 2 * B, N, Dt, g.text_conv_k, st, &m__));
+            KCHK(c, vvk_dwconv(tx, ty, c->Wf(p + ".dwconv.weight"), c->Wf(p + ".dwconv.bias"), seq_len, B, 2 * B, N, Dt, g.text_conv_k, st, &m__, c->text_stream));
         }
         {
             vv_ln_args a{}; a.out_dtype = c->dt; a.x = ty; a.ldx = Dt; a.y = th; a.ldy = Dt; a.R = (int)R2; a.D = Dt;
@@ -561,7 +618,7 @@
         if (int r = launch_gemm(c, gemm_args(c, c->dt, c->dt, VV_EPI_STORE, VV_ACT_GELU_ERF_, th, Dt, w1.c_str(), Dt, b1.c_str(), tm, C2, (int)R2, C2, Dt), VV_PROF_GEMM, st)) return r;
         {
             Prof pr(c, VV_PROF_TEXT, 0, 3.0 * es * R2 * C2, st);
-            KCHK(c, vvk_grn(c->dt, tm, sumsq, c->Wf(p + ".grn.gamma"), c->Wf(p + ".grn.beta"), seq_len, B, 2 * B, N, C2, st, &m__));
+            KCHK(c, vvk_grn(c->dt, tm, sumsq, c->Wf(p + ".grn.gamma"), c->Wf(p + ".grn.beta"), seq_len, B, 2 * B, N, C2, st, &m__, c->text_stream));
         }
         if (int r = launch_gemm(c, gemm_args(c, c->dt, VV_DTYPE_F32, VV_EPI_GATE_RES, VV_ACT_NONE_, tm, C2, w2.c_str(), C2, b2.c_str(), tx, Dt, (int)R2, Dt, C2), VV_PROF_GEMM, st)) return r;
     }
@@ -1749,7 +1806,7 @@
         const std::string p = "voc.blocks." + std::to_string(i);
         {
             Prof pr(c, VV_PROF_VOC_CONV, 2.0 * R * (double)V * v.dw_k, 8.0 * R * V, st);
-            KCHK(c, vvk_dwconv(res, t, c->Wf(p + ".dwconv.weight"), c->Wf(p + ".dwconv.bias"), lens, B, B, T_max, V, v.dw_k, st, &m__));
+            KCHK(c, vvk_dwconv(res, t, c->Wf(p + ".dwconv.weight"), c->Wf(p + ".dwconv.bias"), lens, B, B, T_max, V, v.dw_k, st, &m__, c->text_stream));
         }
         if (int r = vocos_ln(c, t, hn, R, p + ".norm", st)) return r;
         const std::string w1 = p + ".pwconv1.weight", b1 = p + ".pwconv1.bias", w2 = p + ".pwconv2.weight", b2 = p + ".pwconv2.bias";
@@ -1866,6 +1923,12 @@
 int vv_set_option(vv_ctx* c, const char* name, int value) {
     if (!c || !name) return -22;
     if (!strcmp(name, "rope_rows")) { c->rope_rows = value != 0; return 0; }
+    if (!strcmp(name, "mel_form")) {
+        if (value < 0 || value > 2) return c->fail(-22, "vv_set_option: mel_form takes 0 (mel_kernel), 1 (one-walk direct transform, same bits) or 2 (fp32 GEMM on a constant basis)");
+        c->mel_form = value; return 0;
+    }
+    if (!strcmp(name, "text_stream")) { c->text_stream = value != 0; return 0; }
+    if (!strcmp(name, "gelu_erf_tile")) { c->gelu_erf_tile = value != 0; return 0; }
     if (!strcmp(name, "rope_q_attn")) { c->rope_q_attn = value != 0; return 0; }
     if (!strcmp(name, "voc_x3_rows")) {
         if (value != 0 && value != 128) return c->fail(-22, "vv_set_option: voc_x3_rows takes 0 (64-row workgroups) or 128");
@@ -1968,8 +2031,15 @@
     if (!c) return -22;
     if (!c->W("const.window") || !c->W("const.tw_cos") || !c->W("const.tw_sin") || !c->W("const.mel_fb"))
         return c->fail(-2, "vv_mel: constant tables not bound");
-    SINGLE(c, vvk_mel(audio, ld_audio, audio_len, c->Wf("const.window"), c->Wf("const.tw_cos"), c->Wf("const.tw_sin"), c->Wf("const.mel_fb"),
-                      mel, B, F_max, c->cfg.n_fft, c->cfg.hop_length, c->cfg.n_mel, (hipStream_t)st, &m__));
+    hipSetDevice(c->device);
+    {
+        const char* m__ = "";
+        if (int r = vvk_mel_args(audio, ld_audio, audio_len, c->Wf("const.window"), c->Wf("const.tw_cos"), c->Wf("const.tw_sin"), c->Wf("const.mel_fb"), mel,
+                                 B, F_max, c->cfg.n_fft, c->cfg.hop_length, c->cfg.n_mel, &m__)) return c->fail(r, "%s", m__);
+    }
+    MelScratch ms;
+    if (int r = plan_ws(c, nullptr, 0, [&](Arena& a) { mel_scratch(c, a, B, F_max, &ms); })) return r;
+    return mel_stage(c, audio, ld_audio, audio_len, mel, B, F_max, ms, (hipStream_t)st);
 }
 int vv_groupnorm(vv_ctx* c, const float* x, float* y, const float* gamma, const float* beta, int B, int C, int T, int G, float eps, int act, void* st) {
     SINGLE(c, vvk_groupnorm(x, y, gamma, beta, B, C, T, G, eps, act, (hipStream_t)st, &m__));
@@ -2062,7 +2132,7 @@
         return c->fail(-22, "vv_dwconv: bad arguments (out a buffer of its own, C a multiple of 4, KW odd, B >= 1 with seq_len)");
     if (((uintptr_t)in | (uintptr_t)out | (uintptr_t)bias) % 16 || ((uintptr_t)w | (uintptr_t)seq_len) % 4)
         return c->fail(-22, "vv_dwconv: in, out and bias must be 16-byte aligned, w and seq_len 4-byte");
-    SINGLE(c, vvk_dwconv(in, out, w, bias, seq_len, seq_len ? B : 1, n_seq, N, C, KW, (hipStream_t)st, &m__));
+    SINGLE(c, vvk_dwconv(in, out, w, bias, seq_len, seq_len ? B : 1, n_seq, N, C, KW, (hipStream_t)st, &m__, c ? c->text_stream : 1));
 }
 int vv_grn(vv_ctx* c, int dtype, void* x, float* sumsq, const float* gamma, const float* beta, const int32_t* seq_len, int B, int n_seq, int N,
            int C, void* st) {
@@ -2072,7 +2142,7 @@
         return c->fail(-22, "vv_grn: bad arguments (dtype f32 / bf16, C a multiple of 64 up to 8192, B >= 1 with seq_len)");
     if ((uintptr_t)x % (dtype == VV_DTYPE_BF16 ? 8 : 16) || (uintptr_t)beta % 16 || ((uintptr_t)sumsq | (uintptr_t)gamma | (uintptr_t)seq_len) % 4)
         return c->fail(-22, "vv_grn: x must be aligned to 4 elements, beta to 16 bytes, sumsq, gamma and seq_len to 4");
-    SINGLE(c, vvk_grn(dtype, x, sumsq, gamma, beta, seq_len, seq_len ? B : 1, n_seq, N, C, (hipStream_t)st, &m__));
+    SINGLE(c, vvk_grn(dtype, x, sumsq, gamma, beta, seq_len, seq_len ? B : 1, n_seq, N, C, (hipStream_t)st, &m__, c ? c->text_stream : 1));
 }
 int vv_cfg_euler(vv_ctx* c, float* x, const float* pred, int ldp, int BN, int n_mel, float cfg, float dt, void* st) {
     SINGLE(c, vvk_cfg_euler(x, pred, ldp, BN, n_mel, cfg, dt, nullptr, (hipStream_t)st, &m__));
diff --git a/vietvoice-tts_amd/csrc/vv_elementwise.hip b/vietvoice-tts_amd/csrc/vv_elementwise.hip
--- a/vietvoice-tts_amd/csrc/vv_elementwise.hip
+++ b/vietvoice-tts_amd/csrc/vv_elementwise.hip
@@ -717,6 +717,97 @@
 }
 
 #ifndef VV_ELEMENTWISE_HOST_CHECK
+constexpr int DW_RUN = 16;
+
+template <int KW, bool EDGE>
+__device__ __forceinline__ void dwconv_run(const float* __restrict__ src , float* __restrict__ dst,
+                                           const float4 (&w)[KW], float4 b4, int t0, int len, int N, int C) {
+    constexpr int pad = KW / 2;
+    float4 win[KW] = {};
+#pragma unroll
+    for (int j = 0; j < DW_RUN + KW - 1; ++j) {
+        const int tt = t0 - pad + j;
+#pragma unroll
+        for (int k = 0; k < KW - 1; ++k) win[k] = win[k + 1];
+        win[KW - 1] = (!EDGE || (tt >= 0 && tt < len)) ? *(const float4*)(src + (size_t)tt * C) : make_float4(0.f, 0.f, 0.f, 0.f);
+        if (j >= KW - 1) {
+            const int t = tt - pad;
+            float4 acc = b4;
+#pragma unroll
+            for (int k = 0; k < KW; ++k) {
+                const int tk = t + k - pad;
+                if (!EDGE || (tk >= 0 && tk < len)) {
+                    acc.x += w[k].x * win[k].x; acc.y += w[k].y * win[k].y; acc.z += w[k].z * win[k].z; acc.w += w[k].w * win[k].w;
+                }
+            }
+            if (!EDGE || t < N) *(float4*)(dst + (size_t)t * C) = acc;
+        }
+    }
+}
+
+template <int KW>
+__global__ __launch_bounds__(256) void dwconv_stream_kernel(const float* __restrict__ in, float* __restrict__ out, const float* __restrict__ w ,
+                                                            const float* __restrict__ bias, const int* __restrict__ seq_len, int B, int n_seq,
+                                                            int N, int C, int runs) {
+    const int c4 = C >> 2;
+    const size_t i = (size_t)blockIdx.x * 256 + threadIdx.x;
+    if (i >= (size_t)n_seq * runs * c4) return;
+    const int c = (int)(i % c4) * 4;
+    const size_t sr = i / c4;
+    const int t0 = (int)(sr % runs) * DW_RUN, s = (int)(sr / runs);
+    const int len = seq_len ? min(seq_len[s % B], N) : N;
+    float4 wk[KW];
+#pragma unroll
+    for (int k = 0; k < KW; ++k) wk[k] = make_float4(w[(c + 0) * KW + k], w[(c + 1) * KW + k], w[(c + 2) * KW + k], w[(c + 3) * KW + k]);
+    const float4 b4 = *(const float4*)(bias + c);
+    const float* src = in + (size_t)s * N * C + c;
+    float* dst = out + (size_t)s * N * C + c;
+    if (t0 >= KW / 2 && t0 + DW_RUN + KW / 2 <= len) dwconv_run<KW, false>(src, dst, wk, b4, t0, len, N, C);
+    else dwconv_run<KW, true>(src, dst, wk, b4, t0, len, N, C);
+}
+
+template <typename T>
+__global__ __launch_bounds__(64) void grn_stats_stream_kernel(const T* __restrict__ x, float* __restrict__ sumsq, const int* __restrict__ seq_len,
+                                                              int B, int N, int C) {
+    constexpr int V = 16 / sizeof(T), AHEAD = 16;
+    typedef __attribute__((ext_vector_type(4))) unsigned u4;
+    __shared__ float red[4][16 * V + 1];
+    const int s = blockIdx.y, lane = threadIdx.x & 15, ph = threadIdx.x >> 4;
+    const int c = (blockIdx.x * 16 + lane) * V;
+    const int len = seq_len ? min(seq_len[s % B], N) : N;
+    float acc[V];
+#pragma unroll
+    for (int e = 0; e < V; ++e) acc[e] = 0.f;
+    if (c < C) {
+        const T* p = x + (size_t)s * N * C + c;
+        auto add = [&](u4 raw) {
+#pragma unroll
+            for (int e = 0; e < V; ++e) {
+                float v;
+                if constexpr (sizeof(T) == 2) v = __uint_as_float((e & 1) ? (raw[e >> 1] & 0xFFFF0000u) : (raw[e >> 1] << 16));
+                else v = __uint_as_float(raw[e]);
+                acc[e] += v * v;
+            }
+        };
+        int t = ph;
+        for (; t + 4 * (AHEAD - 1) < len; t += 4 * AHEAD) {
+            u4 raw[AHEAD];
+#pragma unroll
+            for (int j = 0; j < AHEAD; ++j) raw[j] = *(const u4*)(p + (size_t)(t + 4 * j) * C);
+#pragma unroll
+            for (int j = 0; j < AHEAD; ++j) add(raw[j]);
+        }
+        for (; t < len; t += 4) add(*(const u4*)(p + (size_t)t * C));
+    }
+#pragma unroll
+    for (int e = 0; e < V; ++e) red[ph][lane * V + e] = acc[e];
+    __syncthreads();
+    for (int i = threadIdx.x; i < 16 * V; i += 64) {
+        const int cc = blockIdx.x * 16 * V + i;
+        if (cc < C) sumsq[(size_t)s * C + cc] = (red[0][i] + red[1][i]) + (red[2][i] + red[3][i]);
+    }
+}
+
 inline int grid_for(size_t total) { return (int)std::min<size_t>((total + 255) / 256, 256 * 8); }
 #endif
 
@@ -937,24 +1028,32 @@
 }
 
 int vvk_dwconv(const float* in, float* out, const float* w, const float* bias, const int* seq_len, int B, int n_seq, int N,
-               int C, int KW, hipStream_t st, const char** err) {
+               int C, int KW, hipStream_t st, const char** err, int stream) {
     if (C % 4) { *err = "dwconv: C % 4"; return -22; }
-    dwconv_kernel<<<grid_for((size_t)n_seq * N * C / 4), 256, 0, st>>>(in, out, w, bias, seq_len, B, n_seq, N, C, KW);
+    const int runs = (N + DW_RUN - 1) / DW_RUN;
+    const size_t items = (size_t)n_seq * runs * (C / 4);
+    if (stream && KW == 7 && items > 0 && (items + 255) / 256 <= 0x7fffffffull)
+        dwconv_stream_kernel<7><<<(unsigned)((items + 255) / 256), 256, 0, st>>>(in, out, w, bias, seq_len, B, n_seq, N, C, runs);
+    else
+        dwconv_kernel<<<grid_for((size_t)n_seq * N * C / 4), 256, 0, st>>>(in, out, w, bias, seq_len, B, n_seq, N, C, KW);
     VVK_CHECK_LAUNCH();
     return 0;
 }
 
 int vvk_grn(int dtype, void* x, float* sumsq, const float* gamma, const float* beta, const int* seq_len, int B, int n_seq,
-            int N, int C, hipStream_t st, const char** err) {
+            int N, int C, hipStream_t st, const char** err, int stream) {
     if (C % 64 || C > 8192) { *err = "grn: C must be a multiple of 64"; return -22; }
     dim3 g1(C / 64, n_seq);
     const int rpb = 16;
     dim3 g2((N + rpb - 1) / rpb, n_seq);
+    const bool fast = stream && (uintptr_t)x % 16 == 0 && n_seq <= 65535;
     if (dtype == VV_BF16) {
-        grn_stats_kernel<bf16><<<g1, 256, 0, st>>>((const bf16*)x, sumsq, seq_len, B, N, C);
+        if (fast) grn_stats_stream_kernel<bf16><<<dim3((C + 127) / 128, n_seq), 64, 0, st>>>((const bf16*)x, sumsq, seq_len, B, N, C);
+        else grn_stats_kernel<bf16><<<g1, 256, 0, st>>>((const bf16*)x, sumsq, seq_len, B, N, C);
         grn_apply_kernel<bf16><<<g2, 256, C * sizeof(float), st>>>((bf16*)x, sumsq, gamma, beta, N, C, rpb);
     } else {
-        grn_stats_kernel<float><<<g1, 256, 0, st>>>((const float*)x, sumsq, seq_len, B, N, C);
+        if (fast) grn_stats_stream_kernel<float><<<dim3(C / 64, n_seq), 64, 0, st>>>((const float*)x, sumsq, seq_len, B, N, C);
+        else grn_stats_kernel<float><<<g1, 256, 0, st>>>((const float*)x, sumsq, seq_len, B, N, C);
         grn_apply_kernel<float><<<g2, 256, C * sizeof(float), st>>>((float*)x, sumsq, gamma, beta, N, C, rpb);
     }
     VVK_CHECK_LAUNCH();
diff --git a/vietvoice-tts_amd/csrc/vv_kernels.h b/vietvoice-tts_amd/csrc/vv_kernels.h
--- a/vietvoice-tts_amd/csrc/vv_kernels.h
+++ b/vietvoice-tts_amd/csrc/vv_kernels.h
@@ -21,7 +21,15 @@
                   hipStream_t st, const char** err);
 int vvk_mel(const int16_t* audio, int ld_audio, const int* audio_len, const float* window, const float* tw_cos,
             const float* tw_sin, const float* fb, float* mel, int B, int F_max, int n_fft, int hop, int n_mel, hipStream_t st,
-            const char** err);
+            const char** err, int direct = 1);
+int vvk_mel_args(const int16_t* audio, int ld_audio, const int* audio_len, const float* window, const float* tw_cos, const float* tw_sin,
+                 const float* fb, const float* mel, int B, int F_max, int n_fft, int hop, int n_mel, const char** err);
+int vvk_mel_matrix_ok(int n_fft);
+int vvk_mel_basis(const float* tw_cos, const float* tw_sin, float* basis, int n_fft, int n_rows, hipStream_t st, const char** err);
+int vvk_mel_frames(const int16_t* audio, int ld_audio, const int* audio_len, const float* window, float* fr, size_t r0, size_t rows, int F_max,
+                   int n_fft, int hop, hipStream_t st, const char** err);
+int vvk_mel_fb(const float* spec, int ld_spec, size_t rows, const int* audio_len, int ld_audio, const float* fb, float* mel, size_t r0, int F_max,
+               int n_fft, int hop, int n_mel, hipStream_t st, const char** err);
 int vvk_pack_cat(int dtype, const float* x, const float* cat, const float* cat_drop, void* out, int ldo, int BN, int n_mel,
                  int cond_dim, int only_x, const int* row_src, hipStream_t st, const char** err);
 int vvk_cfg_euler(float* x, const float* pred, int ldp, int BN, int n_mel, float cfg, float dt, const int* row_src, hipStream_t st,
@@ -40,9 +48,9 @@
 int vvk_text_embed(const int* ids, int ld_ids, const int* text_len, const float* emb, const float* pos, float* out, int B, int N,
                    int Dt, int vocab_rows, hipStream_t st, const char** err);
 int vvk_dwconv(const float* in, float* out, const float* w, const float* bias, const int* seq_len, int B, int n_seq, int N, int C,
-               int KW, hipStream_t st, const char** err);
+               int KW, hipStream_t st, const char** err, int stream = 1);
 int vvk_grn(int dtype, void* x, float* sumsq, const float* gamma, const float* beta, const int* seq_len, int B, int n_seq, int N,
-            int C, hipStream_t st, const char** err);
+            int C, hipStream_t st, const char** err, int stream = 1);
 int vvk_build_cat(const float* mel, int F_max, const int* ref_len, const float* text, float* cat, float* cat_drop, int B, int N,
                   int n_mel, int Dt, hipStream_t st, const char** err, const uint8_t* keep = nullptr, int ld_keep = 0);
 int vvk_ref_len(const int* audio_len, int* ref_len, int B, int hop, hipStream_t st, const char** err);
diff --git a/vietvoice-tts_amd/csrc/vv_mel.hip b/vietvoice-tts_amd/csrc/vv_mel.hip
--- a/vietvoice-tts_amd/csrc/vv_mel.hip
+++ b/vietvoice-tts_amd/csrc/vv_mel.hip
@@ -63,16 +63,232 @@
 }
 
 #ifndef VV_MEL_HOST_CHECK
-int vvk_mel(const int16_t* audio, int ld_audio, const int* audio_len, const float* window, const float* tw_cos, const float* tw_sin,
-            const float* fb, float* mel, int B, int F_max, int n_fft, int hop, int n_mel, hipStream_t st, const char** err) {
+namespace {
+
+constexpr int MEL_DIRECT_THREADS = 320, MEL_DIRECT_FRAMES = 4;
+__device__ __forceinline__ float mel_mag(float re, float im) {
+#pragma clang fp contract(off)
+    const float rr = re * re, ii = im * im;
+    return sqrtf(rr + ii);
+}
+__global__ __launch_bounds__(MEL_DIRECT_THREADS) void mel_direct_kernel(const int16_t* __restrict__ audio, int ld_audio,
+                                                                        const int* __restrict__ audio_len, const float* __restrict__ window,
+                                                                        const float* __restrict__ tw_cos, const float* __restrict__ tw_sin,
+                                                                        const float* __restrict__ fb, float* __restrict__ mel, int F_max,
+                                                                        int n_fft, int hop, int n_mel) {
+    constexpr int FR = MEL_DIRECT_FRAMES;
+    extern __shared__ __attribute__((aligned(16))) char smem[];
+    float4* fr = (float4*)smem;
+    float2* tw = (float2*)(fr + n_fft);
+    float* mag = (float*)(tw + n_fft);
+    const int b = blockIdx.y, f0 = blockIdx.x * FR, tid = threadIdx.x;
+    const int L = min(max(audio_len[b], 0), ld_audio);
+    const int S = max(L, 1);
+    const int frames = L / hop + 1;
+    const int nb = n_fft / 2 + 1, half = n_fft / 2, quarter = n_fft / 4;
+    if (f0 >= frames) {
+        for (int i = tid; i < FR * n_mel; i += MEL_DIRECT_THREADS) {
+            const int f = f0 + i / n_mel;
+            if (f < F_max) mel[((size_t)b * F_max + f) * n_mel + i % n_mel] = 0.f;
+        }
+        return;
+    }
+    const int16_t* a = audio + (size_t)b * ld_audio;
+    for (int i = tid; i < n_fft * FR; i += MEL_DIRECT_THREADS) {
+        const int n = i / FR, q = i % FR;
+        int pos = (f0 + q) * hop + n - half;
+        if (pos < 0) pos = -pos;
+        if (pos >= S) pos = 2 * (S - 1) - pos;
+        pos = min(max(pos, 0), S - 1);
+        ((float*)fr)[i] = (float)a[pos] * (1.0f / 32768.0f) * window[n];
+    }
+    for (int n = tid; n < n_fft; n += MEL_DIRECT_THREADS) tw[n] = make_float2(tw_cos[n], tw_sin[n]);
+    __syncthreads();
+    const int mask = n_fft - 1;
+    if (tid < 256) {
+        for (int k = tid; k < quarter; k += 256) {
+            const int k2 = k + quarter;
+            float re[FR] = {}, im[FR] = {}, re2[FR] = {}, im2[FR] = {};
+#pragma unroll 2
+            for (int n = 0; n < n_fft; ++n) {
+                const float4 x4 = fr[n];
+                const float x[FR] = {x4.x, x4.y, x4.z, x4.w};
+                const float2 w1 = tw[(n * k) & mask], w2 = tw[(n * k2) & mask];
+#pragma unroll
+                for (int q = 0; q < FR; ++q) {
+                    re[q] = fmaf(x[q], w1.x, re[q]);
+                    im[q] = fmaf(x[q], w1.y, im[q]);
+                    re2[q] = fmaf(x[q], w2.x, re2[q]);
+                    im2[q] = fmaf(x[q], w2.y, im2[q]);
+                }
+            }
+#pragma unroll
+            for (int q = 0; q < FR; ++q) {
+                mag[q * nb + k] = mel_mag(re[q], im[q]);
+                mag[q * nb + k2] = mel_mag(re2[q], im2[q]);
+            }
+        }
+    } else if (tid == 256) {
+        float re[FR] = {}, im[FR] = {};
+#pragma unroll 2
+        for (int n = 0; n < n_fft; ++n) {
+            const float4 x4 = fr[n];
+            const float x[FR] = {x4.x, x4.y, x4.z, x4.w};
+            const float2 w1 = tw[(n * half) & mask];
+#pragma unroll
+            for (int q = 0; q < FR; ++q) {
+                re[q] = fmaf(x[q], w1.x, re[q]);
+                im[q] = fmaf(x[q], w1.y, im[q]);
+            }
+        }
+#pragma unroll
+        for (int q = 0; q < FR; ++q) mag[q * nb + half] = mel_mag(re[q], im[q]);
+    }
+    __syncthreads();
+    for (int i = tid; i < FR * n_mel; i += MEL_DIRECT_THREADS) {
+        const int q = i / n_mel, m = i % n_mel, f = f0 + q;
+        if (f >= F_max) continue;
+        float acc = 0.f;
+        if (f < frames)
+            for (int k = 0; k < nb; ++k) acc = fmaf(fb[(size_t)k * n_mel + m], mag[q * nb + k], acc);
+        mel[((size_t)b * F_max + f) * n_mel + m] = f < frames ? logf(fmaxf(acc, 1e-5f)) : 0.f;
+    }
+}
+
+__global__ __launch_bounds__(256) void mel_basis_kernel(const float* __restrict__ tw_cos, const float* __restrict__ tw_sin,
+                                                        float* __restrict__ basis, int n_fft) {
+    const int j = blockIdx.x, k = j >> 1, mask = n_fft - 1;
+    const bool live = j < 2 * (n_fft / 2 + 1);
+    const float* tw = (j & 1) ? tw_sin : tw_cos;
+    for (int n = threadIdx.x; n < n_fft; n += 256) basis[(size_t)j * n_fft + n] = live ? tw[(n * k) & mask] : 0.f;
+}
+
+__global__ __launch_bounds__(256) void mel_frames_kernel(const int16_t* __restrict__ audio, int ld_audio, const int* __restrict__ audio_len,
+                                                         const float* __restrict__ window, float* __restrict__ fr ,
+                                                         size_t r0, int F_max, int n_fft, int hop) {
+    const size_t r = r0 + blockIdx.x;
+    const int b = (int)(r / F_max), f = (int)(r % F_max);
+    const int L = min(max(audio_len[b], 0), ld_audio);
+    const int S = max(L, 1);
+    const int frames = L / hop + 1;
+    float* dst = fr + (size_t)blockIdx.x * n_fft;
+    const int16_t* a = audio + (size_t)b * ld_audio;
+    const int half = n_fft / 2;
+    for (int n = threadIdx.x * 4; n < n_fft; n += 1024) {
+        float v[4];
+#pragma unroll
+        for (int j = 0; j < 4; ++j) {
+            int pos = f * hop + n + j - half;
+            if (pos < 0) pos = -pos;
+            if (pos >= S) pos = 2 * (S - 1) - pos;
+            pos = min(max(pos, 0), S - 1);
+            v[j] = f < frames ? (float)a[pos] * (1.0f / 32768.0f) * window[n + j] : 0.f;
+        }
+        *(float4*)(dst + n) = make_float4(v[0], v[1], v[2], v[3]);
+    }
+}
+
+__global__ __launch_bounds__(256) void mel_fb_kernel(const float* __restrict__ spec, int ld_spec, size_t rows, const int* __restrict__ audio_len,
+                                                     int ld_audio, const float* __restrict__ fb, float* __restrict__ mel, size_t r0, int F_max,
+                                                     int n_fft, int hop, int n_mel) {
+    extern __shared__ __attribute__((aligned(16))) char smem[];
+    float* mag = (float*)smem;
+    const int nb = n_fft / 2 + 1;
+    const size_t c0 = (size_t)blockIdx.x * 8;
+    for (int i = threadIdx.x; i < nb * 8; i += 256) {
+        const int q = i / nb, k = i - q * nb;
+        float m = 0.f;
+        if (c0 + q < rows) {
+            const float2 v = *(const float2*)(spec + (c0 + q) * ld_spec + 2 * k);
+            const float re = v.x, im = v.y;
+            m = sqrtf(re * re + im * im);
+        }
+        mag[k * 8 + q] = m;
+    }
+    __syncthreads();
+    const int q0 = (threadIdx.x >> 7) * 4;
+    bool live[4];
+    size_t out[4];
+#pragma unroll
+    for (int j = 0; j < 4; ++j) {
+        const size_t r = r0 + c0 + q0 + j;
+        const int b = (int)(r / F_max), f = (int)(r % F_max);
+        const bool in = c0 + q0 + j < rows;
+        live[j] = in && f < min(max(audio_len[in ? b : 0], 0), ld_audio) / hop + 1;
+        out[j] = in ? r * n_mel : (size_t)-1;
+    }
+    for (int m = threadIdx.x & 127; m < n_mel; m += 128) {
+        float acc[4] = {0.f, 0.f, 0.f, 0.f};
+#pragma unroll 8
+        for (int k = 0; k < nb; ++k) {
+            const float w = fb[(size_t)k * n_mel + m];
+            const float4 g = *(const float4*)(mag + k * 8 + q0);
+            acc[0] = fmaf(w, g.x, acc[0]); acc[1] = fmaf(w, g.y, acc[1]); acc[2] = fmaf(w, g.z, acc[2]); acc[3] = fmaf(w, g.w, acc[3]);
+        }
+#pragma unroll
+        for (int j = 0; j < 4; ++j)
+            if (out[j] != (size_t)-1) mel[out[j] + m] = live[j] ? logf(fmaxf(acc[j], 1e-5f)) : 0.f;
+    }
+}
+
+int mel_check(const void* audio, int ld_audio, const void* audio_len, const void* window, const void* tw_cos, const void* tw_sin, const void* fb,
+              const void* mel, int B, int F_max, int n_fft, int hop, int n_mel, const char** err) {
     if (B <= 0 || F_max <= 0) { *err = "mel: empty"; return -22; }
     if (!audio || !audio_len || !mel || !window || !tw_cos || !tw_sin || !fb) { *err = "mel: audio, audio_len, mel and the four tables are required"; return -22; }
     if (ld_audio < 1 || hop < 1 || n_mel < 1) { *err = "mel: ld_audio, hop and n_mel must be at least 1"; return -22; }
     if (n_fft < 2 || n_fft & (n_fft - 1) || n_fft > 4096) { *err = "mel: n_fft must be a power of two within [2, 4096]"; return -22; }
     if (B > 65535) { *err = "mel: at most 65535 clips per launch (grid.y)"; return -22; }
+    return 0;
+}
+
+}
+
+int vvk_mel_matrix_ok(int n_fft) { return n_fft >= 32 && n_fft <= 2048 && !(n_fft & (n_fft - 1)); }
+
+int vvk_mel_args(const int16_t* audio, int ld_audio, const int* audio_len, const float* window, const float* tw_cos, const float* tw_sin,
+                 const float* fb, const float* mel, int B, int F_max, int n_fft, int hop, int n_mel, const char** err) {
+    return mel_check(audio, ld_audio, audio_len, window, tw_cos, tw_sin, fb, mel, B, F_max, n_fft, hop, n_mel, err);
+}
+
+int vvk_mel_basis(const float* tw_cos, const float* tw_sin, float* basis, int n_fft, int n_rows, hipStream_t st, const char** err) {
+    if (!tw_cos || !tw_sin || !basis || !vvk_mel_matrix_ok(n_fft) || n_rows < n_fft + 2) { *err = "mel basis: the twiddle tables, a buffer of >= n_fft + 2 rows, n_fft a power of two in [32, 2048]"; return -22; }
+    mel_basis_kernel<<<n_rows, 256, 0, st>>>(tw_cos, tw_sin, basis, n_fft);
+    hipError_t he = hipGetLastError();
+    if (he != hipSuccess) { *err = hipGetErrorString(he); return -5; }
+    return 0;
+}
+
+int vvk_mel_frames(const int16_t* audio, int ld_audio, const int* audio_len, const float* window, float* fr, size_t r0, size_t rows, int F_max,
+                   int n_fft, int hop, hipStream_t st, const char** err) {
+    if (!audio || !audio_len || !window || !fr || rows < 1 || rows > 0x7fffffffull || F_max < 1 || ld_audio < 1 || hop < 1 || !vvk_mel_matrix_ok(n_fft) ||
+        (uintptr_t)fr % 16) { *err = "mel frames: bad arguments"; return -22; }
+    mel_frames_kernel<<<(unsigned)rows, 256, 0, st>>>(audio, ld_audio, audio_len, window, fr, r0, F_max, n_fft, hop);
+    hipError_t he = hipGetLastError();
+    if (he != hipSuccess) { *err = hipGetErrorString(he); return -5; }
+    return 0;
+}
+
+int vvk_mel_fb(const float* spec, int ld_spec, size_t rows, const int* audio_len, int ld_audio, const float* fb, float* mel, size_t r0, int F_max,
+               int n_fft, int hop, int n_mel, hipStream_t st, const char** err) {
+    if (!spec || !audio_len || !fb || !mel || rows < 1 || rows > 0x7fffffffull || F_max < 1 || ld_audio < 1 || hop < 1 || n_mel < 1 ||
+        !vvk_mel_matrix_ok(n_fft) || ld_spec < n_fft + 2 || ld_spec % 2 || (uintptr_t)spec % 8) { *err = "mel filterbank: bad arguments"; return -22; }
+    const size_t lds = (size_t)(n_fft / 2 + 1) * 8 * sizeof(float);
+    mel_fb_kernel<<<(unsigned)((rows + 7) / 8), 256, lds, st>>>(spec, ld_spec, rows, audio_len, ld_audio, fb, mel, r0, F_max, n_fft, hop, n_mel);
+    hipError_t he = hipGetLastError();
+    if (he != hipSuccess) { *err = hipGetErrorString(he); return -5; }
+    return 0;
+}
+
+int vvk_mel(const int16_t* audio, int ld_audio, const int* audio_len, const float* window, const float* tw_cos, const float* tw_sin,
+            const float* fb, float* mel, int B, int F_max, int n_fft, int hop, int n_mel, hipStream_t st, const char** err, int direct) {
+    if (int r = mel_check(audio, ld_audio, audio_len, window, tw_cos, tw_sin, fb, mel, B, F_max, n_fft, hop, n_mel, err)) return r;
     const size_t lds = (size_t)(3 * n_fft + n_fft / 2 + 1) * sizeof(float);
     dim3 grid(F_max, B);
-    mel_kernel<<<grid, 256, lds, st>>>(audio, ld_audio, audio_len, window, tw_cos, tw_sin, fb, mel, F_max, n_fft, hop, n_mel);
+    if (direct && n_fft >= 4 && n_fft <= 1024)
+        mel_direct_kernel<<<dim3((F_max + MEL_DIRECT_FRAMES - 1) / MEL_DIRECT_FRAMES, B), MEL_DIRECT_THREADS,
+                            (size_t)n_fft * 24 + (size_t)MEL_DIRECT_FRAMES * (n_fft / 2 + 1) * sizeof(float), st>>>(audio, ld_audio, audio_len, window, tw_cos, tw_sin, fb, mel, F_max, n_fft, hop, n_mel);
+    else
+        mel_kernel<<<grid, 256, lds, st>>>(audio, ld_audio, audio_len, window, tw_cos, tw_sin, fb, mel, F_max, n_fft, hop, n_mel);
     hipError_t he = hipGetLastError();
     if (he != hipSuccess) { *err = hipGetErrorString(he); return -5; }
     return 0;
```

New measurement: 184.9 (median of 6 runs). No clear change (+0.3%).
